# ina-foss/inaSpeechSegmenter

Hardware: AMD Instinct MI355X
Metric: hours-of-audio segmented/sec (smn+gender, 16 kHz mono) (higher is better)
Workload: dtype f32 (f16x3 split-operand MFMA, f32 accumulate; f64 FFT)

## Files before the change

### inaspeechsegmenter_amd/_native.py

```python
import ctypes as C
import os

import numpy as np

_HERE = os.path.dirname(os.path.abspath(__file__))
LIB_PATH = os.environ.get('ISS_LIB') or os.path.join(_HERE, 'libiss_hip.so')

PROG_COLS = 32
OP_CONV, OP_POOL, OP_SOFTMAX, OP_STATPOOL, OP_ACT, OP_ELT = 1, 2, 3, 4, 5, 6
(ELT_COPY, ELT_ADD, ELT_SUB, ELT_MUL, ELT_MAX, ELT_MIN, ELT_AVG, ELT_ZERO, ELT_PERMUTE) = range(9)
(C_OP, C_IN, C_OUT, C_RES, C_H, C_W, C_CIN, C_HO, C_WO, C_COUT, C_KH, C_KW, C_SH, C_SW, C_PT, C_PL,
 C_ACT, C_WOFF, C_BOFF, C_PSOFF, C_PTOFF, C_INMODE, C_POOLKIND, C_ORDER, C_FPOOLH, C_FPOOLW, C_DUALW, C_DUALB, C_ACTPARAM, C_ACTPARAM2, C_ACTPARAM3) = range(31)
PREC_BF16X3, PREC_F32, PREC_F16X3 = 0, 1, 2
K_ALIGN = 32
BUF_INPUT = -2
MAX_NETS = 8
RS_JOB = np.dtype([('src_offset', '<i8'), ('frames_in', '<i8'), ('channels', '<i4'), ('format', '<i4'), ('filter', '<i4'),
                   ('reserved', '<i4'), ('dst_offset', '<i8'), ('frames_out', '<i8')])
RS_FORMAT = {np.dtype(np.uint8): 0, np.dtype('<i2'): 1, np.dtype('<i4'): 2, np.dtype('<f4'): 3, np.dtype('<f8'): 4}
RS_I8, RS_ULAW, RS_ALAW, RS_SWAP = 8, 9, 10, 0x100
ADPCM_JOB = np.dtype([('src_offset', '<i8'), ('block_begin', '<i8'), ('nblocks', '<i8'), ('frames_total', '<i8'), ('channels', '<i4'),
                      ('block_align', '<i4'), ('output', '<i4'), ('filter', '<i4'), ('dst_offset', '<i8'), ('frames_out', '<i8')])
ADPCM_TO_SIGNAL, ADPCM_TO_STAGE = 0, 1
ADPCM_STATUS = {1: 'step index above 88'}
FLAC_INFO = np.dtype([('sample_rate', '<i4'), ('channels', '<i4'), ('bps', '<i4'), ('min_block', '<i4'), ('max_block', '<i4'),
                      ('reserved', '<i4'), ('total_samples', '<i8')])
FLAC_FRAME = np.dtype([('offset', '<i8'), ('length', '<i8'), ('first_sample', '<i8'), ('block_size', '<i4'),
                       ('channel_mode', '<i4'), ('bps', '<i4'), ('header_bytes', '<i4')])
FLAC_JOB = np.dtype([('src_offset', '<i8'), ('frame_begin', '<i8'), ('nframes', '<i8'), ('frames_total', '<i8'), ('channels', '<i4'),
                     ('bps', '<i4'), ('output', '<i4'), ('filter', '<i4'), ('dst_offset', '<i8'), ('frames_out', '<i8')])
FLAC_TO_SIGNAL, FLAC_TO_STAGE = 0, 1
FLAC_STATUS = {1: 'reserved subframe type', 2: 'subframe header padding bit set', 3: 'wasted bits exceed the sample size',
               4: 'reserved residual coding method', 5: 'residual partition order does not fit the block',
               6: 'invalid LPC precision', 7: 'negative LPC shift', 8: 'residual overruns the frame',
               9: 'nonzero padding before the footer', 10: 'subframes end before the footer', 11: 'CRC-16 mismatch'}


class NativeError(RuntimeError):
    pass


_lib = None


def lib():
    global _lib
    if _lib is not None:
        return _lib
    if not os.path.exists(LIB_PATH):
        raise NativeError(
            f"{LIB_PATH} is missing: the HIP extension has not been built. "
            "Run `python -c 'import __graft_entry__ as g; g.build()'` (needs hipcc). "
            "There is no CPU fallback for the feature/CNN path.")
    try:
        import torch
    except ImportError:
        pass
    L = C.CDLL(LIB_PATH)
    vp, i32, i64, u64 = C.c_void_p, C.c_int32, C.c_int64, C.c_uint64
    pf, pd, pi32, pi64, pu8, pi16 = (C.POINTER(C.c_float), C.POINTER(C.c_double), C.POINTER(C.c_int32),
                                     C.POINTER(C.c_int64), C.POINTER(C.c_uint8), C.POINTER(C.c_int16))
    sig = {
        'iss_create': (C.c_int, [C.c_int, C.POINTER(vp)]),
        'iss_destroy': (None, [vp]),
        'iss_last_error': (C.c_char_p, [vp]),
        'iss_version': (C.c_char_p, []),
        'iss_set_workspace_limit': (C.c_int, [vp, u64]),
        'iss_synchronize': (C.c_int, [vp]),
        'iss_sidekit_tables': (C.c_int, [vp, pd, pf]),
        'iss_signal_pcm16': (C.c_int, [vp, pi16, i64]),
        'iss_signal_f32': (C.c_int, [vp, pf, i64]),
        'iss_signal_pcm16_device': (C.c_int, [vp, vp, i64]),
        'iss_signal_pcm16_device_stream': (C.c_int, [vp, vp, i64, vp]),
        'iss_resample_filter': (C.c_int, [vp, i32, i32, pd, i64, pi32]),
        'iss_resample_pcm16': (C.c_int, [vp, vp, i64, vp, i32, i64]),
        'iss_get_signal_pcm16': (C.c_int, [vp, pi16, i64, i64]),
        'iss_resample_stats': (C.c_int, [vp, pi64, pi64]),
        'iss_flac_index': (C.c_int, [vp, i64, i64, vp, vp, i64, pi64, pi64, C.c_char_p, i32]),
        'iss_flac_crc': (C.c_int, [vp, i64, pi32, pi32]),
        'iss_flac_decode_host': (C.c_int, [vp, i64, vp, i64, i32, i32, i64, vp, pi32]),
        'iss_flac_decode': (C.c_int, [vp, vp, i64, vp, i64, vp, i32, i64, pi32]),
        'iss_flac_get_stage': (C.c_int, [vp, i32, vp, i64]),
        'iss_flac_stats': (C.c_int, [vp, pi64, pi64]),
        'iss_adpcm_decode_host': (C.c_int, [vp, i64, i64, i32, i32, i64, pi16, pi32]),
        'iss_adpcm_decode': (C.c_int, [vp, vp, i64, vp, i32, i64, i64, pi32]),
        'iss_adpcm_get_stage': (C.c_int, [vp, i32, vp, i64]),
        'iss_adpcm_stats': (C.c_int, [vp, pi64, pi64]),
        'iss_host_alloc': (C.c_int, [vp, C.c_size_t, C.POINTER(vp)]),
        'iss_host_free': (C.c_int, [vp, vp]),
        'iss_cnn_probs_async': (C.c_int, [vp, C.c_int, pi32, i32, pf, pu8, pi64]),
        'iss_cnn_dead_stats': (C.c_int, [vp, pi64, pi64]),
        'iss_wait': (C.c_int, [vp, i64]),
        'iss_comm_unique_id': (C.c_int, [vp, pu8]),
        'iss_comm_init': (C.c_int, [vp, pu8, i32, i32]),
        'iss_comm_destroy': (C.c_int, [vp]),
        'iss_allgather_segments': (C.c_int, [vp, pi32, i32, i32, pi32, pi32]),
        'iss_comm_allreduce_max': (C.c_int, [vp, pd]),
        'iss_comm_info': (C.c_int, [vp, pi32, pi32, pi32, C.c_char_p, i32]),
        'iss_sidekit': (C.c_int, [vp, pi32]),
        'iss_get_loge': (C.c_int, [vp, pf]),
        'iss_get_mspec': (C.c_int, [vp, pf]),
        'iss_set_mspec': (C.c_int, [vp, pf, i32]),
        'iss_cnn_load': (C.c_int, [vp, C.c_int, pi32, i32, pf, i64, i32, pi64, i32, i32, i32, i32]),
        'iss_cnn_load_shared': (C.c_int, [vp, C.c_int, C.c_int, pi32, i32, i32, pi64, i32, i32, i32, i32]),
        'iss_cnn_probs': (C.c_int, [vp, C.c_int, pi32, i32, pf, pu8]),
        'iss_cnn_forward': (C.c_int, [vp, C.c_int, pf, i32, pf]),
        'iss_cnn_flops': (C.c_int, [vp, C.c_int, pd]),
        'iss_set_precision': (C.c_int, [vp, C.c_int]),
        'iss_set_precision_guard': (C.c_int, [vp, C.c_float]),
        'iss_cnn_precision_info': (C.c_int, [vp, C.c_int, pi32, pf, pi32, pi32, pf]),
        'iss_cnn_set_net_precision': (C.c_int, [vp, C.c_int, C.c_int]),
        'iss_vbx_tables': (C.c_int, [vp, pd, pd]),
        'iss_vbx_features': (C.c_int, [vp, pi32, pd, i64, pf, pi32]),
        'iss_vbx_set_dither': (C.c_int, [vp, pd, i64]),
        'iss_vbx_features_pcm16': (C.c_int, [vp, pi16, i64, pf, pi32]),
        'iss_vbx_features_batch_pcm16': (C.c_int, [vp, pi16, pi64, i32, pi32, pf]),
        'iss_vbx_embed': (C.c_int, [vp, C.c_int, pi32, i32, pf]),
        'iss_prof_enable': (C.c_int, [vp, C.c_int]),
        'iss_prof_get': (C.c_int, [vp, C.c_int, pd, pi64, pd]),
        'iss_prof_reset': (C.c_int, [vp]),
        'iss_prof_get_row': (C.c_int, [vp, C.c_int, pd, pi64]),
        'iss_prof_get_instance': (C.c_int, [vp, C.c_int, C.c_char_p, i32, pd, pi64, pd]),
        'iss_set_diag': (C.c_int, [vp, C.c_uint32]),
        'iss_scribble': (C.c_int, [vp, C.c_uint32]),
        'iss_viterbi_f64': (C.c_int, [pd, i64, i32, pd, pi32]),
        'iss_viterbi_f32': (C.c_int, [pf, i64, i32, pd, pi32]),
        'iss_energy_viterbi': (C.c_int, [pf, i64, C.c_double, C.c_double, C.c_double, pd, pi32]),
        'iss_viterbi_segments_f32': (C.c_int, [pf, pi64, i64, i32, pd, pi32]),
    }
    for name, (res, args) in sig.items():
        fn = getattr(L, name)
        fn.restype = res
        fn.argtypes = args
    L._iss_symbols = tuple(sig)
    _lib = L
    return L


DIAG_BITS = {'no_shared_first': 0x001, 'no_flrows': 0x002, 'no_ws': 0x004, 'no_ws3': 0x008, 'no_direct1': 0x010,
             'no_nh2': 0x020, 'no_tr': 0x040, 'no_pw': 0x080, 'no_pws': 0x100, 'no_pws2': 0x200, 'no_wq': 0x400,
             'no_dual': 0x800, 'no_chain': 0x1000, 'no_ring': 0x2000, 'no_fsame': 0x4000, 'no_f32ws': 0x8000, 'no_ncb1': 0x10000, 'no_wsu3': 0x20000, 'no_gfused': 0x40000, 'no_hl': 0x80000,
             'no_skip_dead': 0x100000}


def diag_flags(names):
    flags = 0
    for nm in str(names).replace(' ', '').replace('+', ',').lower().split(','):
        if nm:
            flags |= DIAG_BITS[nm]
    return flags


def _ptr(a, ty):
    return a.ctypes.data_as(C.POINTER(ty))


def viterbi(emission, transition):
    L = lib()
    em = np.ascontiguousarray(emission)
    if em.dtype not in (np.float32, np.float64):
        em = em.astype(np.float64)
    tr = np.ascontiguousarray(transition, dtype=np.float64)
    T, K = em.shape
    out = np.empty(T, dtype=np.int32)
    if em.dtype == np.float32:
        rc = L.iss_viterbi_f32(_ptr(em, C.c_float), T, K, _ptr(tr, C.c_double), _ptr(out, C.c_int32))
    else:
        rc = L.iss_viterbi_f64(_ptr(em, C.c_double), T, K, _ptr(tr, C.c_double), _ptr(out, C.c_int32))
    if rc != 0:
        raise NativeError(f"iss_viterbi failed ({rc}): T={T} K={K}")
    return out


def viterbi_segments(emission, seg_len, transition):
    L = lib()
    em = np.ascontiguousarray(emission, dtype=np.float32)
    sl = np.ascontiguousarray(seg_len, dtype=np.int64)
    tr = np.ascontiguousarray(transition, dtype=np.float64)
    n, K = em.shape
    assert int(sl.sum()) == n
    out = np.empty(n, dtype=np.int32)
    rc = L.iss_viterbi_segments_f32(_ptr(em, C.c_float), _ptr(sl, C.c_int64), sl.size, K, _ptr(tr, C.c_double), _ptr(out, C.c_int32))
    if rc != 0:
        raise NativeError(f"iss_viterbi_segments_f32 failed ({rc}): n={n} K={K} segments={sl.size}")
    return out


_LOG_EPS = np.log(np.full(1, 1e-10))[0], np.log(np.full(1, 1 - 1e-10))[0]


def energy_viterbi(loge, threshold, transition):
    L = lib()
    x = np.ascontiguousarray(loge, dtype=np.float32)
    tr = np.ascontiguousarray(transition, dtype=np.float64)
    out = np.empty(x.size, dtype=np.int32)
    rc = L.iss_energy_viterbi(_ptr(x, C.c_float), x.size, float(threshold), float(_LOG_EPS[0]), float(_LOG_EPS[1]),
                              _ptr(tr, C.c_double), _ptr(out, C.c_int32))
    if rc != 0:
        raise NativeError(f"iss_energy_viterbi failed ({rc}): T={x.size}")
    return out


def flac_crc(buf):
    b = np.frombuffer(bytes(buf), dtype=np.uint8)
    c8, c16 = C.c_int32(), C.c_int32()
    if lib().iss_flac_crc(C.c_void_p(b.ctypes.data), b.size, C.byref(c8), C.byref(c16)) != 0:
        raise NativeError('iss_flac_crc failed')
    return c8.value, c16.value


def flac_index(buf, first_frame, info):
    L = lib()
    inf = np.ascontiguousarray(np.array(info, dtype=FLAC_INFO).reshape(1))
    cap = max(16, int(inf['total_samples'][0]) // max(1, int(inf['min_block'][0]) or 1) + 2) if inf['total_samples'][0] > 0 \
        else buf.size // 64 + 16
    err = C.create_string_buffer(256)
    n, off = C.c_int64(), C.c_int64()
    for _ in range(2):
        rows = np.zeros(cap, dtype=FLAC_FRAME)
        rc = L.iss_flac_index(C.c_void_p(buf.ctypes.data), buf.size, int(first_frame), C.c_void_p(inf.ctypes.data),
                              C.c_void_p(rows.ctypes.data), cap, C.byref(n), C.byref(off), err, 256)
        if rc != -5:
            break
        cap = buf.size // 9 + 16
    if rc != 0:
        raise ValueError(off.value, err.value.decode())
    return rows[:n.value].copy()


def flac_decode_host(buf, frames, channels, bps, frames_total):
    fr = np.ascontiguousarray(frames, dtype=FLAC_FRAME)
    out = np.empty((int(frames_total), int(channels)), dtype=np.int32 if bps > 16 else np.int16)
    st = np.zeros(len(fr), dtype=np.int32)
    rc = lib().iss_flac_decode_host(C.c_void_p(buf.ctypes.data), buf.size, C.c_void_p(fr.ctypes.data), len(fr), int(channels),
                                    int(bps), int(frames_total), C.c_void_p(out.ctypes.data), _ptr(st, C.c_int32))
    if rc != 0:
        raise NativeError(f'iss_flac_decode_host failed ({rc}): bad frame rows')
    return (out[:, 0] if channels == 1 else out), st


def adpcm_decode_host(buf, nblocks, channels, block_align, frames_total):
    buf = np.ascontiguousarray(buf, dtype=np.uint8)
    out = np.empty((int(frames_total), int(channels)), dtype=np.int16)
    st = np.zeros(int(nblocks), dtype=np.int32)
    rc = lib().iss_adpcm_decode_host(C.c_void_p(buf.ctypes.data), buf.size, int(nblocks), int(channels), int(block_align),
                                     int(frames_total), _ptr(out, C.c_int16), _ptr(st, C.c_int32))
    if rc != 0:
        raise NativeError(f'iss_adpcm_decode_host failed ({rc}): bad block geometry')
    return (out[:, 0] if channels == 1 else out), st


class Context:

    def __init__(self, device=0):
        self._L = lib()
        h = C.c_void_p()
        rc = self._L.iss_create(int(device), C.byref(h))
        if rc != 0:
            raise NativeError(f"iss_create(device={device}) failed ({rc}): "
                              f"{self._L.iss_last_error(None).decode()}")
        self._h = h
        self.device = device
        self.T = 0
        self._net_out = {}
        self._dither_n = 0
        self._pinned = {}
        self.comm_rank, self.comm_world = 0, 1
        self.precision = None
        self.workspace_limit = None
        self.diag = 0
        env = os.environ.get('ISS_DIAG', '')
        if env:
            self.set_diag(diag_flags(env))
        self.guard_threshold = None
        env = os.environ.get('ISS_PREC_GUARD', '')
        if env:
            self.set_precision_guard(float(env))

    def close(self):
        if getattr(self, '_h', None):
            for p in list(self._pinned.values()):
                self._L.iss_host_free(self._h, C.c_void_p(p))
            self._pinned.clear()
            self._L.iss_destroy(self._h)
            self._h = None

    def __del__(self):
        try:
            self.close()
        except Exception:
            pass

    def _ck(self, rc, what):
        if rc != 0:
            raise NativeError(f"{what} failed ({rc}): {self._L.iss_last_error(self._h).decode()}")

    def sidekit_tables(self, window, melbank):
        w = np.ascontiguousarray(window, dtype=np.float64)
        b = np.ascontiguousarray(melbank, dtype=np.float32)
        assert w.shape == (400,) and b.shape == (24, 257)
        self._ck(self._L.iss_sidekit_tables(self._h, _ptr(w, C.c_double), _ptr(b, C.c_float)), 'iss_sidekit_tables')

    def set_signal(self, sig):
        sig = np.ascontiguousarray(sig)
        if sig.dtype == np.int16:
            self._ck(self._L.iss_signal_pcm16(self._h, _ptr(sig, C.c_int16), sig.size), 'iss_signal_pcm16')
        elif sig.dtype == np.float32:
            self._ck(self._L.iss_signal_f32(self._h, _ptr(sig, C.c_float), sig.size), 'iss_signal_f32')
        else:
            raise TypeError(f"signal dtype {sig.dtype}: need int16 or float32")
        self._keep = sig

    def set_signal_device(self, dev_ptr, n, producer_stream=None):
        self._ck(self._L.iss_signal_pcm16_device_stream(self._h, C.c_void_p(int(dev_ptr)), int(n),
                                                        C.c_void_p(int(producer_stream)) if producer_stream else None),
                 'iss_signal_pcm16_device')

    def resample_filter(self, sr):
        from . import resample
        up, down, h = resample.plan(sr)
        fid = C.c_int32()
        self._ck(self._L.iss_resample_filter(self._h, up, down, _ptr(h, C.c_double), h.size, C.byref(fid)), 'iss_resample_filter')
        return fid.value, up, down

    def resample_job(self, x, sr, src_offset, dst_offset, fmt=None):
        fid, up, down = self.resample_filter(sr)
        n = x.shape[0]
        return (src_offset, n, 1 if x.ndim == 1 else x.shape[1], RS_FORMAT[x.dtype] if fmt is None else int(fmt), fid, 0,
                dst_offset, -(-n * up // down))

    def resample(self, src, jobs, n_signal=-1):
        src = np.ascontiguousarray(src, dtype=np.uint8)
        jb = np.ascontiguousarray(np.array(jobs, dtype=RS_JOB))
        self._ck(self._L.iss_resample_pcm16(self._h, C.c_void_p(src.ctypes.data), src.size, C.c_void_p(jb.ctypes.data),
                                            jb.size, int(n_signal)), 'iss_resample_pcm16')
        self._keep_rs = src

    def resample_signal(self, x, sr, fmt=None):
        x = np.ascontiguousarray(x)
        job = self.resample_job(x, sr, 0, 0, fmt)
        self.resample(x.reshape(-1).view(np.uint8), [job], n_signal=job[-1])
        return job[-1]

    def get_signal_pcm16(self, offset, n):
        out = np.empty(int(n), dtype=np.int16)
        self._ck(self._L.iss_get_signal_pcm16(self._h, _ptr(out, C.c_int16), int(offset), int(n)), 'iss_get_signal_pcm16')
        return out

    def _counters(self, fn):
        a, b = C.c_int64(), C.c_int64()
        self._ck(getattr(self._L, fn)(self._h, C.byref(a), C.byref(b)), fn)
        return a.value, b.value

    def _get_stage(self, fn, job, frames_total, channels, dtype):
        out = np.empty((int(frames_total), int(channels)), dtype=dtype)
        self._ck(getattr(self._L, fn)(self._h, int(job), C.c_void_p(out.ctypes.data), out.nbytes), fn)
        return out[:, 0] if channels == 1 else out

    def resample_stats(self):
        return self._counters('iss_resample_stats')

    def _status(self, name, n):
        st, n = self.__dict__.get(name), max(int(n), 1)
        if st is None or st.size < n:
            if st is not None:
                self.pinned_free(st)
            st = self.__dict__[name] = self.pinned_empty((int(n * 1.25) + 256,), np.int32)
        return st

    def flac_decode(self, src, frames, jobs, n_signal=-1):
        src = np.ascontiguousarray(src, dtype=np.uint8)
        fr = np.ascontiguousarray(frames, dtype=FLAC_FRAME)
        jb = np.ascontiguousarray(np.array(jobs, dtype=FLAC_JOB).reshape(-1))
        st = self._status('_flac_status', len(fr))
        self._ck(self._L.iss_flac_decode(self._h, C.c_void_p(src.ctypes.data), src.size, C.c_void_p(fr.ctypes.data), len(fr),
                                         C.c_void_p(jb.ctypes.data), jb.size, int(n_signal), _ptr(st, C.c_int32)),
                 'iss_flac_decode')
        self._keep_flac = (src, fr)
        return st[:len(fr)]

    def flac_get_stage(self, job, frames_total, channels, bps):
        return self._get_stage('iss_flac_get_stage', job, frames_total, channels, np.int32 if bps > 16 else np.int16)

    def flac_stats(self):
        return self._counters('iss_flac_stats')

    def adpcm_decode(self, src, jobs, nblocks, n_signal=-1):
        src = np.ascontiguousarray(src, dtype=np.uint8)
        jb = np.ascontiguousarray(np.array(jobs, dtype=ADPCM_JOB).reshape(-1))
        st = self._status('_adpcm_status', nblocks)
        self._ck(self._L.iss_adpcm_decode(self._h, C.c_void_p(src.ctypes.data), src.size, C.c_void_p(jb.ctypes.data), jb.size,
                                          int(nblocks), int(n_signal), _ptr(st, C.c_int32)), 'iss_adpcm_decode')
        self._keep_adpcm = src
        return st[:int(nblocks)]

    def adpcm_get_stage(self, job, frames_total, channels):
        return self._get_stage('iss_adpcm_get_stage', job, frames_total, channels, np.int16)

    def adpcm_stats(self):
        return self._counters('iss_adpcm_stats')

    def pinned_empty(self, shape, dtype):
        dt = np.dtype(dtype)
        n = int(np.prod(shape)) * dt.itemsize
        p = C.c_void_p()
        self._ck(self._L.iss_host_alloc(self._h, n, C.byref(p)), 'iss_host_alloc')
        buf = (C.c_uint8 * max(n, 1)).from_address(p.value)
        a = np.frombuffer(buf, dtype=dt, count=int(np.prod(shape))).reshape(shape)
        self._pinned[a.ctypes.data] = p.value
        return a

    def pinned_free(self, a):
        p = self._pinned.pop(a.ctypes.data, None)
        if p is not None and self._h:
            self._ck(self._L.iss_host_free(self._h, C.c_void_p(p)), 'iss_host_free')

    def sidekit(self):
        t = C.c_int32()
        self._ck(self._L.iss_sidekit(self._h, C.byref(t)), 'iss_sidekit')
        self.T = t.value
        return self.T

    def get_loge(self):
        out = np.empty(self.T, dtype=np.float32)
        self._ck(self._L.iss_get_loge(self._h, _ptr(out, C.c_float)), 'iss_get_loge')
        return out

    def get_mspec(self):
        out = np.empty((self.T, 24), dtype=np.float32)
        self._ck(self._L.iss_get_mspec(self._h, _ptr(out, C.c_float)), 'iss_get_mspec')
        return out

    def set_mspec(self, mspec):
        m = np.ascontiguousarray(mspec, dtype=np.float32)
        assert m.ndim == 2 and m.shape[1] == 24
        self._ck(self._L.iss_set_mspec(self._h, _ptr(m, C.c_float), m.shape[0]), 'iss_set_mspec')
        self.T = m.shape[0]

    def cnn_load(self, net_id, compiled):
        prog = np.ascontiguousarray(compiled.prog, dtype=np.int32)
        blob = np.ascontiguousarray(compiled.blob, dtype=np.float32)
        be = np.ascontiguousarray(compiled.buf_elems, dtype=np.int64)
        h, w, c = compiled.in_shape
        self._ck(self._L.iss_cnn_load(self._h, net_id, _ptr(prog, C.c_int32), prog.shape[0], _ptr(blob, C.c_float),
                                      blob.size, be.size, _ptr(be, C.c_int64), h, w, c, compiled.out_dim),
                 'iss_cnn_load')
        self._net_out[net_id] = compiled.out_dim

    def cnn_load_shared(self, net_id, src_id, compiled):
        prog = np.ascontiguousarray(compiled.prog, dtype=np.int32)
        be = np.ascontiguousarray(compiled.buf_elems, dtype=np.int64)
        h, w, c = compiled.in_shape
        self._ck(self._L.iss_cnn_load_shared(self._h, net_id, src_id, _ptr(prog, C.c_int32), prog.shape[0], be.size,
                                             _ptr(be, C.c_int64), h, w, c, compiled.out_dim), 'iss_cnn_load_shared')
        self._net_out[net_id] = compiled.out_dim

    def cnn_probs(self, net_id, win_row):
        wr = np.ascontiguousarray(win_row, dtype=np.int32)
        n = wr.size
        probs = np.empty((n, self._net_out[net_id]), dtype=np.float32)
        fin = np.empty(n, dtype=np.uint8)
        self._ck(self._L.iss_cnn_probs(self._h, net_id, _ptr(wr, C.c_int32), n, _ptr(probs, C.c_float),
                                       _ptr(fin, C.c_uint8)), 'iss_cnn_probs')
        return probs, fin.astype(bool)

    def cnn_probs_async(self, net_id, win_row, probs_out=None, finite_out=None):
        wr = np.ascontiguousarray(win_row, dtype=np.int32)
        n = wr.size
        if probs_out is None:
            probs_out = np.empty((n, self._net_out[net_id]), dtype=np.float32)
        if finite_out is None:
            finite_out = np.empty(n, dtype=np.uint8)
        assert probs_out.size >= n * self._net_out[net_id] and finite_out.size >= n
        t = C.c_int64(-1)
        self._ck(self._L.iss_cnn_probs_async(self._h, net_id, _ptr(wr, C.c_int32), n, _ptr(probs_out, C.c_float),
                                             _ptr(finite_out, C.c_uint8), C.byref(t)), 'iss_cnn_probs_async')
        return t.value, probs_out, finite_out

    def cnn_dead_stats(self):
        w, d = C.c_int64(0), C.c_int64(0)
        self._ck(self._L.iss_cnn_dead_stats(self._h, C.byref(w), C.byref(d)), 'iss_cnn_dead_stats')
        return {'windows': w.value, 'dead': d.value}

    def wait(self, ticket=-1):
        self._ck(self._L.iss_wait(self._h, int(ticket)), 'iss_wait')

    def comm_unique_id(self):
        buf = np.zeros(128, dtype=np.uint8)
        self._ck(self._L.iss_comm_unique_id(self._h, _ptr(buf, C.c_uint8)), 'iss_comm_unique_id')
        return buf.tobytes()

    def comm_init(self, uid, rank, world):
        buf = np.frombuffer(bytes(uid), dtype=np.uint8).copy()
        assert buf.size == 128
        self._ck(self._L.iss_comm_init(self._h, _ptr(buf, C.c_uint8), int(rank), int(world)), 'iss_comm_init')
        self.comm_rank, self.comm_world = int(rank), int(world)

    def comm_destroy(self):
        self._ck(self._L.iss_comm_destroy(self._h), 'iss_comm_destroy')
        self.comm_rank, self.comm_world = 0, 1

    def allgather_segments(self, rows, capacity):
        world = self.comm_world
        out = np.zeros((world, capacity, 4), dtype=np.int32)
        counts = np.zeros(world, dtype=np.int32)
        if rows is None:
            rows, n = np.zeros((1, 4), np.int32), -1
        else:
            rows = np.ascontiguousarray(rows, dtype=np.int32).reshape(-1, 4)
            n = rows.shape[0]
        self._ck(self._L.iss_allgather_segments(self._h, _ptr(rows, C.c_int32), n, int(capacity),
                                                _ptr(out, C.c_int32), _ptr(counts, C.c_int32)), 'iss_allgather_segments')
        return out, counts

    def comm_info(self):
        w, r, v = C.c_int32(), C.c_int32(), C.c_int32()
        buf = C.create_string_buffer(512)
        self._ck(self._L.iss_comm_info(self._h, C.byref(w), C.byref(r), C.byref(v), buf, 512), 'iss_comm_info')
        return {'world': w.value, 'rank': r.value, 'version': v.value, 'lib': buf.value.decode(errors='replace')}

    def comm_allreduce_max(self, value):
        v = C.c_double(float(value))
        self._ck(self._L.iss_comm_allreduce_max(self._h, C.byref(v)), 'iss_comm_allreduce_max')
        return v.value

    def cnn_forward(self, net_id, x):
        x = np.ascontiguousarray(x, dtype=np.float32)
        n = x.shape[0]
        out = np.empty((n, self._net_out[net_id]), dtype=np.float32)
        self._ck(self._L.iss_cnn_forward(self._h, net_id, _ptr(x, C.c_float), n, _ptr(out, C.c_float)), 'iss_cnn_forward')
        return out

    def cnn_flops(self, net_id):
        f = C.c_double()
        self._ck(self._L.iss_cnn_flops(self._h, net_id, C.byref(f)), 'iss_cnn_flops')
        return f.value

    def set_precision(self, mode):
        self._ck(self._L.iss_set_precision(self._h, int(mode)), 'iss_set_precision')
        self.precision = int(mode)

    def set_precision_guard(self, threshold):
        self._ck(self._L.iss_set_precision_guard(self._h, float(threshold)), 'iss_set_precision_guard')
        self.guard_threshold = float(threshold)

    def cnn_precision_info(self, net_id):
        mode, slots, state, d, du = C.c_int32(0), C.c_int32(0), C.c_int32(0), C.c_float(0), C.c_float(0)
        self._ck(self._L.iss_cnn_precision_info(self._h, int(net_id), C.byref(mode), C.byref(d), C.byref(slots), C.byref(state), C.byref(du)),
                 'iss_cnn_precision_info')
        return {'mode': {PREC_F32: 'f32', PREC_F16X3: 'f16x3'}.get(mode.value, 'bf16x3'), 'max_dlogp': None if d.value < 0 else float(d.value),
                'max_dlogp_in_use': None if du.value < 0 else float(du.value),
                'slots': slots.value, 'state': ('pending', 'passed', 'escalated', 'fixed')[state.value]}

    def cnn_set_net_precision(self, net_id, mode):
        self._ck(self._L.iss_cnn_set_net_precision(self._h, int(net_id), int(mode)), 'iss_cnn_set_net_precision')

    def set_workspace_limit(self, nbytes):
        self._ck(self._L.iss_set_workspace_limit(self._h, int(nbytes)), 'iss_set_workspace_limit')
        self.workspace_limit = int(nbytes)

    def mirror_settings(self, other):
        if getattr(other, 'precision', None) is not None and other.precision != getattr(self, 'precision', None):
            self.set_precision(other.precision)
        if getattr(other, 'workspace_limit', None) is not None and other.workspace_limit != getattr(self, 'workspace_limit', None):
            self.set_workspace_limit(other.workspace_limit)
        if getattr(other, 'diag', 0) != getattr(self, 'diag', 0):
            self.set_diag(other.diag)
        if getattr(other, 'guard_threshold', None) is not None and other.guard_threshold != getattr(self, 'guard_threshold', None):
            self.set_precision_guard(other.guard_threshold)

    def set_diag(self, flags):
        flags = diag_flags(flags) if isinstance(flags, str) else int(flags)
        self._ck(self._L.iss_set_diag(self._h, flags), 'iss_set_diag')
        self.diag = flags

    def scribble(self, word):
        self._ck(self._L.iss_scribble(self._h, int(word) & 0xFFFFFFFF), 'iss_scribble')

    def synchronize(self):
        self._ck(self._L.iss_synchronize(self._h), 'iss_synchronize')

    def vbx_tables(self, window, melbank):
        w = np.ascontiguousarray(window, dtype=np.float64)
        b = np.ascontiguousarray(melbank, dtype=np.float64)
        assert w.shape == (400,) and b.shape == (257, 64)
        self._ck(self._L.iss_vbx_tables(self._h, _ptr(w, C.c_double), _ptr(b, C.c_double)), 'iss_vbx_tables')

    def vbx_features(self, sig_i32, dither_u):
        s = np.ascontiguousarray(sig_i32, dtype=np.int32)
        u = np.ascontiguousarray(dither_u, dtype=np.float64)
        assert s.shape == u.shape and s.ndim == 1
        T = (s.size + 320 - 400) // 160 + 1
        out = np.empty((T, 64), dtype=np.float32)
        t = C.c_int32()
        self._ck(self._L.iss_vbx_features(self._h, _ptr(s, C.c_int32), _ptr(u, C.c_double), s.size,
                                          _ptr(out, C.c_float), C.byref(t)), 'iss_vbx_features')
        self._dither_n = 0
        assert t.value == T
        return out

    def vbx_set_dither(self, dither_u):
        u = np.ascontiguousarray(dither_u, dtype=np.float64)
        self._ck(self._L.iss_vbx_set_dither(self._h, _ptr(u, C.c_double), u.size), 'iss_vbx_set_dither')
        self._dither_n = u.size

    def vbx_features_pcm16(self, pcm, to_host=True):
        s = np.ascontiguousarray(pcm, dtype=np.int16)
        T = (s.size + 320 - 400) // 160 + 1
        t = C.c_int32()
        if not to_host:
            self._ck(self._L.iss_vbx_features_pcm16(self._h, _ptr(s, C.c_int16), s.size, None, C.byref(t)), 'iss_vbx_features_pcm16')
            assert t.value == T
            return T
        out = np.empty((T, 64), dtype=np.float32)
        self._ck(self._L.iss_vbx_features_pcm16(self._h, _ptr(s, C.c_int16), s.size, _ptr(out, C.c_float), C.byref(t)),
                 'iss_vbx_features_pcm16')
        assert t.value == T
        return out

    def vbx_features_batch_pcm16(self, pcms, to_host=True):
        pcms = [np.asarray(p, dtype=np.int16) for p in pcms]
        soff = np.zeros(len(pcms) + 1, dtype=np.int64)
        soff[1:] = np.cumsum([p.size for p in pcms])
        s = np.ascontiguousarray(np.concatenate(pcms) if pcms else np.zeros(0, np.int16))
        foff = np.zeros(len(pcms) + 1, dtype=np.int32)
        T = int(sum((p.size + 320 - 400) // 160 + 1 for p in pcms))
        out = np.empty((T, 64), dtype=np.float32) if to_host else None
        self._ck(self._L.iss_vbx_features_batch_pcm16(self._h, _ptr(s, C.c_int16), _ptr(soff, C.c_int64), len(pcms),
                                                      _ptr(foff, C.c_int32), _ptr(out, C.c_float) if to_host else None),
                 'iss_vbx_features_batch_pcm16')
        return foff, out

    def vbx_embed(self, net_id, starts):
        st = np.ascontiguousarray(starts, dtype=np.int32)
        out = np.empty((st.size, self._net_out[net_id]), dtype=np.float32)
        self._ck(self._L.iss_vbx_embed(self._h, net_id, _ptr(st, C.c_int32), st.size, _ptr(out, C.c_float)), 'iss_vbx_embed')
        return out

    def prof_enable(self, on=True):
        self._ck(self._L.iss_prof_enable(self._h, 1 if on else 0), 'iss_prof_enable')

    def prof_reset(self):
        self._ck(self._L.iss_prof_reset(self._h), 'iss_prof_reset')

    def prof_get(self, kind):
        ms, n, fl = C.c_double(), C.c_int64(), C.c_double()
        self._ck(self._L.iss_prof_get(self._h, kind, C.byref(ms), C.byref(n), C.byref(fl)), 'iss_prof_get')
        return ms.value, n.value, fl.value

    def prof_instances(self):
        out = []
        buf = C.create_string_buffer(192)
        i = 0
        while True:
            ms, n, fl = C.c_double(), C.c_int64(), C.c_double()
            if self._L.iss_prof_get_instance(self._h, i, buf, 192, C.byref(ms), C.byref(n), C.byref(fl)) != 0:
                break
            out.append({'kernel': buf.value.decode(), 'ms': ms.value, 'launches': n.value, 'flops': fl.value})
            i += 1
        return out

    def prof_get_row(self, row):
        ms, n = C.c_double(), C.c_int64()
        self._ck(self._L.iss_prof_get_row(self._h, int(row), C.byref(ms), C.byref(n)), 'iss_prof_get_row')
        return ms.value, n.value
```

### inaspeechsegmenter_amd/csrc/cnn.hip

```cpp
#include "conv_select.h"

using namespace issk;

namespace {

template <int MODE>
__global__ __launch_bounds__(256) void conv_igemm_kernel(const ConvArgs p) {
    __shared__ __attribute__((aligned(16))) float sA[2][BM * LDK];
    __shared__ __attribute__((aligned(16))) float sB[2][BN * LDK];

    const int tid = threadIdx.x, lane = tid & 63, wv = tid >> 6;
    unsigned mt, nt;
    gemm_tile_of_block(blockIdx.x, p.nblk, p.nblk_n, mt, nt);
    const long long m0 = (long long)mt * BM;
    const int n0 = (int)nt * BN;

    const int k4 = tid & 3;
    const int lr = tid >> 2;
    RowSrc rs[2];
#pragma unroll
    for (int j = 0; j < 2; ++j) rs[j] = row_source<MODE>(p, m0 + lr + 64 * j);
    const int bn = n0 + lr;
    const bool bok = bn < p.Cout;
    const float* wrow = p.w + (size_t)(bok ? bn : 0) * p.Kpad + k4 * 4;
// ... 918 lines not shown
    return ISS_OK;
}

namespace {
int cnn_set_program(iss_ctx* c, IssNet& n, const char* who, const int32_t* prog, int32_t nrows, int64_t blob_floats,
                    int32_t nbuf, const int64_t* buf_elems, int32_t in_h, int32_t in_w, int32_t in_c, int32_t out_dim,
                    std::vector<int32_t>& ktab) {
    n.prog.assign(prog, prog + (size_t)nrows * ISS_PROG_COLS);
    n.nrows = nrows; n.nbuf = nbuf; n.buf_elems.assign(buf_elems, buf_elems + nbuf);
    n.in_h = in_h; n.in_w = in_w; n.in_c = in_c; n.out_dim = out_dim;
    n.kpad.assign(nrows, 0); n.ktab_off.assign(nrows, -1);
    double flops = 0;
    for (int r = 0; r < nrows; ++r) {
        const int32_t* R = &n.prog[(size_t)r * ISS_PROG_COLS];
        auto bad = [&](const char* what) { return iss_fail(c, ISS_EINVAL, "%s: row %d: %s", who, r, what); };
        if (R[ISS_C_IN] != ISS_BUF_INPUT && (R[ISS_C_IN] < 0 || R[ISS_C_IN] >= nbuf)) return bad("IN buffer id");
        if (R[ISS_C_OUT] < 0 || R[ISS_C_OUT] >= nbuf) return bad("OUT buffer id");
        if (R[ISS_C_OP] == ISS_OP_CONV) {
            const int K = R[ISS_C_KH] * R[ISS_C_KW] * R[ISS_C_CIN];
            const int Kpad = roundup(K, KALIGN);
            if (K <= 0 || R[ISS_C_COUT] <= 0) return bad("conv shape");
            if (R[ISS_C_WOFF] < 0 || (R[ISS_C_WOFF] & 7) || (int64_t)R[ISS_C_WOFF] + (int64_t)R[ISS_C_COUT] * Kpad > blob_floats)
                return bad("weight offset misaligned or outside blob (weights must be [Cout][roundup32(K)], offset % 8 == 0)");
            if (R[ISS_C_RES] >= nbuf) return bad("RES buffer id");
            if (R[ISS_C_KH] > 32767 || R[ISS_C_KW] > 32767) return bad("kernel too large");
            int fph, fpw;
            fused_pool_of(R, fph, fpw);
            if (fph * fpw != 1 && fph * fpw != 2 && fph * fpw != 4) return bad("fused pool window must cover 2 or 4 outputs");
            if (fph * fpw > 1 && (R[ISS_C_RES] >= 0 || R[ISS_C_HO] / fph < 1 || R[ISS_C_WO] / fpw < 1))
                return bad("fused pool with residual / empty pooled output");
            const bool patch = R[ISS_C_INMODE] == 1;
            const bool window = R[ISS_C_INMODE] == 2;
            if (patch && (R[ISS_C_CIN] != 1 || R[ISS_C_H] != 68 || R[ISS_C_W] > 24)) return bad("patch-mode conv must read (68, <=24, 1)");
            if (window && (R[ISS_C_CIN] != 1 || R[ISS_C_H] != 64)) return bad("window-mode conv must read (64, frames, 1)");
            const int rs = patch ? 24 : (window ? 1 : R[ISS_C_W] * R[ISS_C_CIN]);
            const int ps = patch ? 1 : (window ? R[ISS_C_H] : R[ISS_C_CIN]);
            n.kpad[r] = Kpad; n.ktab_off[r] = (int64_t)ktab.size();
            for (int k = 0; k < Kpad; ++k) {
                if (k < K) {
                    const int cc = k % R[ISS_C_CIN], kk = k / R[ISS_C_CIN];
                    const int kx = kk % R[ISS_C_KW], ky = kk / R[ISS_C_KW];
                    ktab.push_back(ky * rs + kx * ps + cc);
                    ktab.push_back((ky << 16) | kx);
                } else {
                    ktab.push_back(0);
                    ktab.push_back((0x7fff << 16) | 0x7fff);
                }
            }
            flops += 2.0 * K * R[ISS_C_COUT] * (double)(R[ISS_C_HO] / fph * fph) * (double)(R[ISS_C_WO] / fpw * fpw);
            if (R[ISS_C_DUALW] != 0 || R[ISS_C_DUALB] != 0) {
                if (r < 1) return bad("ISS_C_DUALW on the first row");
                const int32_t* P = &n.prog[(size_t)(r - 1) * ISS_PROG_COLS];
                int pph, ppw;
                fused_pool_of(P, pph, ppw);
                const bool shapes = P[ISS_C_OP] == ISS_OP_CONV && P[ISS_C_KH] == 1 && P[ISS_C_KW] == 1 && R[ISS_C_KH] == 1 && R[ISS_C_KW] == 1 &&
                                    R[ISS_C_SH] == 1 && R[ISS_C_SW] == 1 && P[ISS_C_SH] >= 1 && P[ISS_C_SW] >= 1 &&
                                    R[ISS_C_PT] == 0 && R[ISS_C_PL] == 0 && P[ISS_C_PT] == 0 && P[ISS_C_PL] == 0 &&
                                    R[ISS_C_INMODE] == 0 && P[ISS_C_INMODE] == 0 && fph * fpw == 1 && pph * ppw == 1 &&
                                    R[ISS_C_HO] == R[ISS_C_H] && R[ISS_C_WO] == R[ISS_C_W] && P[ISS_C_HO] == R[ISS_C_HO] &&
                                    P[ISS_C_WO] == R[ISS_C_WO] && P[ISS_C_COUT] == R[ISS_C_COUT] &&
                                    (P[ISS_C_HO] - 1) * P[ISS_C_SH] < P[ISS_C_H] && (P[ISS_C_WO] - 1) * P[ISS_C_SW] < P[ISS_C_W] &&
                                    R[ISS_C_CIN] % 32 == 0 && P[ISS_C_CIN] % 32 == 0;
                const bool chain = R[ISS_C_RES] >= 0 && R[ISS_C_RES] == P[ISS_C_OUT] && R[ISS_C_OUT] == R[ISS_C_RES] &&
                                   R[ISS_C_IN] != P[ISS_C_OUT] && P[ISS_C_IN] != P[ISS_C_OUT] && P[ISS_C_RES] < 0 && P[ISS_C_ACT] == 0 &&
                                   P[ISS_C_PSOFF] < 0 && R[ISS_C_PSOFF] < 0 && P[ISS_C_BOFF] >= 0 && R[ISS_C_BOFF] >= 0;
                const int64_t wo = (int64_t)R[ISS_C_DUALW] - 1, bo = (int64_t)R[ISS_C_DUALB] - 1;
                const bool offs = wo >= 0 && bo >= 0 && (wo & 7) == 0 &&
                                  wo + (int64_t)R[ISS_C_COUT] * (R[ISS_C_CIN] + P[ISS_C_CIN]) <= blob_floats && bo + R[ISS_C_COUT] <= blob_floats;
                if (!shapes || !chain || !offs)
                    return bad("ISS_C_DUALW / ISS_C_DUALB: rows r - 1, r are not a linear 1x1 projection and the in-place 1x1 expansion it is added to, "
                               "or the concatenated parameters lie outside the blob (include/iss.h)");
            }
        } else if (R[ISS_C_OP] == ISS_OP_ACT) {
            if (R[ISS_C_ACT] < 4 || R[ISS_C_ACT] > 9) return bad("ISS_OP_ACT: activation code must be 4 (elu), 5 (leaky relu), 6 (selu), 7 (softplus), 8 (relu with max_value) or 9 (keras ReLU in full)");
            if (R[ISS_C_IN] == ISS_BUF_INPUT) return bad("ISS_OP_ACT: an elementwise activation cannot read the network input (it works in place)");
        } else if (R[ISS_C_OP] == ISS_OP_ELT) {
            const int k = R[ISS_C_ACT];
            const long long hw = (long long)R[ISS_C_H] * R[ISS_C_W];
            if (k < ISS_ELT_COPY || k > ISS_ELT_PERMUTE) return bad("ISS_OP_ELT: unknown kind");
            if (R[ISS_C_HO] < 1 || R[ISS_C_WO] < 1 || R[ISS_C_COUT] < 1 || R[ISS_C_CIN] < 1 || hw < 1) return bad("ISS_OP_ELT: shape");
            if ((long long)R[ISS_C_HO] * R[ISS_C_WO] * R[ISS_C_COUT] > buf_elems[R[ISS_C_OUT]]) return bad("ISS_OP_ELT: output larger than its buffer");
            if (R[ISS_C_IN] != ISS_BUF_INPUT && k != ISS_ELT_ZERO && hw * R[ISS_C_CIN] > buf_elems[R[ISS_C_IN]]) return bad("ISS_OP_ELT: input larger than its buffer");
            if (R[ISS_C_IN] == ISS_BUF_INPUT && k != ISS_ELT_ZERO) return bad("ISS_OP_ELT: a merge row cannot read the network input");
            if (k >= ISS_ELT_ADD && k <= ISS_ELT_AVG) {
                if (R[ISS_C_RES] < 0 || R[ISS_C_RES] >= nbuf) return bad("ISS_OP_ELT: a binary row needs its second operand in ISS_C_RES");
                if (R[ISS_C_HO] != R[ISS_C_H] || R[ISS_C_WO] != R[ISS_C_W] || R[ISS_C_COUT] != R[ISS_C_CIN]) return bad("ISS_OP_ELT: binary rows keep the shape");
                if (hw * R[ISS_C_CIN] > buf_elems[R[ISS_C_RES]]) return bad("ISS_OP_ELT: second operand larger than its buffer");
            } else if (k == ISS_ELT_COPY || k == ISS_ELT_ZERO) {
                if (R[ISS_C_HO] != R[ISS_C_H] || R[ISS_C_WO] != R[ISS_C_W]) return bad("ISS_OP_ELT: COPY / ZERO keep the pixel grid");
                if (R[ISS_C_KH] < 1 || R[ISS_C_PL] < 0 || R[ISS_C_PL] + R[ISS_C_KH] > R[ISS_C_COUT]) return bad("ISS_OP_ELT: destination channel range outside COUT");
                if (k == ISS_ELT_COPY && (R[ISS_C_PT] < 0 || R[ISS_C_PT] + R[ISS_C_KH] > R[ISS_C_CIN] || R[ISS_C_IN] == R[ISS_C_OUT]))
                    return bad("ISS_OP_ELT: COPY source channel range outside CIN, or IN == OUT");
            } else {
                const int pm[3] = {R[ISS_C_KH], R[ISS_C_KW], R[ISS_C_SH]};
                const int dims[3] = {R[ISS_C_H], R[ISS_C_W], R[ISS_C_CIN]};
                if (pm[0] < 0 || pm[0] > 2 || pm[1] < 0 || pm[1] > 2 || pm[2] < 0 || pm[2] > 2 || pm[0] == pm[1] || pm[0] == pm[2] || pm[1] == pm[2])
                    return bad("ISS_OP_ELT: PERMUTE needs a permutation of (0, 1, 2) in KH, KW, SH");
                if (R[ISS_C_HO] != dims[pm[0]] || R[ISS_C_WO] != dims[pm[1]] || R[ISS_C_COUT] != dims[pm[2]] || R[ISS_C_IN] == R[ISS_C_OUT])
                    return bad("ISS_OP_ELT: PERMUTE output shape is not the permuted input shape, or IN == OUT");
            }
        } else if (R[ISS_C_OP] != ISS_OP_POOL && R[ISS_C_OP] != ISS_OP_SOFTMAX && R[ISS_C_OP] != ISS_OP_STATPOOL) {
            return bad("unknown op");
        }
    }
    n.flops_per_sample = flops; n.blob_floats = blob_floats;
    return ISS_OK;
}

int cnn_upload_tables(iss_ctx* c, IssNet& n, const float* blob, const std::vector<int32_t>& ktab) {
    const int nrows = n.nrows;
    {
        std::vector<float> wsum;
        n.wsum_off.assign(nrows, -1);
        n.wsumx_off.assign(nrows, -1);
        std::vector<float> wdev;
        for (int r = 0; r < nrows; ++r) {
            const int32_t* R = &n.prog[(size_t)r * ISS_PROG_COLS];
            if (R[ISS_C_OP] != ISS_OP_CONV || R[ISS_C_INMODE] != 1) continue;
            const int K = R[ISS_C_KH] * R[ISS_C_KW] * R[ISS_C_CIN];
            const float* w = blob ? blob + R[ISS_C_WOFF] : nullptr;
            if (!w) {
                wdev.resize((size_t)R[ISS_C_COUT] * n.kpad[r]);
                ISS_HIP(c, hipMemcpy(wdev.data(), n.d_blob + R[ISS_C_WOFF], wdev.size() * sizeof(float), hipMemcpyDeviceToHost));
                w = wdev.data();
            }
            n.wsum_off[r] = (int64_t)wsum.size();
            for (int co = 0; co < R[ISS_C_COUT]; ++co) {
                double acc = 0.0;
                for (int k = 0; k < K; ++k) acc += (double)w[(int64_t)co * n.kpad[r] + k];
                wsum.push_back((float)acc);
            }
            while (wsum.size() % 8) wsum.push_back(0.f);
            if ((R[ISS_C_PT] != 0 || R[ISS_C_PL] != 0 || R[ISS_C_WO] == R[ISS_C_W]) && R[ISS_C_CIN] == 1 && R[ISS_C_SW] == 1) {
                n.wsumx_off[r] = (int64_t)wsum.size();
                const int W = R[ISS_C_W], kh = R[ISS_C_KH], kw = R[ISS_C_KW], pl = R[ISS_C_PL];
                for (int x = 0; x < W; ++x)
                    for (int co = 0; co < R[ISS_C_COUT]; ++co) {
                        double acc = 0.0;
                        for (int ky = 0; ky < kh; ++ky)
                            for (int kx = 0; kx < kw; ++kx)
                                if (x - pl + kx >= 0 && x - pl + kx < W) acc += (double)w[(int64_t)co * n.kpad[r] + ky * kw + kx];
                        wsum.push_back((float)acc);
                    }
                while (wsum.size() % 8) wsum.push_back(0.f);
            }
        }
        if (!wsum.empty()) {
            ISS_HIP(c, hipMalloc((void**)&n.d_wsum, wsum.size() * sizeof(float)));
            ISS_HIP(c, hipMemcpy(n.d_wsum, wsum.data(), wsum.size() * sizeof(float), hipMemcpyHostToDevice));
        }
    }
    if (!ktab.empty()) {
        ISS_HIP(c, hipMalloc((void**)&n.d_ktab, ktab.size() * sizeof(int32_t)));
        ISS_HIP(c, hipMemcpy(n.d_ktab, ktab.data(), ktab.size() * sizeof(int32_t), hipMemcpyHostToDevice));
    }
    return ISS_OK;
}
}

extern "C" int iss_cnn_load(iss_ctx* c, int id, const int32_t* prog, int32_t nrows, const float* blob,
                            int64_t blob_floats, int32_t nbuf, const int64_t* buf_elems, int32_t in_h, int32_t in_w,
                            int32_t in_c, int32_t out_dim) {
    if (!c) return ISS_EINVAL;
    if (id < 0 || id >= ISS_MAX_NETS || !prog || nrows <= 0 || !blob || blob_floats <= 0 || nbuf <= 0 || !buf_elems)
        return iss_fail(c, ISS_EINVAL, "iss_cnn_load: bad argument");
    ISS_HIP(c, hipSetDevice(c->device));
    iss_cnn_free(c, id);
    IssNet& n = c->nets[id];
    std::vector<int32_t> ktab;
    int rc = cnn_set_program(c, n, "iss_cnn_load", prog, nrows, blob_floats, nbuf, buf_elems, in_h, in_w, in_c, out_dim, ktab);
    if (rc) return rc;
    ISS_HIP(c, hipMalloc((void**)&n.d_blob, (size_t)blob_floats * sizeof(float)));
    ISS_HIP(c, hipMemcpy(n.d_blob, blob, (size_t)blob_floats * sizeof(float), hipMemcpyHostToDevice));
    {
        std::vector<uint16_t> hi((size_t)blob_floats), lo((size_t)blob_floats);
        for (int64_t i = 0; i < blob_floats; ++i) {
            hi[i] = bf16_rne(blob[i]);
            lo[i] = bf16_rne(blob[i] - bf16_to_f32(hi[i]));
        }
        std::vector<uint16_t> hi16((size_t)blob_floats), lo16((size_t)blob_floats);
        n.f16_ok = true;
        for (int64_t i = 0; i < blob_floats; ++i) {
            const float x = blob[i];
            if (!(std::fabs(x) < 65504.f)) { n.f16_ok = false; hi16[i] = lo16[i] = 0; continue; }
            const _Float16 h = (_Float16)x;
            const _Float16 l = (_Float16)(x - (float)h);
            memcpy(&hi16[i], &h, 2); memcpy(&lo16[i], &l, 2);
        }
        ISS_HIP(c, hipMalloc((void**)&n.d_wh16, (size_t)blob_floats * 2 + 16));
        ISS_HIP(c, hipMalloc((void**)&n.d_wl16, (size_t)blob_floats * 2 + 16));
        ISS_HIP(c, hipMemcpy(n.d_wh16, hi16.data(), (size_t)blob_floats * 2, hipMemcpyHostToDevice));
        ISS_HIP(c, hipMemcpy(n.d_wl16, lo16.data(), (size_t)blob_floats * 2, hipMemcpyHostToDevice));
        ISS_HIP(c, hipMalloc((void**)&n.d_wh, (size_t)blob_floats * 2 + 16));
        ISS_HIP(c, hipMalloc((void**)&n.d_wl, (size_t)blob_floats * 2 + 16));
        ISS_HIP(c, hipMemcpy(n.d_wh, hi.data(), (size_t)blob_floats * 2, hipMemcpyHostToDevice));
        ISS_HIP(c, hipMemcpy(n.d_wl, lo.data(), (size_t)blob_floats * 2, hipMemcpyHostToDevice));
    }
    if ((rc = cnn_upload_tables(c, n, blob, ktab))) return rc;
    n.loaded = true;
    return ISS_OK;
}

extern "C" int iss_cnn_load_shared(iss_ctx* c, int id, int src, const int32_t* prog, int32_t nrows, int32_t nbuf,
                                   const int64_t* buf_elems, int32_t in_h, int32_t in_w, int32_t in_c, int32_t out_dim) {
    if (!c) return ISS_EINVAL;
    if (id < 0 || id >= ISS_MAX_NETS || src < 0 || src >= ISS_MAX_NETS || src == id || !prog || nrows <= 0 || nbuf <= 0 || !buf_elems)
        return iss_fail(c, ISS_EINVAL, "iss_cnn_load_shared: bad argument");
    if (!c->nets[src].loaded || !c->nets[src].d_blob)
        return iss_fail(c, ISS_ESTATE, "iss_cnn_load_shared: source net %d not loaded", src);
    ISS_HIP(c, hipSetDevice(c->device));
    iss_cnn_free(c, id);
    IssNet& s = c->nets[src];
    IssNet& n = c->nets[id];
    std::vector<int32_t> ktab;
    int rc = cnn_set_program(c, n, "iss_cnn_load_shared", prog, nrows, s.blob_floats, nbuf, buf_elems, in_h, in_w, in_c, out_dim, ktab);
    if (rc) return rc;
    if (!s.shared_params) {
        s.shared_params = std::make_shared<IssParamArrays>();
        IssParamArrays& a = *s.shared_params;
        a.blob = s.d_blob; a.wh = s.d_wh; a.wl = s.d_wl; a.wh16 = s.d_wh16; a.wl16 = s.d_wl16;
    }
    n.shared_params = s.shared_params;
    n.d_blob = s.d_blob; n.d_wh = s.d_wh; n.d_wl = s.d_wl; n.d_wh16 = s.d_wh16; n.d_wl16 = s.d_wl16;
    n.f16_ok = s.f16_ok;
    if ((rc = cnn_upload_tables(c, n, nullptr, ktab))) return rc;
    n.loaded = true;
    return ISS_OK;
}

extern "C" int iss_set_precision(iss_ctx* c, int mode) {
    if (!c) return ISS_EINVAL;
    if (mode != ISS_PREC_BF16X3 && mode != ISS_PREC_F32 && mode != ISS_PREC_F16X3) return iss_fail(c, ISS_EINVAL, "iss_set_precision: unknown mode %d", mode);
    if (mode == c->precision) return ISS_OK;
    c->precision = mode;
    for (IssNet& n : c->nets) {
        if (!n.loaded || n.prec_by_caller) continue;
        n.prec_override = -1;
        n.guard_state = ISS_GUARD_PENDING;
        n.guard_dlogp = n.guard_dlogp_chosen = -1.f;
        n.guard_slots = 0;
    }
    return ISS_OK;
}

extern "C" int iss_set_precision_guard(iss_ctx* c, float threshold) {
    if (!c) return ISS_EINVAL;
    if (!(threshold == threshold)) return iss_fail(c, ISS_EINVAL, "iss_set_precision_guard: threshold is NaN");
    c->guard_threshold = threshold;
    return ISS_OK;
}

extern "C" int iss_cnn_set_net_precision(iss_ctx* c, int id, int mode) {
    if (!c || id < 0 || id >= ISS_MAX_NETS) return ISS_EINVAL;
    if (mode != -1 && mode != ISS_PREC_BF16X3 && mode != ISS_PREC_F32 && mode != ISS_PREC_F16X3) return iss_fail(c, ISS_EINVAL, "iss_cnn_set_net_precision: unknown mode %d", mode);
    if (!c->nets[id].loaded) return iss_fail(c, ISS_ESTATE, "net %d not loaded", id);
    c->nets[id].prec_override = mode;
    c->nets[id].prec_by_caller = mode != -1;
    c->nets[id].guard_state = mode == -1 ? ISS_GUARD_PENDING : ISS_GUARD_FIXED;
    return ISS_OK;
}

static bool net_reads_patches(const IssNet& n) {
    for (int r = 0; r < n.nrows; ++r)
        if (n.prog[(size_t)r * ISS_PROG_COLS + ISS_C_OP] == ISS_OP_CONV && n.prog[(size_t)r * ISS_PROG_COLS + ISS_C_INMODE] == 1) return true;
    return false;
}

static int effective_precision(const iss_ctx* c, const IssNet& n) {
    const int prec = n.prec_override >= 0 ? n.prec_override : c->precision;
    if (prec == ISS_PREC_F16X3 && !(n.f16_ok && n.d_wh16 != nullptr && net_reads_patches(n))) return ISS_PREC_BF16X3;
    return prec;
}

extern "C" int iss_cnn_precision_info(iss_ctx* c, int id, int32_t* mode, float* max_dlogp, int32_t* slots, int32_t* state, float* dlogp_in_use) {
    if (!c || id < 0 || id >= ISS_MAX_NETS) return ISS_EINVAL;
    const IssNet& n = c->nets[id];
    if (!n.loaded) return iss_fail(c, ISS_ESTATE, "net %d not loaded", id);
    if (mode) *mode = effective_precision(c, n);
    if (max_dlogp) *max_dlogp = n.guard_dlogp;
    if (slots) *slots = n.guard_slots;
    if (state) *state = n.guard_state;
    if (dlogp_in_use) *dlogp_in_use = n.guard_dlogp_chosen;
    return ISS_OK;
}

extern "C" int iss_set_diag(iss_ctx* c, uint32_t flags) {
    if (!c) return ISS_EINVAL;
    if (flags & ~(uint32_t)ISS_DIAG_ALL) return iss_fail(c, ISS_EINVAL, "iss_set_diag: unknown bits 0x%x", flags & ~(uint32_t)ISS_DIAG_ALL);
    c->diag = flags;
    return ISS_OK;
}

extern "C" int iss_cnn_flops(iss_ctx* c, int id, double* f) {
    if (!c || id < 0 || id >= ISS_MAX_NETS || !f) return ISS_EINVAL;
    if (!c->nets[id].loaded) return iss_fail(c, ISS_ESTATE, "net %d not loaded", id);
    *f = c->nets[id].flops_per_sample;
    return ISS_OK;
}

namespace {

struct PassIo { const int32_t* d_winrow; const float* d_stats; const uint8_t* d_fin; const float* d_input; };

int conv_args(iss_ctx* c, IssNet& n, const PassIo& io, int bc, const ConvChoice& ch, ConvArgs& a) {
    const int r = ch.row;
    const int32_t* R = &n.prog[(size_t)r * ISS_PROG_COLS];
    memset(&a, 0, sizeof(a));
    fill_geometry(a, R, bc);
    a.in = R[ISS_C_IN] == ISS_BUF_INPUT ? io.d_input : (const float*)c->act[R[ISS_C_IN]].p;
    a.w = n.d_blob + R[ISS_C_WOFF];
    a.bias = R[ISS_C_BOFF] >= 0 ? n.d_blob + R[ISS_C_BOFF] : nullptr;
    a.ps = R[ISS_C_PSOFF] >= 0 ? n.d_blob + R[ISS_C_PSOFF] : nullptr;
    a.pt = R[ISS_C_PTOFF] >= 0 ? n.d_blob + R[ISS_C_PTOFF] : nullptr;
    a.res = R[ISS_C_RES] >= 0 ? (const float*)c->act[R[ISS_C_RES]].p : nullptr;
    a.out = (float*)c->act[R[ISS_C_OUT]].p;
    a.ktab = n.d_ktab + n.ktab_off[r];
    a.wh = n.d_wh + R[ISS_C_WOFF]; a.wl = n.d_wl + R[ISS_C_WOFF];
    a.Kpad = n.kpad[r]; a.mode = ch.mode; a.tmr = ch.tmr;
    if (ch.kernel == ConvKernel::Dhl) return ISS_OK;
    if (R[ISS_C_INMODE] == 1) {
        if (!io.d_winrow) return iss_fail(c, ISS_ESTATE, "patch-mode network run without a window list");
        a.in = (const float*)c->mspec.p; a.win_row = io.d_winrow; a.stats = io.d_stats; a.finite = io.d_fin;
    } else if (R[ISS_C_INMODE] == 2) {
        if (!io.d_winrow || !c->vbx_out.p) return iss_fail(c, ISS_ESTATE, "window-mode network run without resident vbx features");
        a.in = (const float*)c->vbx_out.p; a.win_row = io.d_winrow;
    } else if (!a.in) return iss_fail(c, ISS_ESTATE, "network input missing");
    a.nblk = (unsigned)((a.M + BM - 1) / BM);
    set_fast_div(a, 0, a.pp); set_fast_div(a, 1, a.pw); set_fast_div(a, 2, a.Hq * a.Wq); set_fast_div(a, 3, a.Wq);
#ifdef ISS_EXPERIMENTS
    { static const int dbg = getenv("ISS_DBG") ? atoi(getenv("ISS_DBG")) : 0; a.dbg = dbg; }
#endif
    a.nblk_n = (unsigned)((a.Cout + BN - 1) / BN);
    if (ch.kernel == ConvKernel::Pwc) {
        const int32_t* Q = &n.prog[(size_t)ch.partner * ISS_PROG_COLS];
        a.wh2 = n.d_wh + Q[ISS_C_WOFF]; a.wl2 = n.d_wl + Q[ISS_C_WOFF];
        a.bias2 = Q[ISS_C_BOFF] >= 0 ? n.d_blob + Q[ISS_C_BOFF] : nullptr;
        a.out2 = (float*)c->act[Q[ISS_C_OUT]].p;
        a.act2 = Q[ISS_C_ACT]; a.Cout2 = Q[ISS_C_COUT];
    } else if (ch.kernel == ConvKernel::Pws2Dual) {
        const int32_t* P = &n.prog[(size_t)ch.partner * ISS_PROG_COLS];
        a.in2 = P[ISS_C_IN] == ISS_BUF_INPUT ? io.d_input : (const float*)c->act[P[ISS_C_IN]].p;
        a.Cin2 = P[ISS_C_CIN]; a.H2 = P[ISS_C_H]; a.W2 = P[ISS_C_W]; a.sh2 = P[ISS_C_SH]; a.sw2 = P[ISS_C_SW];
        const int64_t wo = (int64_t)R[ISS_C_DUALW] - 1;
        a.w = n.d_blob + wo; a.wh = n.d_wh + wo; a.wl = n.d_wl + wo;
        a.bias = n.d_blob + (R[ISS_C_DUALB] - 1); a.res = nullptr;
        a.Kpad = a.Cin + a.Cin2;
    }
    if (ch.f16) { a.f16 = 1; a.wh = n.d_wh16 + R[ISS_C_WOFF]; a.wl = n.d_wl16 + R[ISS_C_WOFF]; }
    if (ch.kernel == ConvKernel::Wq3h) { a.in_hl = 1; a.in_np = ch.in_np; }
    if (ch.out != OutLayout::F32) { a.out_hl = 1; a.out_np = ch.out_np; a.out_f16 = ch.generic_out && ch.out_f16 ? 1 : 0; }
    return ISS_OK;
}

int launch_shared_first_layer(iss_ctx* c, IssNet& n, const PassIo& io, int pend, int bc, int rmin, int rmax, ConvArgs& a, double* fl) {
    const int32_t* R1 = &n.prog[(size_t)pend * ISS_PROG_COLS];
    const bool fs1 = R1[ISS_C_HO] == R1[ISS_C_H];
    int ph1, pw1;
    fused_pool_of(R1, ph1, pw1);
    const bool pool1 = ph1 * pw1 != 1;
    const long long rrows = (long long)(rmax - rmin) + R1[ISS_C_HO];
    const long long rtot = rrows * R1[ISS_C_WO] * (R1[ISS_C_COUT] / 4);
    const int f_ne = fs1 ? R1[ISS_C_KH] - 1 : 0;
    const long long etot = (long long)bc * f_ne * R1[ISS_C_WO] * (R1[ISS_C_COUT] / 4);
    const int plane_rows = pool1 ? (int)(rrows / ph1) + 2 : 0;
    const long long ptot = pool1 ? (long long)ph1 * plane_rows * (R1[ISS_C_WO] / pw1) * (R1[ISS_C_COUT] / 4) : 0;
    { const int rc = iss_reserve(c, c->raw1, (size_t)(rtot + etot + ptot) * 16 + (pool1 ? (size_t)bc * 4 + 16 : 0)); if (rc) return rc; }
    float* Rraw = (float*)c->raw1.p;
    const float* mspec = (const float*)c->mspec.p;
    const float* w1 = n.d_blob + R1[ISS_C_WOFF];
    const size_t lds1 = (size_t)R1[ISS_C_KH] * R1[ISS_C_KW] * R1[ISS_C_COUT] * 4;
    iss_prof_begin(c, 2, 0);
    if (fs1) {
        const int pt1 = R1[ISS_C_PT], pl1 = R1[ISS_C_PL], pb1 = R1[ISS_C_KH] - 1 - pt1;
        const float* S = n.d_wsum + n.wsumx_off[pend];
        if (rtot >= (1ll << 31) || etot >= (1ll << 31)) return iss_fail(c, ISS_EINVAL, "internal: shared first layer over %lld + %lld items", rtot, etot);
        hipLaunchKernelGGL(first_layer_same_kernel, dim3((unsigned)std::min<long long>((rtot + 255) / 256, 4096)), dim3(256), lds1, c->stream,
                           mspec, (int)c->T, rmin, rtot, R1[ISS_C_WO], R1[ISS_C_COUT], R1[ISS_C_KH], R1[ISS_C_KW], pt1, pl1, w1, n.kpad[pend], Rraw);
        if (etot > 0)
            hipLaunchKernelGGL(first_layer_edge_kernel, dim3((unsigned)std::min<long long>((etot + 255) / 256, 8192)), dim3(256), lds1, c->stream,
                               mspec, io.d_winrow, io.d_stats, etot, R1[ISS_C_H], R1[ISS_C_WO], R1[ISS_C_COUT], R1[ISS_C_KH],
                               R1[ISS_C_KW], pt1, pb1, pl1, w1, n.kpad[pend], S, Rraw + (size_t)rtot * 4);
        a.f_padt = pt1; a.f_padb = pb1; a.f_erow0 = (int)rrows;
    } else {
        const dim3 rgrid((unsigned)std::min<long long>((rtot + 255) / 256, 4096));
        const bool no_rows = (c->diag & ISS_DIAG_NO_FLROWS) != 0;
        const bool rows_ok = !no_rows && R1[ISS_C_KH] == 4 && R1[ISS_C_KW] == 5 && (R1[ISS_C_WO] == 17 || R1[ISS_C_WO] == 20) &&
                             rrows * (R1[ISS_C_COUT] / 4) < (1ll << 31);
        const dim3 rowgrid((unsigned)std::min<long long>((rrows * (R1[ISS_C_COUT] / 4) + 255) / 256, 4096));
        if (rows_ok && R1[ISS_C_WO] == 17)
            hipLaunchKernelGGL((first_layer_rows_kernel<4, 5, 17>), rowgrid, dim3(256), lds1, c->stream, mspec, rmin, (int)rrows, R1[ISS_C_COUT], w1, n.kpad[pend], Rraw);
        else if (rows_ok)
            hipLaunchKernelGGL((first_layer_rows_kernel<4, 5, 20>), rowgrid, dim3(256), lds1, c->stream, mspec, rmin, (int)rrows, R1[ISS_C_COUT], w1, n.kpad[pend], Rraw);
        else if (R1[ISS_C_KH] == 4 && R1[ISS_C_KW] == 5)
            hipLaunchKernelGGL((first_layer_raw_kernel<4, 5>), rgrid, dim3(256), lds1, c->stream, mspec, rmin, rtot, R1[ISS_C_WO], R1[ISS_C_COUT], 4, 5, w1, n.kpad[pend], Rraw);
        else
            hipLaunchKernelGGL((first_layer_raw_kernel<0, 0>), rgrid, dim3(256), lds1, c->stream, mspec, rmin, rtot, R1[ISS_C_WO], R1[ISS_C_COUT],
                               R1[ISS_C_KH], R1[ISS_C_KW], w1, n.kpad[pend], Rraw);
    }
    a.in = Rraw; a.win_row = io.d_winrow; a.f_rmin = rmin;
    if (pool1) {
        if (ptot >= (1ll << 40)) return iss_fail(c, ISS_EINVAL, "internal: pooled first layer over %lld items", ptot);
        float* P = Rraw + (size_t)(rtot + etot) * 4;
        int32_t* wr2 = reinterpret_cast<int32_t*>(P + (size_t)ptot * 4);
        hipLaunchKernelGGL(pool_rows_kernel, dim3((unsigned)std::min<long long>((ptot + 255) / 256, 8192)), dim3(256), 0, c->stream,
                           (const float*)Rraw, P, ptot, (int)rrows, R1[ISS_C_WO], R1[ISS_C_COUT], ph1, pw1, plane_rows);
        hipLaunchKernelGGL(winrow_pool_kernel, dim3((unsigned)((bc + 255) / 256)), dim3(256), 0, c->stream, io.d_winrow, wr2, bc, rmin, ph1, plane_rows);
        a.in = P; a.win_row = wr2; a.f_rmin = 0;
    }
    iss_prof_end(c);
    a.stats = io.d_stats; a.finite = io.d_fin;
    a.f_bias = n.d_blob + R1[ISS_C_BOFF];
    a.f_wsum = fs1 ? n.d_wsum + n.wsumx_off[pend] : n.d_wsum + n.wsum_off[pend];
    a.f_ps = R1[ISS_C_PSOFF] >= 0 ? n.d_blob + R1[ISS_C_PSOFF] : nullptr;
    a.f_pt = R1[ISS_C_PTOFF] >= 0 ? n.d_blob + R1[ISS_C_PTOFF] : nullptr;
    a.f_act = R1[ISS_C_ACT];
    *fl += 2.0 * R1[ISS_C_KH] * R1[ISS_C_KW] * (double)R1[ISS_C_COUT] * (double)bc * R1[ISS_C_HO] * R1[ISS_C_WO];
    return ISS_OK;
}

int launch_conv(iss_ctx* c, IssNet& n, const ConvChoice& ch, ConvArgs& a, double fl) {
    const int r = ch.row;
    const int32_t* R = &n.prog[(size_t)r * ISS_PROG_COLS];
    const bool padded = ch.padded, tr = ch.tr, fused = ch.fused;
    const int nh = ch.nh;
    const dim3 grid(a.nblk, a.nblk_n);
    const unsigned ny = (unsigned)std::max(1, a.Cout / (2 * BN));
    const unsigned tiles = (unsigned)((a.M + WS_TM - 1) / WS_TM);
    const unsigned groups = (unsigned)((a.M + (long long)WS_TM * WS_G - 1) / ((long long)WS_TM * WS_G));
    const unsigned qtiles = ch.tmr > 0 ? (unsigned)((a.M + ch.tmr - 1) / ch.tmr) : 0;
    iss_prof_begin(c, 0, fl);
    iss_prof_tag(c, ch.tag), iss_prof_row(c, r), iss_prof_inst(c, "%s", inst_name(ch).c_str());
    switch (ch.kernel) {
    case ConvKernel::Dhl: {
        const int K = R[ISS_C_CIN];
        uint16_t*& wp = n.dhl_wp[{r, ch.f16 ? 1 : 0}];
        if (!wp) {
            ISS_HIP(c, hipMalloc((void**)&wp, dhl_packed_elems(K, R[ISS_C_COUT]) * 2));
            iss_dhl_pack((ch.f16 ? n.d_wh16 : n.d_wh) + R[ISS_C_WOFF], (ch.f16 ? n.d_wl16 : n.d_wl) + R[ISS_C_WOFF], wp, R[ISS_C_COUT], n.kpad[r], K, c->stream);
        }
        DhlArgs d;
        d.a = reinterpret_cast<const uint16_t*>(a.in); d.wp = wp; d.bias = a.bias; d.out = a.out;
        d.np = ch.in_np; d.M = (int)a.M; d.K = K; d.Cout = R[ISS_C_COUT]; d.act = R[ISS_C_ACT];
        iss_dhl_launch(d, c->stream, ch.f16);
        break;
    }
    case ConvKernel::Pwc: iss_pwc_launch(a, c->stream); break;
    case ConvKernel::Pws2Dual: iss_pws2_launch(a, c->stream, false, true); break;
    case ConvKernel::Direct1: {
        const long long items = (long long)(a.M / ((long long)a.H * a.W)) * ((a.H + 7) / 8) * a.W * (a.Cout / 4);
        if (items >= (1ll << 32)) return iss_fail(c, ISS_EINVAL, "internal: direct first layer over %lld work items", items);
        const dim3 dgrid((unsigned)std::min<long long>((items + 255) / 256, 8192));
        const size_t dlds = (size_t)9 * a.Cout * sizeof(float);
        if (ch.window) hipLaunchKernelGGL(conv1_direct3x3_kernel<true>, dgrid, dim3(256), dlds, c->stream, a);
        else hipLaunchKernelGGL(conv1_direct3x3_kernel<false>, dgrid, dim3(256), dlds, c->stream, a);
        break;
    }
    case ConvKernel::WsNh2F32: iss_ws_launch_f32_nh2_3x3(a, dim3(std::min<unsigned>(tiles, std::max(1u, 256u / ny)), ny), c->stream, tr); break;
    case ConvKernel::WsNh2: {
        const dim3 g2(std::min<unsigned>(tiles, std::max(1u, 256u / ny)), ny);
        if (padded && !tr) iss_ws_launch_nh2_3x3_padded_pool(a, g2, c->stream);
        else if (padded) iss_ws_launch_nh2_3x3_padded(a, g2, c->stream);
        else iss_ws_launch_nh2_3x3(a, g2, c->stream, tr);
        break;
    }
    case ConvKernel::Wq3: case ConvKernel::Wq3h: {
        const dim3 qgrid(std::min<unsigned>((qtiles + 1) / 2, std::max(1u, 256u / ny)), ny);
        if (ch.kernel == ConvKernel::Wq3h) iss_wq3h_launch(a, qgrid, c->stream, ch.kind);
        else iss_wq3_launch(a, qgrid, c->stream, ch.kind);
        break;
    }
    case ConvKernel::WsPlainU: iss_ws_launch_plain_3x3_unpadded(a, dim3(std::min<unsigned>(groups, std::max(1u, 256u / grid.y)), grid.y), c->stream, tr); break;
    case ConvKernel::WsPlain: iss_ws_launch_plain_3x3(a, dim3(std::min<unsigned>(groups, std::max(1u, 256u / grid.y)), grid.y), c->stream); break;
    case ConvKernel::WsF32Fused: iss_ws_launch_f32_fused_5x3(a, dim3(std::min<unsigned>(groups, 256u), grid.y), c->stream); break;
    case ConvKernel::WsRing: iss_ws_launch_ring(a, dim3(std::min<unsigned>(qtiles, 256u), grid.y), c->stream, padded); break;
    case ConvKernel::WsFs: {
        const dim3 wgrid(std::min<unsigned>(tiles, 256u), grid.y);
        if (tr) iss_ws_launch_fs_5x3_tr(a, wgrid, c->stream);
        else if (a.H_k == 5) iss_ws_launch_fs_5x3(a, wgrid, c->stream, padded);
        else iss_ws_launch_fs_3x3(a, wgrid, c->stream, padded);
        break;
    }
    case ConvKernel::WsNcb1: iss_ws_launch_ncb1_5x3(a, dim3(std::min<unsigned>(groups, 256u), grid.y), c->stream); break;
    case ConvKernel::Wq: iss_wq_launch_5x3(a, dim3(std::min<unsigned>((qtiles + 1) / 2, 256u), grid.y), c->stream); break;
    case ConvKernel::Ws: {
        const dim3 wgrid(std::min<unsigned>(groups, 256u), grid.y);
#define ISS_WS_CASE(KH_, KW_) if (a.H_k == KH_ && a.kw == KW_) iss_ws_launch_##KH_##x##KW_(a, wgrid, c->stream, padded, tr, fused); else
        ISS_WS_SHAPES(ISS_WS_CASE) { return iss_fail(c, ISS_EINVAL, "internal: no weight-stationary kernel for %dx%d", a.H_k, a.kw); }
#undef ISS_WS_CASE
        break;
    }
    case ConvKernel::Fp: {
        const dim3 pgrid(std::min<unsigned>(a.nblk, 512u), grid.y / nh);
#define ISS_FP_CASE(KH_, KW_) if (a.H_k == KH_ && a.kw == KW_) iss_fp_launch_##KH_##x##KW_(a, pgrid, c->stream, padded, tr, fused, nh); else
        ISS_FP_SHAPES(ISS_FP_CASE) { return iss_fail(c, ISS_EINVAL, "internal: no footprint kernel for %dx%d", a.H_k, a.kw); }
#undef ISS_FP_CASE
        break;
    }
    case ConvKernel::Patch1: {
        const dim3 pgrid(std::min<unsigned>(a.nblk, 512u), grid.y);
        if (tr && ch.f16) hipLaunchKernelGGL((conv1_patch_x3_kernel<true, true>), pgrid, dim3(256), 0, c->stream, a);
        else if (tr) hipLaunchKernelGGL((conv1_patch_x3_kernel<true, false>), pgrid, dim3(256), 0, c->stream, a);
        else if (ch.f16) hipLaunchKernelGGL((conv1_patch_x3_kernel<false, true>), pgrid, dim3(256), 0, c->stream, a);
        else hipLaunchKernelGGL((conv1_patch_x3_kernel<false, false>), pgrid, dim3(256), 0, c->stream, a);
        break;
    }
    case ConvKernel::Gather: case ConvKernel::X3: {
        constexpr int ntn = 2;
        a.nblk_n = (unsigned)((a.Cout + 32 * ntn - 1) / (32 * ntn));
        const dim3 gridw(a.nblk * a.nblk_n);
        if (a.mode == 4 && tr) hipLaunchKernelGGL((conv_x3_kernel<4, true, 2>), gridw, dim3(256), 0, c->stream, a);
        else if (a.mode == 4) hipLaunchKernelGGL((conv_x3_kernel<4, false, 2>), gridw, dim3(256), 0, c->stream, a);
        else if (a.mode == 3 && tr) hipLaunchKernelGGL((conv_x3_kernel<3, true, 2>), gridw, dim3(256), 0, c->stream, a);
        else if (a.mode == 3) hipLaunchKernelGGL((conv_x3_kernel<3, false, 2>), gridw, dim3(256), 0, c->stream, a);
        else if (a.mode == 0 && tr) hipLaunchKernelGGL((conv_x3_kernel<0, true, 2>), gridw, dim3(256), 0, c->stream, a);
        else if (a.mode == 0) hipLaunchKernelGGL((conv_x3_kernel<0, false, 2>), gridw, dim3(256), 0, c->stream, a);
        else if (a.mode == 1 && tr) hipLaunchKernelGGL((conv_x3_kernel<1, true, 2>), gridw, dim3(256), 0, c->stream, a);
        else if (a.mode == 1) hipLaunchKernelGGL((conv_x3_kernel<1, false, 2>), gridw, dim3(256), 0, c->stream, a);
        else hipLaunchKernelGGL((conv_x3_kernel<2, false, 2>), gridw, dim3(256), 0, c->stream, a);
        break;
    }
    case ConvKernel::Pws2Strided: case ConvKernel::Pws2: case ConvKernel::Pws: case ConvKernel::Pw: {
        if (ch.kernel == ConvKernel::Pws2Strided) iss_pws2_launch(a, c->stream, true);
        else if (ch.kernel == ConvKernel::Pws2) iss_pws2_launch(a, c->stream);
        else if (ch.kernel == ConvKernel::Pws) iss_pws_launch(a, dim3(std::min<unsigned>(a.nblk * a.nblk_n, 512u)), c->stream);
        else if (ch.f16) hipLaunchKernelGGL(conv_x3_pw_kernel<true>, dim3(std::min<unsigned>(a.nblk * a.nblk_n, 768u)), dim3(256), 0, c->stream, a);
        else hipLaunchKernelGGL(conv_x3_pw_kernel<false>, dim3(std::min<unsigned>(a.nblk * a.nblk_n, 768u)), dim3(256), 0, c->stream, a);
        break;
    }
    case ConvKernel::Igemm: {
        const dim3 grid1(a.nblk * a.nblk_n);
        if (a.mode == 0) hipLaunchKernelGGL(conv_igemm_kernel<0>, grid1, dim3(256), 0, c->stream, a);
        else if (a.mode == 1) hipLaunchKernelGGL(conv_igemm_kernel<1>, grid1, dim3(256), 0, c->stream, a);
        else hipLaunchKernelGGL(conv_igemm_kernel<2>, grid1, dim3(256), 0, c->stream, a);
        break;
    }
    case ConvKernel::Declined: return iss_fail(c, ISS_EINVAL, "internal: row %d has no kernel", r);
    }
    iss_prof_end(c);
    return ISS_OK;
}

int run_conv(iss_ctx* c, IssNet& n, const ConvEnv& env, const PassIo& io, const ConvChoice& ch, int pend) {
    const int32_t* R = &n.prog[(size_t)ch.row * ISS_PROG_COLS];
    ConvArgs a;
    int rc = conv_args(c, n, io, env.bc, ch, a);
    if (rc) return rc;
    double fl = conv_flops(R, (double)a.M);
    if (ch.kernel == ConvKernel::Dhl) fl = 2.0 * R[ISS_C_CIN] * (double)R[ISS_C_COUT] * (double)env.bc;
    if (ch.kernel == ConvKernel::Pwc) fl += 2.0 * a.Cout * (double)a.Cout2 * (double)a.M;
    if (ch.kernel == ConvKernel::Pws2Dual) fl += 2.0 * a.Cin2 * (double)a.Cout * (double)a.M;
    if (ch.first == FirstLayer::Fused || ch.first == FirstLayer::Gather)
        if ((rc = launch_shared_first_layer(c, n, io, pend, env.bc, env.rmin, env.rmax, a, &fl))) return rc;
    return launch_conv(c, n, ch, a, fl);
}

int run_program(iss_ctx* c, IssNet& n, int bc, const int32_t* d_winrow, const float* d_stats,
                const uint8_t* d_fin, const float* d_input, float** result, int rmin = 0, int rmax = -1,
                bool share_first = false) {
    const PassIo io{d_winrow, d_stats, d_fin, d_input};
    std::vector<ChlState> layout(std::max<size_t>(c->act.size(), (size_t)n.nbuf));
    ConvEnv env = make_env(n, bc, rmin, rmax, share_first, effective_precision(c, n), c->diag, d_winrow != nullptr, d_input != nullptr,
                           c->vbx_out.p != nullptr, layout.data());
    int pending = -1;
    for (int r = 0; r < n.nrows; ++r) {
        const int32_t* R = &n.prog[(size_t)r * ISS_PROG_COLS];
        const float* in = R[ISS_C_IN] == ISS_BUF_INPUT ? d_input : (const float*)c->act[R[ISS_C_IN]].p;
        float* out = (float*)c->act[R[ISS_C_OUT]].p;
        const int op = R[ISS_C_OP];
        ChlState out_layout;
        if (op == ISS_OP_CONV) {
            if (pending < 0 && can_defer(env, r)) { pending = r; *result = out; continue; }
            const ConvChoice ch = select_conv(env, r, pending);
            int rc = ISS_OK;
            if (ch.first == FirstLayer::Alone) rc = run_conv(c, n, env, io, select_row(env, pending, -1, -1, -1), -1);
            if (!rc) rc = run_conv(c, n, env, io, ch, pending);
            if (pending >= 0) layout[n.prog[(size_t)pending * ISS_PROG_COLS + ISS_C_OUT]] = ChlState{};
            pending = -1;
            if (rc) return rc;
            if (ch.rows == 1 && env.layout_of(R[ISS_C_IN]).np && !ch.in_np)
                return iss_fail(c, ISS_EINVAL, "internal: row %d reads a CHL tensor on a kernel that expects f32", r);
            if (ch.rows == 2) {
                layout[R[ISS_C_OUT]] = ChlState{};
                R = &n.prog[(size_t)++r * ISS_PROG_COLS];
                out = (float*)c->act[R[ISS_C_OUT]].p;
            }
            if (ch.out != OutLayout::F32) out_layout = ChlState{ch.out_np, ch.out_f16, ch.out == OutLayout::ChlDense};
        } else if (op == ISS_OP_POOL) {
            const long long total = (long long)bc * R[ISS_C_HO] * R[ISS_C_WO] * R[ISS_C_CIN];
            iss_prof_begin(c, 2, 0);
            hipLaunchKernelGGL(pool_kernel, dim3((unsigned)((total + 255) / 256)), dim3(256), 0, c->stream, in, out,
                               total, R[ISS_C_H], R[ISS_C_W], R[ISS_C_CIN], R[ISS_C_HO], R[ISS_C_WO], R[ISS_C_KH],
                               R[ISS_C_KW], R[ISS_C_SH], R[ISS_C_SW], R[ISS_C_PT], R[ISS_C_PL], R[ISS_C_POOLKIND]);
            iss_prof_end(c);
        } else if (op == ISS_OP_SOFTMAX) {
            const long long rows = (long long)bc * R[ISS_C_H] * R[ISS_C_W];
            iss_prof_begin(c, 2, 0);
            hipLaunchKernelGGL(softmax_kernel, dim3((unsigned)((rows + 255) / 256)), dim3(256), 0, c->stream, in, out,
                               rows, R[ISS_C_CIN]);
            iss_prof_end(c);
        } else if (op == ISS_OP_ACT) {
            const long long total = (long long)bc * R[ISS_C_H] * R[ISS_C_W] * R[ISS_C_CIN];
            float alpha, p2, p3;
            { const int32_t bits = R[ISS_C_ACTPARAM]; memcpy(&alpha, &bits, sizeof(float)); }
            { const int32_t bits = R[ISS_C_ACTPARAM2]; memcpy(&p2, &bits, sizeof(float)); }
            { const int32_t bits = R[ISS_C_ACTPARAM3]; memcpy(&p3, &bits, sizeof(float)); }
            iss_prof_begin(c, 2, 0);
            hipLaunchKernelGGL(act_kernel, dim3((unsigned)std::min<long long>((total + 1023) / 1024, 1 << 20)), dim3(256), 0, c->stream, in, out, total,
                               R[ISS_C_ACT], alpha, p2, p3);
            iss_prof_end(c);
        } else if (op == ISS_OP_ELT) {
            const int k = R[ISS_C_ACT];
            const long long hw = (long long)R[ISS_C_H] * R[ISS_C_W];
            const bool chan = k == ISS_ELT_COPY || k == ISS_ELT_ZERO;
            const long long total = (long long)bc * hw * (chan ? R[ISS_C_KH] : R[ISS_C_CIN]);
            const float* res = R[ISS_C_RES] >= 0 ? (const float*)c->act[R[ISS_C_RES]].p : nullptr;
            if (res && layout[R[ISS_C_RES]].np) return iss_fail(c, ISS_EINVAL, "internal: row %d reads a CHL tensor", r);
            int st[3] = {0, 0, 0};
            if (k == ISS_ELT_PERMUTE) {
                const int sin[3] = {R[ISS_C_W] * R[ISS_C_CIN], R[ISS_C_CIN], 1};
                st[0] = sin[R[ISS_C_KH]]; st[1] = sin[R[ISS_C_KW]]; st[2] = sin[R[ISS_C_SH]];
            }
            iss_prof_begin(c, 2, 0);
            hipLaunchKernelGGL(elt_kernel, dim3((unsigned)std::min<long long>((total + 255) / 256, 1 << 20)), dim3(256), 0, c->stream, in, res, out,
                               total, k, R[ISS_C_CIN], R[ISS_C_COUT], R[ISS_C_KH], R[ISS_C_PT], R[ISS_C_PL],
                               R[ISS_C_HO], R[ISS_C_WO], R[ISS_C_COUT], st[0], st[1], st[2], R[ISS_C_ORDER] == 1 ? 1 : 0);
            iss_prof_end(c);
        } else if (op == ISS_OP_STATPOOL) {
            const long long total = (long long)bc * R[ISS_C_H] * R[ISS_C_CIN];
            iss_prof_begin(c, 2, 0);
            hipLaunchKernelGGL(statpool_kernel, dim3((unsigned)((total + 255) / 256)), dim3(256), 0, c->stream, in, out,
                               total, R[ISS_C_H], R[ISS_C_W], R[ISS_C_CIN]);
            iss_prof_end(c);
        }
        ISS_HIP(c, hipGetLastError());
        *result = out;
        layout[R[ISS_C_OUT]] = out_layout;
        if (op != ISS_OP_CONV && R[ISS_C_IN] != ISS_BUF_INPUT && layout[R[ISS_C_IN]].np)
            return iss_fail(c, ISS_EINVAL, "internal: row %d reads a CHL tensor", r);
    }
    return ISS_OK;
}

int plan_chunk(iss_ctx* c, IssNet& n, int total, int* bc_out) {
    int64_t per = 0;
    for (auto e : n.buf_elems) per += e;
    int64_t bc = (int64_t)(c->ws_limit / (uint64_t)(per * sizeof(float)));
    if (bc < 1) bc = 1;
    if (bc > total) bc = total;
    int64_t emax = 1;
    for (auto e : n.buf_elems) emax = std::max<int64_t>(emax, e);
    bc = std::min<int64_t>(bc, ((1ll << 31) - 1) / emax);
    if (bc < 1) return iss_fail(c, ISS_EINVAL, "network activation of %lld floats per sample exceeds the 2^31 element limit", (long long)emax);
    if (bc > 8) bc -= bc % 8;
    if ((int)c->act.size() < n.nbuf) c->act.resize(n.nbuf);
    for (int i = 0; i < n.nbuf; ++i) {
        int rc = iss_reserve(c, c->act[i], (size_t)bc * n.buf_elems[i] * sizeof(float) + issk::ISS_ACT_SLACK);
        if (rc) return rc;
    }
    *bc_out = (int)bc;
    return ISS_OK;
}

}

static int cnn_probs_impl(iss_ctx* c, int id, const int32_t* win_row, int32_t nslots, float* probs_out,
                          uint8_t* finite_out, bool async, int64_t* ticket_out);

static int precision_guard(iss_ctx* c, int id, const int32_t* win_row, int32_t nslots) {
    IssNet& n = c->nets[id];
    const int eff = effective_precision(c, n);
    if (eff == ISS_PREC_F32) { n.guard_state = ISS_GUARD_FIXED; return ISS_OK; }
    if (!(c->guard_threshold > 0.f)) return ISS_OK;
    const int runs = nslots >= 256 ? 4 : 1, per = nslots >= 256 ? 64 : nslots;
    const size_t od = (size_t)n.out_dim;
    std::vector<float> pref((size_t)runs * per * od), pm((size_t)per * od);
    std::vector<uint8_t> fref((size_t)runs * per), fm(per);
    auto window_run = [&](int r) { return win_row + (runs == 1 ? 0 : (size_t)r * (nslots - per) / (runs - 1)); };
    int rc = ISS_OK, compared = 0;
    auto probe = [&](int mode, double& worst) {
        worst = 0.0; compared = 0;
        for (int r = 0; r < runs && rc == ISS_OK; ++r) {
            n.prec_override = mode;
            rc = cnn_probs_impl(c, id, window_run(r), per, pm.data(), fm.data(), false, nullptr);
            if (rc != ISS_OK) return;
            for (int i = 0; i < per; ++i) {
                if (!fm[i] || !fref[(size_t)r * per + i]) continue;
                ++compared;
                for (size_t k = 0; k < od; ++k) {
                    const float a = pm[(size_t)i * od + k], b = pref[((size_t)r * per + i) * od + k];
                    if (!(a == a)) { worst = 1e30; continue; }
                    if (!(a > 1e-30f) || !(b > 1e-30f)) continue;
                    worst = std::max(worst, std::fabs(std::log((double)a) - std::log((double)b)));
                }
            }
        }
    };
    c->in_guard = true;
    for (int r = 0; r < runs && rc == ISS_OK; ++r) {
        n.prec_override = ISS_PREC_F32;
        rc = cnn_probs_impl(c, id, window_run(r), per, pref.data() + (size_t)r * per * od, fref.data() + (size_t)r * per, false, nullptr);
    }
    double worst = 0.0;
    int chosen = eff;
    if (rc == ISS_OK) probe(eff, worst);
    const double first = worst;
    if (rc == ISS_OK && worst > (double)c->guard_threshold) {
        chosen = ISS_PREC_F32;
        const int other = eff == ISS_PREC_BF16X3 ? ISS_PREC_F16X3 : ISS_PREC_BF16X3;
        if (other == ISS_PREC_BF16X3 || n.f16_ok) {
            double w2 = 0.0;
            probe(other, w2);
            if (rc == ISS_OK && w2 <= (double)c->guard_threshold) { chosen = other; worst = w2; }
        }
    }
    c->in_guard = false;
    n.prec_override = -1;
    if (rc != ISS_OK) return rc;
    if (compared == 0) { n.guard_slots = 0; return ISS_OK; }
    n.guard_dlogp = (float)std::min(first, 1e30); n.guard_slots = compared;
    n.guard_dlogp_chosen = chosen == eff ? n.guard_dlogp : (chosen == ISS_PREC_F32 ? 0.f : (float)worst);
    if (chosen != eff) { n.prec_override = chosen; n.guard_state = ISS_GUARD_ESCALATED; }
    else n.guard_state = ISS_GUARD_PASSED;
    return ISS_OK;
}

static int ensure_row_flags(iss_ctx* c) {
    if (c->flags_epoch == c->feat_epoch) return ISS_OK;
    int rc;
    if ((rc = iss_reserve(c, c->d_rowflag, (size_t)c->T))) return rc;
    if ((rc = iss_rowflag_host(c, (size_t)c->T))) return rc;
    iss_prof_begin(c, 2, 0);
    hipLaunchKernelGGL(row_flags_kernel, dim3((c->T + 255) / 256), dim3(256), 0, c->stream, (const float*)c->mspec.p, (int)c->T,
                       (uint8_t*)c->d_rowflag.p);
    iss_prof_end(c);
    ISS_HIP(c, hipGetLastError());
    ISS_HIP(c, hipMemcpyAsync(c->h_rowflag, c->d_rowflag.p, (size_t)c->T, hipMemcpyDeviceToHost, c->stream));
    ISS_HIP(c, hipStreamSynchronize(c->stream));
    c->bad_prefix.clear();
    c->flags_epoch = c->feat_epoch;
    return ISS_OK;
}

static const std::vector<int32_t>& bad_prefix(iss_ctx* c, int w) {
    std::vector<int32_t>& P = c->bad_prefix[w];
    if (P.size() != (size_t)c->T + 1) {
        P.resize((size_t)c->T + 1);
        P[0] = 0;
        for (int32_t t = 0; t < c->T; ++t) P[t + 1] = P[t] + (c->h_rowflag[t] < w ? 1 : 0);
    }
    return P;
}

extern "C" int iss_cnn_dead_stats(iss_ctx* c, int64_t* windows, int64_t* dead) {
    if (!c) return ISS_EINVAL;
    if (windows) *windows = c->win_total;
    if (dead) *dead = c->win_dead;
    return ISS_OK;
}

static int cnn_probs_impl(iss_ctx* c, int id, const int32_t* win_row, int32_t nslots, float* probs_out,
                          uint8_t* finite_out, bool async, int64_t* ticket_out) {
    if (!c) return ISS_EINVAL;
    if (ticket_out) *ticket_out = -1;
    if (id < 0 || id >= ISS_MAX_NETS || nslots < 0 || (nslots > 0 && (!win_row || !probs_out || !finite_out)))
        return iss_fail(c, ISS_EINVAL, "iss_cnn_probs: bad argument");
    IssNet& n = c->nets[id];
    if (!n.loaded) return iss_fail(c, ISS_ESTATE, "iss_cnn_probs: net %d not loaded", id);
    if (!c->have_feats) return iss_fail(c, ISS_ESTATE, "iss_cnn_probs: no mel spectrogram resident");
    if (n.in_h != 68 || n.in_c != 1 || n.in_w > 24) return iss_fail(c, ISS_EINVAL, "net %d is not a (68,h,1) patch network", id);
    if (nslots == 0) return ISS_OK;
    for (int i = 0; i < nslots; ++i)
        if (win_row[i] < 0 || win_row[i] + 68 > c->T)
            return iss_fail(c, ISS_EINVAL, "iss_cnn_probs: window %d (row %d) outside the %d resident frames", i, win_row[i], c->T);
    ISS_HIP(c, hipSetDevice(c->device));
    int rc;
    std::vector<int32_t> lm;
    int nlive = nslots;
    if (!(c->diag & ISS_DIAG_NO_SKIP_DEAD)) {
        if ((rc = ensure_row_flags(c))) return rc;
        const std::vector<int32_t>& P = bad_prefix(c, n.in_w);
        int dead = 0;
        for (int i = 0; i < nslots; ++i) dead += P[win_row[i] + 68] != P[win_row[i]];
        if (dead) {
            nlive = nslots - dead;
            lm.resize(2 * (size_t)nlive);
            for (int i = 0, j = 0; i < nslots; ++i)
                if (P[win_row[i] + 68] == P[win_row[i]]) { lm[j] = win_row[i]; lm[(size_t)nlive + j] = i; ++j; }
        }
        if (!c->in_guard) c->win_dead += dead;
    }
    if (!c->in_guard) c->win_total += nslots;
    const bool compact = nlive < nslots;
    const int32_t* rows = compact ? lm.data() : win_row;
    if (!c->in_guard && n.guard_state == ISS_GUARD_PENDING && nlive > 0 && (rc = precision_guard(c, id, rows, nlive))) return rc;
    const size_t nup = compact ? 2 * (size_t)nlive : (size_t)nslots;
    if ((rc = iss_reserve(c, c->d_winrow, (nup ? nup : 1) * 4))) return rc;
    if ((rc = iss_reserve(c, c->d_stats, (size_t)nslots * 8))) return rc;
    if ((rc = iss_reserve(c, c->d_finite, (size_t)nslots))) return rc;
    if (compact && (rc = iss_reserve(c, c->d_lfinite, (size_t)(nlive ? nlive : 1)))) return rc;
    if ((rc = iss_reserve(c, c->d_out, (size_t)nslots * n.out_dim * 4))) return rc;
    int bc = 0;
    if (nlive > 0 && (rc = plan_chunk(c, n, nlive, &bc))) return rc;
    if (nup == 0) {
    } else if (async || compact) {
        void* pinned; int slot;
        if ((rc = iss_stage_host(c, rows, nup * 4, &pinned, &slot))) return rc;
        ISS_HIP(c, hipMemcpyAsync(c->d_winrow.p, pinned, nup * 4, hipMemcpyHostToDevice, c->stream));
        iss_stage_mark(c, slot);
    } else {
        ISS_HIP(c, hipMemcpyAsync(c->d_winrow.p, win_row, (size_t)nslots * 4, hipMemcpyHostToDevice, c->stream));
    }
    const int32_t* d_map = (const int32_t*)c->d_winrow.p + nlive;
    uint8_t* d_fin = compact ? (uint8_t*)c->d_lfinite.p : (uint8_t*)c->d_finite.p;
    const long long tot = (long long)nslots * n.out_dim;
    if (compact) {
        iss_prof_begin(c, 2, 0);
        hipLaunchKernelGGL(fill_half_kernel, dim3((unsigned)((tot + 255) / 256)), dim3(256), 0, c->stream, (float*)c->d_out.p, tot);
        iss_prof_end(c);
        ISS_HIP(c, hipGetLastError());
        ISS_HIP(c, hipMemsetAsync(c->d_finite.p, 0, (size_t)nslots, c->stream));
    }
    if (nlive > 0) {
        iss_prof_begin(c, 2, 0);
        hipLaunchKernelGGL(patch_stats_kernel, dim3((nlive + 3) / 4), dim3(256), 0, c->stream, (const float*)c->mspec.p,
                           (const int32_t*)c->d_winrow.p, nlive, n.in_w, (float*)c->d_stats.p, d_fin);
        iss_prof_end(c);
        ISS_HIP(c, hipGetLastError());
    }
    bool share = !(c->diag & ISS_DIAG_NO_SHARED_FIRST);
    if (nlive > 0) {
        int gmin = rows[0], gmax = rows[0];
        for (int i = 1; i < nlive; ++i) { gmin = std::min(gmin, rows[i]); gmax = std::max(gmax, rows[i]); }
        if ((long long)(gmax - gmin + 68) * 4 > (long long)nlive * 68) share = false;
    }
    for (int s0 = 0; s0 < nlive; s0 += bc) {
        const int cur = std::min(bc, nlive - s0);
        float* res = nullptr;
        int rmin = rows[s0], rmax = rows[s0];
        for (int i = s0 + 1; i < s0 + cur; ++i) { rmin = std::min(rmin, rows[i]); rmax = std::max(rmax, rows[i]); }
        rc = run_program(c, n, cur, (const int32_t*)c->d_winrow.p + s0, (const float*)c->d_stats.p + 2 * (size_t)s0,
                         (const uint8_t*)d_fin + s0, nullptr, &res, rmin, rmax, share);
        if (rc) return rc;
        if (compact) {
            const long long ct = (long long)cur * n.out_dim;
            iss_prof_begin(c, 2, 0);
            hipLaunchKernelGGL(scatter_probs_kernel, dim3((unsigned)((ct + 255) / 256)), dim3(256), 0, c->stream, (const float*)res,
                               (const uint8_t*)d_fin + s0, d_map + s0, (long long)cur, n.out_dim, (float*)c->d_out.p, (uint8_t*)c->d_finite.p);
            iss_prof_end(c);
            ISS_HIP(c, hipGetLastError());
        } else {
            ISS_HIP(c, hipMemcpyAsync((float*)c->d_out.p + (size_t)s0 * n.out_dim, res, (size_t)cur * n.out_dim * 4,
                                      hipMemcpyDeviceToDevice, c->stream));
        }
    }
    if (!compact) {
        hipLaunchKernelGGL(mask_probs_kernel, dim3((unsigned)((tot + 255) / 256)), dim3(256), 0, c->stream,
                           (float*)c->d_out.p, (const uint8_t*)c->d_finite.p, (long long)nslots, n.out_dim);
        ISS_HIP(c, hipGetLastError());
    }
    ISS_HIP(c, hipMemcpyAsync(probs_out, c->d_out.p, (size_t)tot * 4, hipMemcpyDeviceToHost, c->stream));
    ISS_HIP(c, hipMemcpyAsync(finite_out, c->d_finite.p, (size_t)nslots, hipMemcpyDeviceToHost, c->stream));
    if (async) {
        hipEvent_t ev;
        if (!c->ev_pool.empty()) { ev = c->ev_pool.back(); c->ev_pool.pop_back(); }
        else ISS_HIP(c, hipEventCreate(&ev));
        ISS_HIP(c, hipEventRecord(ev, c->stream));
        c->ticket_ev.push_back(ev);
        if (ticket_out) *ticket_out = c->ticket_base + (int64_t)c->ticket_ev.size() - 1;
        return ISS_OK;
    }
    ISS_HIP(c, hipStreamSynchronize(c->stream));
    iss_prof_collect(c);
    return ISS_OK;
}

extern "C" int iss_cnn_probs(iss_ctx* c, int id, const int32_t* win_row, int32_t nslots, float* probs_out,
                             uint8_t* finite_out) {
    return cnn_probs_impl(c, id, win_row, nslots, probs_out, finite_out, false, nullptr);
}

extern "C" int iss_cnn_probs_async(iss_ctx* c, int id, const int32_t* win_row, int32_t nslots, float* probs_out,
                                   uint8_t* finite_out, int64_t* ticket_out) {
    return cnn_probs_impl(c, id, win_row, nslots, probs_out, finite_out, true, ticket_out);
}

extern "C" int iss_cnn_forward(iss_ctx* c, int id, const float* x, int32_t nsamp, float* out) {
    if (!c) return ISS_EINVAL;
    if (id < 0 || id >= ISS_MAX_NETS || nsamp < 0 || (nsamp > 0 && (!x || !out)))
        return iss_fail(c, ISS_EINVAL, "iss_cnn_forward: bad argument");
    IssNet& n = c->nets[id];
    if (!n.loaded) return iss_fail(c, ISS_ESTATE, "iss_cnn_forward: net %d not loaded", id);
    if (net_reads_patches(n)) return iss_fail(c, ISS_EINVAL, "iss_cnn_forward: net %d reads mspec patches; use iss_cnn_probs", id);
    if (nsamp == 0) return ISS_OK;
    ISS_HIP(c, hipSetDevice(c->device));
    const size_t in_elems = (size_t)n.in_h * n.in_w * n.in_c;
    int rc, bc = 0;
    if ((rc = plan_chunk(c, n, nsamp, &bc))) return rc;
    if ((rc = iss_reserve(c, c->d_in, (size_t)bc * in_elems * 4))) return rc;
    if ((rc = iss_reserve(c, c->d_out, (size_t)nsamp * n.out_dim * 4))) return rc;
    for (int s0 = 0; s0 < nsamp; s0 += bc) {
        const int cur = std::min(bc, nsamp - s0);
        ISS_HIP(c, hipMemcpyAsync(c->d_in.p, x + (size_t)s0 * in_elems, (size_t)cur * in_elems * 4, hipMemcpyHostToDevice, c->stream));
        float* res = nullptr;
        rc = run_program(c, n, cur, nullptr, nullptr, nullptr, (const float*)c->d_in.p, &res);
        if (rc) return rc;
        ISS_HIP(c, hipMemcpyAsync((float*)c->d_out.p + (size_t)s0 * n.out_dim, res, (size_t)cur * n.out_dim * 4,
                                  hipMemcpyDeviceToDevice, c->stream));
    }
    ISS_HIP(c, hipMemcpyAsync(out, c->d_out.p, (size_t)nsamp * n.out_dim * 4, hipMemcpyDeviceToHost, c->stream));
    ISS_HIP(c, hipStreamSynchronize(c->stream));
    iss_prof_collect(c);
    return ISS_OK;
}

extern "C" int iss_vbx_embed(iss_ctx* c, int id, const int32_t* starts, int32_t nwin, float* out) {
    if (!c) return ISS_EINVAL;
    if (id < 0 || id >= ISS_MAX_NETS || nwin < 0 || (nwin > 0 && (!starts || !out)))
        return iss_fail(c, ISS_EINVAL, "iss_vbx_embed: bad argument");
    IssNet& n = c->nets[id];
    if (!n.loaded) return iss_fail(c, ISS_ESTATE, "iss_vbx_embed: net %d not loaded", id);
    if (n.prog[ISS_C_OP] != ISS_OP_CONV || n.prog[ISS_C_INMODE] != 2)
        return iss_fail(c, ISS_EINVAL, "iss_vbx_embed: net %d does not start with a window-mode conv", id);
    if (c->vbx_T <= 0) return iss_fail(c, ISS_ESTATE, "iss_vbx_embed: no vbx features resident (iss_vbx_features*)");
    if (nwin == 0) return ISS_OK;
    for (int i = 0; i < nwin; ++i)
        if (starts[i] < 0 || starts[i] + n.in_w > c->vbx_T)
            return iss_fail(c, ISS_EINVAL, "iss_vbx_embed: window %d (frames %d..%d) outside the %d resident frames", i, starts[i],
                            starts[i] + n.in_w, c->vbx_T);
    ISS_HIP(c, hipSetDevice(c->device));
    int rc, bc = 0;
    if ((rc = iss_reserve(c, c->d_winrow, (size_t)nwin * 4))) return rc;
    if ((rc = iss_reserve(c, c->d_out, (size_t)nwin * n.out_dim * 4))) return rc;
    if ((rc = plan_chunk(c, n, nwin, &bc))) return rc;
    ISS_HIP(c, hipMemcpyAsync(c->d_winrow.p, starts, (size_t)nwin * 4, hipMemcpyHostToDevice, c->stream));
    for (int s0 = 0; s0 < nwin; s0 += bc) {
        const int cur = std::min(bc, nwin - s0);
        float* res = nullptr;
        rc = run_program(c, n, cur, (const int32_t*)c->d_winrow.p + s0, nullptr, nullptr, nullptr, &res);
        if (rc) return rc;
        ISS_HIP(c, hipMemcpyAsync((float*)c->d_out.p + (size_t)s0 * n.out_dim, res, (size_t)cur * n.out_dim * 4,
                                  hipMemcpyDeviceToDevice, c->stream));
    }
    ISS_HIP(c, hipMemcpyAsync(out, c->d_out.p, (size_t)nwin * n.out_dim * 4, hipMemcpyDeviceToHost, c->stream));
    ISS_HIP(c, hipStreamSynchronize(c->stream));
    iss_prof_collect(c);
    return ISS_OK;
}
```

### inaspeechsegmenter_amd/csrc/iss_core.cpp

```cpp
#include "iss_internal.h"
#include <cstring>
#include <cmath>
#include <mutex>

static std::string g_err;
static std::mutex g_err_mu;

int iss_fail(iss_ctx* c, int code, const char* fmt, ...) {
    char buf[1024];
    va_list ap;
    va_start(ap, fmt);
    vsnprintf(buf, sizeof(buf), fmt, ap);
    va_end(ap);
    if (c) c->err = buf;
    else { std::lock_guard<std::mutex> l(g_err_mu); g_err = buf; }
    return code;
}

int iss_reserve(iss_ctx* c, DevBuf& b, size_t bytes) {
    if (bytes <= b.cap) return ISS_OK;
    if (b.p) { ISS_HIP(c, hipStreamSynchronize(c->stream)); ISS_HIP(c, hipFree(b.p)); b.p = nullptr; b.cap = 0; }
    size_t want = bytes + (bytes >> 3) + 256;
    hipError_t e = hipMalloc(&b.p, want);
    if (e != hipSuccess) {
        b.p = nullptr;
        return iss_fail(c, ISS_ENOMEM, "hipMalloc(%zu) failed: %s", want, hipGetErrorString(e));
    }
    b.cap = want;
    return ISS_OK;
}

extern "C" const char* iss_version(void) { return "iss-hip 0.1 (gfx950)"; }

extern "C" const char* iss_last_error(const iss_ctx* c) {
    if (c) return c->err.c_str();
    std::lock_guard<std::mutex> l(g_err_mu);
    return g_err.c_str();
}

extern "C" int iss_create(int device_id, iss_ctx** out) {
    if (!out) return iss_fail(nullptr, ISS_EINVAL, "iss_create: out is NULL");
    *out = nullptr;
    int ndev = 0;
    hipError_t e = hipGetDeviceCount(&ndev);
    if (e != hipSuccess || ndev <= 0)
        return iss_fail(nullptr, ISS_ENODEV, "no HIP device visible (%s); this library has no CPU fallback",
                        e == hipSuccess ? "device count 0" : hipGetErrorString(e));
    if (device_id < 0 || device_id >= ndev)
        return iss_fail(nullptr, ISS_EINVAL, "device_id %d out of range [0,%d)", device_id, ndev);
    hipDeviceProp_t prop;
    e = hipGetDeviceProperties(&prop, device_id);
    if (e != hipSuccess) return iss_fail(nullptr, ISS_EHIP, "hipGetDeviceProperties: %s", hipGetErrorString(e));
    if (strncmp(prop.gcnArchName, "gfx950", 6) != 0)
        return iss_fail(nullptr, ISS_ENODEV, "device %d is %s; this library is built for gfx950 only",
                        device_id, prop.gcnArchName);
    iss_ctx* c = new iss_ctx();
    c->device = device_id;
    if (hipSetDevice(device_id) != hipSuccess ||
        hipStreamCreateWithFlags(&c->stream, hipStreamNonBlocking) != hipSuccess) {
        delete c;
        return iss_fail(nullptr, ISS_EHIP, "cannot create a stream on device %d", device_id);
    }
    *out = c;
    return ISS_OK;
}

static void free_buf(DevBuf& b) { if (b.p) (void)hipFree(b.p); b.p = nullptr; b.cap = 0; }

extern "C" void iss_destroy(iss_ctx* c) {
    if (!c) return;
    (void)hipSetDevice(c->device);
    if (c->stream) (void)hipStreamSynchronize(c->stream);
    for (int i = 0; i < ISS_MAX_NETS; ++i) iss_cnn_free(c, i);
    void* singles[] = {c->d_window, c->d_melw, c->d_mellim, c->d_tw, c->d_vbx_window, c->d_vbx_melw, c->d_vbx_mellim};
    for (void* p : singles) if (p) (void)hipFree(p);
    DevBuf* bufs[] = {&c->sig, &c->mspec, &c->loge, &c->d_winrow, &c->d_stats, &c->d_finite, &c->d_out, &c->d_in, &c->raw1, &c->d_rowflag, &c->d_lfinite,
                      &c->vbx_sig, &c->vbx_dither, &c->vbx_fb, &c->vbx_out, &c->vbx_meta, &c->rs_src, &c->rs_jobs,
                      &c->flac.src, &c->flac.rows, &c->flac.status, &c->flac.stage,
                      &c->adpcm.src, &c->adpcm.rows, &c->adpcm.status, &c->adpcm.stage};
    for (DevBuf* b : bufs) free_buf(*b);
    for (auto& b : c->act) free_buf(b);
    for (auto& f : c->rs_filters) if (f.d_taps) (void)hipFree(f.d_taps);
    for (auto& p : c->pending) { (void)hipEventDestroy(p.a); (void)hipEventDestroy(p.b); }
    for (auto& e : c->ev_pool) (void)hipEventDestroy(e);
    for (auto& e : c->ticket_ev) (void)hipEventDestroy(e);
    for (auto& s : c->staging) { if (s.p) (void)hipHostFree(s.p); if (s.done) (void)hipEventDestroy(s.done); }
    if (c->order_ev) (void)hipEventDestroy(c->order_ev);
    if (c->h_rowflag) (void)hipHostFree(c->h_rowflag);
    iss_comm_destroy(c);
    free_buf(c->comm_send); free_buf(c->comm_recv);
    if (c->stream) (void)hipStreamDestroy(c->stream);
    delete c;
}

extern "C" int iss_set_workspace_limit(iss_ctx* c, uint64_t bytes) {
    if (!c) return ISS_EINVAL;
    if (bytes < (64ull << 20)) return iss_fail(c, ISS_EINVAL, "workspace limit below 64 MiB");
    c->ws_limit = bytes;
    return ISS_OK;
}

extern "C" int iss_synchronize(iss_ctx* c) {
    if (!c) return ISS_EINVAL;
    ISS_HIP(c, hipSetDevice(c->device));
    ISS_HIP(c, hipStreamSynchronize(c->stream));
    return ISS_OK;
}

extern "C" int iss_scribble(iss_ctx* c, uint32_t word) {
    if (!c) return ISS_EINVAL;
    ISS_HIP(c, hipSetDevice(c->device));
    ISS_HIP(c, hipStreamSynchronize(c->stream));
    std::vector<DevBuf*> bufs = {&c->raw1, &c->d_stats, &c->d_finite, &c->d_lfinite, &c->d_out, &c->d_in, &c->d_winrow, &c->d_rowflag,
                                 &c->vbx_fb, &c->vbx_meta, &c->vbx_sig, &c->rs_src, &c->rs_jobs,
                                 &c->flac.src, &c->flac.rows, &c->flac.status, &c->flac.stage,
                                 &c->adpcm.src, &c->adpcm.rows, &c->adpcm.status, &c->adpcm.stage};
    for (auto& b : c->act) bufs.push_back(&b);
    for (DevBuf* b : bufs) {
        if (!b->p) continue;
        if (b->cap >= 4) ISS_HIP(c, hipMemsetD32Async((hipDeviceptr_t)b->p, (int)word, b->cap / 4, c->stream));
        for (size_t i = b->cap & ~(size_t)3; i < b->cap; ++i)
            ISS_HIP(c, hipMemsetD8Async((hipDeviceptr_t)((char*)b->p + i), (unsigned char)(word >> (8 * (i & 3))), 1, c->stream));
    }
    c->flags_epoch = 0;
    c->bad_prefix.clear();
    return ISS_OK;
}

extern "C" int iss_sidekit_tables(iss_ctx* c, const double* window400, const float* bank) {
    if (!c || !window400 || !bank) return iss_fail(c, ISS_EINVAL, "iss_sidekit_tables: NULL argument");
    ISS_HIP(c, hipSetDevice(c->device));
    std::vector<int32_t> lim(24 * 3);
    std::vector<float> w;
    for (int f = 0; f < 24; ++f) {
        int lo = -1, hi = -1;
        for (int k = 0; k < 257; ++k)
            if (bank[f * 257 + k] != 0.0f) { if (lo < 0) lo = k; hi = k; }
        if (lo < 0) { lo = 0; hi = -1; }
        if (hi >= 256) return iss_fail(c, ISS_EINVAL, "mel filter %d touches bin 256; unsupported table", f);
        lim[f * 3 + 0] = lo; lim[f * 3 + 1] = hi - lo + 1; lim[f * 3 + 2] = (int32_t)w.size();
        for (int k = lo; k <= hi; ++k) w.push_back(bank[f * 257 + k]);
    }
    if (w.size() > 1024) return iss_fail(c, ISS_EINVAL, "mel bank has %zu weights (>1024)", w.size());
    std::vector<double> tw(2 * 256 * 2);
    for (int k = 0; k < 256; ++k) {
        tw[2 * k] = cos(-2.0 * M_PI * k / 256.0);       tw[2 * k + 1] = sin(-2.0 * M_PI * k / 256.0);
        tw[512 + 2 * k] = cos(-2.0 * M_PI * k / 512.0); tw[512 + 2 * k + 1] = sin(-2.0 * M_PI * k / 512.0);
    }
    if (!c->d_window) ISS_HIP(c, hipMalloc((void**)&c->d_window, 400 * sizeof(double)));
    if (!c->d_melw) ISS_HIP(c, hipMalloc((void**)&c->d_melw, 1024 * sizeof(float)));
    if (!c->d_mellim) ISS_HIP(c, hipMalloc((void**)&c->d_mellim, 72 * sizeof(int32_t)));
    if (!c->d_tw) ISS_HIP(c, hipMalloc((void**)&c->d_tw, tw.size() * sizeof(double)));
    w.resize(1024, 0.0f);
    ISS_HIP(c, hipMemcpy(c->d_window, window400, 400 * sizeof(double), hipMemcpyHostToDevice));
    ISS_HIP(c, hipMemcpy(c->d_melw, w.data(), 1024 * sizeof(float), hipMemcpyHostToDevice));
    ISS_HIP(c, hipMemcpy(c->d_mellim, lim.data(), 72 * sizeof(int32_t), hipMemcpyHostToDevice));
    ISS_HIP(c, hipMemcpy(c->d_tw, tw.data(), tw.size() * sizeof(double), hipMemcpyHostToDevice));
    c->sk_tables = true;
    return ISS_OK;
}

void iss_set_signal(iss_ctx* c, const void* ptr, int kind, int64_t n) {
    c->sig_ptr = ptr; c->sig_kind = kind; c->sig_n = n;
    c->have_feats = false; ++c->feat_epoch;
}

static int put_signal(iss_ctx* c, const void* host, int64_t n, size_t esz, int kind) {
    if (!c || (!host && n > 0) || n < 0) return iss_fail(c, ISS_EINVAL, "iss_signal: bad argument");
    ISS_HIP(c, hipSetDevice(c->device));
    int rc = iss_reserve(c, c->sig, (size_t)n * esz + 16);
    if (rc) return rc;
    if (n > 0) ISS_HIP(c, hipMemcpyAsync(c->sig.p, host, (size_t)n * esz, hipMemcpyHostToDevice, c->stream));
    iss_set_signal(c, c->sig.p, kind, n);
    return ISS_OK;
}
extern "C" int iss_signal_pcm16(iss_ctx* c, const int16_t* pcm, int64_t n) { return put_signal(c, pcm, n, 2, 1); }
extern "C" int iss_signal_f32(iss_ctx* c, const float* sig, int64_t n) { return put_signal(c, sig, n, 4, 2); }
extern "C" int iss_signal_pcm16_device_stream(iss_ctx* c, const void* dev, int64_t n, void* producer_stream) {
    if (!c || (!dev && n > 0) || n < 0) return iss_fail(c, ISS_EINVAL, "iss_signal_pcm16_device: bad argument");
    ISS_HIP(c, hipSetDevice(c->device));
    if (n > 0) {
        hipPointerAttribute_t at;
        hipError_t e = hipPointerGetAttributes(&at, dev);
        if (e != hipSuccess) {
            (void)hipGetLastError();
            return iss_fail(c, ISS_EINVAL, "iss_signal_pcm16_device: %p is not a HIP allocation (%s)", dev, hipGetErrorString(e));
        }
        if (at.type != hipMemoryTypeDevice || at.device != c->device)
            return iss_fail(c, ISS_EINVAL, "iss_signal_pcm16_device: pointer belongs to %s %d, the context runs on device %d",
                            at.type == hipMemoryTypeDevice ? "device" : "host / managed memory of device", at.device, c->device);
    }
    if (!c->order_ev) ISS_HIP(c, hipEventCreateWithFlags(&c->order_ev, hipEventDisableTiming));
    ISS_HIP(c, hipEventRecord(c->order_ev, (hipStream_t)producer_stream));
    ISS_HIP(c, hipStreamWaitEvent(c->stream, c->order_ev, 0));
    iss_set_signal(c, dev, 1, n);
    return ISS_OK;
}
extern "C" int iss_signal_pcm16_device(iss_ctx* c, const void* dev, int64_t n) {
    return iss_signal_pcm16_device_stream(c, dev, n, nullptr);
}
extern "C" int iss_get_signal_pcm16(iss_ctx* c, int16_t* out, int64_t offset, int64_t n) {
    if (!c || (!out && n > 0) || offset < 0 || n < 0) return iss_fail(c, ISS_EINVAL, "iss_get_signal_pcm16: bad argument");
    if (c->sig_kind != 1) return iss_fail(c, ISS_ESTATE, "iss_get_signal_pcm16: no resident PCM16 signal");
    if (offset + n > c->sig_n)
        return iss_fail(c, ISS_EINVAL, "iss_get_signal_pcm16: [%lld, %lld) outside the %lld-sample signal", (long long)offset,
                        (long long)(offset + n), (long long)c->sig_n);
    ISS_HIP(c, hipSetDevice(c->device));
    if (n > 0) ISS_HIP(c, hipMemcpyAsync(out, (const int16_t*)c->sig_ptr + offset, (size_t)n * 2, hipMemcpyDeviceToHost, c->stream));
    ISS_HIP(c, hipStreamSynchronize(c->stream));
    return ISS_OK;
}

extern "C" int iss_host_alloc(iss_ctx* c, size_t bytes, void** out) {
    if (!c || !out) return iss_fail(c, ISS_EINVAL, "iss_host_alloc: NULL argument");
    *out = nullptr;
    ISS_HIP(c, hipSetDevice(c->device));
    hipError_t e = hipHostMalloc(out, bytes ? bytes : 1, hipHostMallocDefault);
    if (e != hipSuccess) { *out = nullptr; return iss_fail(c, ISS_ENOMEM, "hipHostMalloc(%zu) failed: %s", bytes, hipGetErrorString(e)); }
    return ISS_OK;
}
extern "C" int iss_host_free(iss_ctx* c, void* p) {
    if (!c) return ISS_EINVAL;
    if (!p) return ISS_OK;
    ISS_HIP(c, hipSetDevice(c->device));
    ISS_HIP(c, hipStreamSynchronize(c->stream));
    ISS_HIP(c, hipHostFree(p));
    return ISS_OK;
}

int iss_stage_host(iss_ctx* c, const void* src, size_t bytes, void** pinned_out, int* slot_out) {
    int slot = -1;
    for (size_t i = 0; i < c->staging.size(); ++i) {
        auto& s = c->staging[i];
        if (s.busy && hipEventQuery(s.done) == hipSuccess) s.busy = false;
        if (!s.busy && s.cap >= bytes && slot < 0) slot = (int)i;
    }
    if (slot < 0) {
        for (size_t i = 0; i < c->staging.size() && slot < 0; ++i)
            if (!c->staging[i].busy) slot = (int)i;
        if (slot < 0) { c->staging.emplace_back(); slot = (int)c->staging.size() - 1; }
        auto& s = c->staging[slot];
        if (s.p) { (void)hipHostFree(s.p); s.p = nullptr; s.cap = 0; }
        const size_t want = bytes + (bytes >> 2) + 4096;
        hipError_t e = hipHostMalloc(&s.p, want, hipHostMallocDefault);
        if (e != hipSuccess) { s.p = nullptr; return iss_fail(c, ISS_ENOMEM, "hipHostMalloc(%zu) failed: %s", want, hipGetErrorString(e)); }
        s.cap = want;
        if (!s.done) ISS_HIP(c, hipEventCreateWithFlags(&s.done, hipEventDisableTiming));
    }
    memcpy(c->staging[slot].p, src, bytes);
    *pinned_out = c->staging[slot].p;
    *slot_out = slot;
    return ISS_OK;
}
int iss_rowflag_host(iss_ctx* c, size_t rows) {
    if (rows <= c->h_rowflag_cap) return ISS_OK;
    if (c->h_rowflag) { ISS_HIP(c, hipStreamSynchronize(c->stream)); (void)hipHostFree(c->h_rowflag); c->h_rowflag = nullptr; c->h_rowflag_cap = 0; }
    const size_t want = rows + (rows >> 2) + 4096;
    hipError_t e = hipHostMalloc((void**)&c->h_rowflag, want, hipHostMallocDefault);
    if (e != hipSuccess) { c->h_rowflag = nullptr; return iss_fail(c, ISS_ENOMEM, "hipHostMalloc(%zu) failed: %s", want, hipGetErrorString(e)); }
    c->h_rowflag_cap = want;
    return ISS_OK;
}
void iss_stage_mark(iss_ctx* c, int slot) {
    auto& s = c->staging[slot];
    (void)hipEventRecord(s.done, c->stream);
    s.busy = true;
}

extern "C" int iss_wait(iss_ctx* c, int64_t ticket) {
    if (!c) return ISS_EINVAL;
    ISS_HIP(c, hipSetDevice(c->device));
    const int64_t last = c->ticket_base + (int64_t)c->ticket_ev.size() - 1;
    if (ticket < 0 || ticket >= last) {
        ISS_HIP(c, hipStreamSynchronize(c->stream));
        for (auto e : c->ticket_ev) c->ev_pool.push_back(e);
        c->ticket_base += (int64_t)c->ticket_ev.size();
        c->ticket_ev.clear();
        iss_prof_collect(c);
        return ISS_OK;
    }
    if (ticket < c->ticket_base) return ISS_OK;
    ISS_HIP(c, hipEventSynchronize(c->ticket_ev[(size_t)(ticket - c->ticket_base)]));
    return ISS_OK;
}

extern "C" int iss_sidekit(iss_ctx* c, int32_t* T_out) {
    if (!c) return ISS_EINVAL;
    if (!c->sk_tables) return iss_fail(c, ISS_ESTATE, "iss_sidekit: call iss_sidekit_tables first");
    if (c->sig_kind == 0) return iss_fail(c, ISS_ESTATE, "iss_sidekit: no resident signal");
    ISS_HIP(c, hipSetDevice(c->device));
    int64_t n = c->sig_n;
    int64_t T = n >= 400 ? (n - 400) / 160 + 1 : 0;
    if (T > 0x7fffffffLL / 24) return iss_fail(c, ISS_EINVAL, "signal too long (%lld frames)", (long long)T);
    c->T = (int32_t)T;
    int rc = iss_reserve(c, c->mspec, (size_t)(T > 0 ? T : 1) * 24 * sizeof(float));
    if (rc) return rc;
    rc = iss_reserve(c, c->loge, (size_t)(T > 0 ? T : 1) * sizeof(float));
    if (rc) return rc;
    if (T > 0) { rc = iss_launch_sidekit(c); if (rc) return rc; }
    c->have_feats = true; ++c->feat_epoch;
    if (T_out) *T_out = (int32_t)T;
    return ISS_OK;
}

extern "C" int iss_get_loge(iss_ctx* c, float* out) {
    if (!c || !out) return iss_fail(c, ISS_EINVAL, "iss_get_loge: NULL");
    if (!c->have_feats) return iss_fail(c, ISS_ESTATE, "iss_get_loge: no features resident");
    ISS_HIP(c, hipSetDevice(c->device));
    if (c->T > 0) ISS_HIP(c, hipMemcpyAsync(out, c->loge.p, (size_t)c->T * sizeof(float), hipMemcpyDeviceToHost, c->stream));
    ISS_HIP(c, hipStreamSynchronize(c->stream));
    iss_prof_collect(c);
    return ISS_OK;
}

extern "C" int iss_get_mspec(iss_ctx* c, float* out) {
    if (!c || !out) return iss_fail(c, ISS_EINVAL, "iss_get_mspec: NULL");
    if (!c->have_feats) return iss_fail(c, ISS_ESTATE, "iss_get_mspec: no features resident");
    ISS_HIP(c, hipSetDevice(c->device));
    if (c->T > 0) ISS_HIP(c, hipMemcpyAsync(out, c->mspec.p, (size_t)c->T * 24 * sizeof(float), hipMemcpyDeviceToHost, c->stream));
    ISS_HIP(c, hipStreamSynchronize(c->stream));
    iss_prof_collect(c);
    return ISS_OK;
}

extern "C" int iss_set_mspec(iss_ctx* c, const float* mspec, int32_t T) {
    if (!c || !mspec || T <= 0) return iss_fail(c, ISS_EINVAL, "iss_set_mspec: bad argument");
    ISS_HIP(c, hipSetDevice(c->device));
    int rc = iss_reserve(c, c->mspec, (size_t)T * 24 * sizeof(float));
    if (rc) return rc;
    ISS_HIP(c, hipMemcpyAsync(c->mspec.p, mspec, (size_t)T * 24 * sizeof(float), hipMemcpyHostToDevice, c->stream));
    ISS_HIP(c, hipStreamSynchronize(c->stream));
    c->T = T; c->have_feats = true; ++c->feat_epoch;
    if ((rc = iss_rowflag_host(c, (size_t)T))) return rc;
    for (int32_t t = 0; t < T; ++t) c->h_rowflag[t] = (uint8_t)iss_row_flag(mspec + (size_t)t * 24);
    c->bad_prefix.clear();
    c->flags_epoch = c->feat_epoch;
    return ISS_OK;
}

static hipEvent_t get_event(iss_ctx* c) {
    if (!c->ev_pool.empty()) { hipEvent_t e = c->ev_pool.back(); c->ev_pool.pop_back(); return e; }
    hipEvent_t e; (void)hipEventCreate(&e); return e;
}
void iss_prof_begin(iss_ctx* c, int kind, double flops) {
    if (!c->prof) return;
    iss_ctx::Pending p; p.a = get_event(c); p.b = get_event(c); p.kind = kind; p.sub = -1; p.row = -1; p.flops = flops;
    (void)hipEventRecord(p.a, c->stream);
    c->pending.push_back(p);
}
void iss_prof_tag(iss_ctx* c, int sub) {
    if (!c->prof || c->pending.empty() || sub < 0 || sub >= ISS_PROF_KINDS) return;
    c->pending.back().sub = sub;
}
void iss_prof_row(iss_ctx* c, int row) {
    if (!c->prof || c->pending.empty() || row < 0 || row >= ISS_PROF_ROWS) return;
    c->pending.back().row = row;
}
void iss_prof_inst(iss_ctx* c, const char* fmt, ...) {
    if (!c->prof || c->pending.empty()) return;
    char buf[160];
    va_list ap;
    va_start(ap, fmt);
    vsnprintf(buf, sizeof(buf), fmt, ap);
    va_end(ap);
    c->pending.back().inst = buf;
}
void iss_prof_end(iss_ctx* c) {
    if (!c->prof || c->pending.empty()) return;
    (void)hipEventRecord(c->pending.back().b, c->stream);
}
void iss_prof_collect(iss_ctx* c) {
    for (auto& p : c->pending) {
        float ms = 0;
        if (hipEventElapsedTime(&ms, p.a, p.b) == hipSuccess) {
            c->prof_ms[p.kind] += ms; c->prof_launch[p.kind] += 1; c->prof_flops[p.kind] += p.flops;
            if (p.sub >= 0) { c->prof_ms[p.sub] += ms; c->prof_launch[p.sub] += 1; c->prof_flops[p.sub] += p.flops; }
            if (p.row >= 0) { c->prof_row_ms[p.row] += ms; c->prof_row_launch[p.row] += 1; }
            if (!p.inst.empty()) {
                iss_ctx::Inst* e = nullptr;
                for (auto& i : c->prof_inst) if (i.name == p.inst) { e = &i; break; }
                if (!e) { c->prof_inst.emplace_back(); e = &c->prof_inst.back(); e->name = p.inst; }
                e->ms += ms; e->launches += 1; e->flops += p.flops;
            }
        }
        c->ev_pool.push_back(p.a); c->ev_pool.push_back(p.b);
    }
    c->pending.clear();
}
extern "C" int iss_prof_enable(iss_ctx* c, int on) { if (!c) return ISS_EINVAL; c->prof = on != 0; return ISS_OK; }
extern "C" int iss_prof_reset(iss_ctx* c) {
    if (!c) return ISS_EINVAL;
    ISS_HIP(c, hipStreamSynchronize(c->stream));
    iss_prof_collect(c);
    for (int i = 0; i < ISS_PROF_KINDS; ++i) { c->prof_ms[i] = 0; c->prof_launch[i] = 0; c->prof_flops[i] = 0; }
    for (int i = 0; i < ISS_PROF_ROWS; ++i) { c->prof_row_ms[i] = 0; c->prof_row_launch[i] = 0; }
    c->prof_inst.clear();
    return ISS_OK;
}
extern "C" int iss_prof_get_instance(iss_ctx* c, int index, char* name_out, int32_t name_len, double* ms, int64_t* launches, double* flops) {
    if (!c || index < 0) return ISS_EINVAL;
    ISS_HIP(c, hipStreamSynchronize(c->stream));
    iss_prof_collect(c);
    if (index >= (int)c->prof_inst.size()) return ISS_EINVAL;
    const iss_ctx::Inst& e = c->prof_inst[(size_t)index];
    if (name_out && name_len > 0) { snprintf(name_out, (size_t)name_len, "%s", e.name.c_str()); }
    if (ms) *ms = e.ms;
    if (launches) *launches = e.launches;
    if (flops) *flops = e.flops;
    return ISS_OK;
}
extern "C" int iss_prof_get_row(iss_ctx* c, int row, double* ms, int64_t* launches) {
    if (!c || row < 0 || row >= ISS_PROF_ROWS) return ISS_EINVAL;
    ISS_HIP(c, hipStreamSynchronize(c->stream));
    iss_prof_collect(c);
    if (ms) *ms = c->prof_row_ms[row];
    if (launches) *launches = c->prof_row_launch[row];
    return ISS_OK;
}
extern "C" int iss_prof_get(iss_ctx* c, int kind, double* ms, int64_t* launches, double* flops) {
    if (!c || kind < 0 || kind >= ISS_PROF_KINDS) return ISS_EINVAL;
    ISS_HIP(c, hipStreamSynchronize(c->stream));
    iss_prof_collect(c);
    if (ms) *ms = c->prof_ms[kind];
    if (launches) *launches = c->prof_launch[kind];
    if (flops) *flops = c->prof_flops[kind];
    return ISS_OK;
}
```

### inaspeechsegmenter_amd/csrc/iss_internal.h

```cpp
#pragma once
#include <hip/hip_runtime.h>
#include <array>
#include <cstdint>
#include <cstdio>
#include <cstdarg>
#include <string>
#include <vector>
#include <unordered_map>
#include <map>
#include <memory>
#include "../../include/iss.h"

struct DevBuf {
    void* p = nullptr;
    size_t cap = 0;
};

struct ConvOp;

struct IssCounters { int64_t launches = 0, units = 0; };
struct IssCodec {
    const char* name;
    DevBuf src, rows, status, stage;
    std::vector<int64_t> stage_off, stage_bytes;
    IssCounters count;
};

struct IssParamArrays {
    float* blob = nullptr;
    uint16_t *wh = nullptr, *wl = nullptr, *wh16 = nullptr, *wl16 = nullptr;
    ~IssParamArrays();
};

struct IssNet {
    bool loaded = false;
    std::vector<int32_t> prog;
    int nrows = 0;
    float* d_blob = nullptr;
    uint16_t* d_wh = nullptr;
    uint16_t* d_wl = nullptr;
    uint16_t* d_wh16 = nullptr;
    uint16_t* d_wl16 = nullptr;
    bool f16_ok = false;
    std::shared_ptr<IssParamArrays> shared_params;
    std::map<std::pair<int, int>, uint16_t*> dhl_wp;
    float* d_wsum = nullptr;
    std::vector<int64_t> wsum_off;
    std::vector<int64_t> wsumx_off;
    int64_t blob_floats = 0;
    std::vector<int64_t> w_dev_off;
    std::vector<int32_t> kpad;
    int32_t* d_ktab = nullptr;
    std::vector<int64_t> ktab_off;
    int nbuf = 0;
    std::vector<int64_t> buf_elems;
    int in_h = 0, in_w = 0, in_c = 0, out_dim = 0;
    double flops_per_sample = 0;
    std::map<std::array<int, 4>, int> fp_pix;
    int prec_override = -1;
    bool prec_by_caller = false;
    int guard_state = 0;
    float guard_dlogp = -1.f;
    float guard_dlogp_chosen = -1.f;
    int guard_slots = 0;
};

struct iss_ctx {
    int device = -1;
    hipStream_t stream = nullptr;
    std::string err;

    bool sk_tables = false;
    double* d_window = nullptr;
    float* d_melw = nullptr;
    int32_t* d_mellim = nullptr;
    double* d_tw = nullptr;

    DevBuf sig;
    const void* sig_ptr = nullptr;
    int sig_kind = 0;
    int64_t sig_n = 0;

    struct RsFilter { int32_t up = 1, down = 1, hl = 0; int64_t ntaps = 1; double* d_taps = nullptr; };
    std::vector<RsFilter> rs_filters;
    std::map<std::pair<int32_t, int32_t>, int32_t> rs_filter_id;
    DevBuf rs_src, rs_jobs;
    IssCounters rs_count;

    IssCodec flac{"flac"}, adpcm{"adpcm"};

    DevBuf mspec, loge;
    int32_t T = 0;
    bool have_feats = false;
    uint64_t feat_epoch = 1;

    uint64_t flags_epoch = 0;
    DevBuf d_rowflag;
    uint8_t* h_rowflag = nullptr;
    size_t h_rowflag_cap = 0;
    std::map<int, std::vector<int32_t>> bad_prefix;
    DevBuf d_lfinite;
    int64_t win_total = 0, win_dead = 0;

    IssNet nets[ISS_MAX_NETS];
    uint64_t ws_limit = 24ull << 30;
    int precision = ISS_PREC_F16X3;
    float guard_threshold = 5e-4f;
    bool in_guard = false;
    uint32_t diag = 0;
    std::vector<DevBuf> act;
    DevBuf d_winrow, d_stats, d_finite, d_out, d_in;
    DevBuf raw1;

    bool vbx_tables = false;
    double* d_vbx_window = nullptr;
    double* d_vbx_melw = nullptr;
    int32_t* d_vbx_mellim = nullptr;
    DevBuf vbx_sig, vbx_dither, vbx_fb, vbx_out;
    DevBuf vbx_meta;
    int32_t vbx_T = 0;
    int64_t vbx_dither_n = 0;

    struct Staging { void* p = nullptr; size_t cap = 0; hipEvent_t done = nullptr; bool busy = false; };
    std::vector<Staging> staging;
    std::vector<hipEvent_t> ticket_ev;
    int64_t ticket_base = 1;
    hipEvent_t order_ev = nullptr;

    void* comm = nullptr;
    int comm_rank = 0, comm_world = 1;
    DevBuf comm_send, comm_recv;

    bool prof = false;
    double prof_ms[ISS_PROF_KINDS] = {};
    int64_t prof_launch[ISS_PROF_KINDS] = {};
    double prof_flops[ISS_PROF_KINDS] = {};
    double prof_row_ms[ISS_PROF_ROWS] = {};
    int64_t prof_row_launch[ISS_PROF_ROWS] = {};
    struct Pending { hipEvent_t a, b; int kind; int sub; int row; double flops; std::string inst; };
    std::vector<Pending> pending;
    struct Inst { std::string name; double ms = 0; int64_t launches = 0; double flops = 0; };
    std::vector<Inst> prof_inst;
    std::vector<hipEvent_t> ev_pool;
};

int iss_fail(iss_ctx* c, int code, const char* fmt, ...);
int iss_reserve(iss_ctx* c, DevBuf& b, size_t bytes);
void iss_set_signal(iss_ctx* c, const void* ptr, int kind, int64_t n);
int iss_stage_host(iss_ctx* c, const void* src, size_t bytes, void** pinned_out, int* slot_out);
void iss_stage_mark(iss_ctx* c, int slot);
int iss_rowflag_host(iss_ctx* c, size_t rows);

__host__ __device__ inline int iss_row_flag(const float* row) {
    for (int k = 0; k < 24; ++k) {
        const float v = row[k];
        if (!(v - v == 0.f)) return k;
    }
    return 24;
}

#define ISS_HIP(c, call)                                                                  \
    do {                                                                                  \
        hipError_t e__ = (call);                                                          \
        if (e__ != hipSuccess)                                                            \
            return iss_fail((c), ISS_EHIP, "%s failed: %s (%s:%d)", #call,                \
                            hipGetErrorString(e__), __FILE__, __LINE__);                  \
    } while (0)

void iss_prof_begin(iss_ctx* c, int kind, double flops);
void iss_prof_tag(iss_ctx* c, int sub);
void iss_prof_row(iss_ctx* c, int row);
void iss_prof_inst(iss_ctx* c, const char* fmt, ...);
void iss_prof_end(iss_ctx* c);
void iss_prof_collect(iss_ctx* c);

struct RsJobDev {
    int64_t src_off, n_in, dst_off, n_out, tile_base;
    const double* taps;
    int32_t ch, fmt, up, down, hl, tile, lds_tab, pad;
};
struct IssRsPlan {
    std::vector<RsJobDev> dj;
    int64_t tiles = 0, lds = 0;
};
int iss_resample_plan(iss_ctx* c, const iss_resample_job* jobs, int32_t njobs, int64_t src_bytes, int64_t nsig,
                      std::vector<std::pair<int64_t, int64_t>> ranges, const char* who, IssRsPlan& plan);
int iss_resample_launch(iss_ctx* c, const uint8_t* dev_src, const IssRsPlan& plan);

int iss_launch_sidekit(iss_ctx* c);
int iss_cnn_free(iss_ctx* c, int net_id);
```

### include/iss.h

```cpp
#ifndef ISS_H
#define ISS_H

#include <stdint.h>
#include <stddef.h>

#ifdef __cplusplus
extern "C" {
#endif

#define ISS_OK        0
#define ISS_EINVAL   -1
#define ISS_ENODEV   -2
#define ISS_EHIP     -3
#define ISS_ESTATE   -4
#define ISS_ENOMEM   -5
#define ISS_ETIMEOUT -6

typedef struct iss_ctx iss_ctx;

int         iss_create(int device_id, iss_ctx** out);
void        iss_destroy(iss_ctx* ctx);
const char* iss_last_error(const iss_ctx* ctx);
const char* iss_version(void);
int         iss_set_workspace_limit(iss_ctx* ctx, uint64_t bytes);
int         iss_synchronize(iss_ctx* ctx);


int iss_sidekit_tables(iss_ctx* ctx, const double* window400, const float* melbank_24x257);

int iss_signal_pcm16(iss_ctx* ctx, const int16_t* pcm, int64_t n);
int iss_signal_f32(iss_ctx* ctx, const float* sig, int64_t n);
int iss_signal_pcm16_device(iss_ctx* ctx, const void* dev_pcm, int64_t n);
int iss_signal_pcm16_device_stream(iss_ctx* ctx, const void* dev_pcm, int64_t n, void* producer_stream);

#define ISS_RS_U8   0
#define ISS_RS_I16  1
#define ISS_RS_I32  2
#define ISS_RS_F32  3
#define ISS_RS_F64  4
#define ISS_RS_I8   8
#define ISS_RS_ULAW 9
#define ISS_RS_ALAW 10
#define ISS_RS_SWAP 0x100
typedef struct {
    int64_t src_offset;
    int64_t frames_in;
    int32_t channels;
    int32_t format;
    int32_t filter;
    int32_t reserved;
    int64_t dst_offset;
    int64_t frames_out;
} iss_resample_job;
int iss_resample_filter(iss_ctx* ctx, int32_t up, int32_t down, const double* taps, int64_t ntaps, int32_t* id_out);
int iss_resample_pcm16(iss_ctx* ctx, const void* src, int64_t src_bytes, const iss_resample_job* jobs, int32_t njobs,
                       int64_t n_signal);
int iss_get_signal_pcm16(iss_ctx* ctx, int16_t* out, int64_t offset, int64_t n);
int iss_resample_stats(iss_ctx* ctx, int64_t* launches, int64_t* jobs);

typedef struct {
    int32_t sample_rate, channels, bps;
    int32_t min_block, max_block;
    int32_t reserved;
    int64_t total_samples;
} iss_flac_info;
typedef struct {
    int64_t offset;
    int64_t length;
    int64_t first_sample;
    int32_t block_size;
    int32_t channel_mode;
    int32_t bps;
    int32_t header_bytes;
} iss_flac_frame;
int iss_flac_index(const uint8_t* buf, int64_t len, int64_t first_frame, const iss_flac_info* info, iss_flac_frame* frames,
                   int64_t cap, int64_t* nframes, int64_t* err_offset, char* err, int32_t err_len);
int iss_flac_crc(const uint8_t* buf, int64_t n, int32_t* crc8_out, int32_t* crc16_out);
#define ISS_FLAC_OK               0
#define ISS_FLAC_SUBFRAME_TYPE    1
#define ISS_FLAC_PAD_BIT          2
#define ISS_FLAC_WASTED           3
#define ISS_FLAC_RESIDUAL_METHOD  4
#define ISS_FLAC_PARTITION        5
#define ISS_FLAC_LPC_PRECISION    6
#define ISS_FLAC_LPC_SHIFT        7
#define ISS_FLAC_OVERRUN          8
#define ISS_FLAC_PADDING          9
#define ISS_FLAC_FOOTER          10
#define ISS_FLAC_CRC16           11
int iss_flac_decode_host(const uint8_t* buf, int64_t len, const iss_flac_frame* frames, int64_t nframes, int32_t channels,
                         int32_t bps, int64_t frames_total, void* out, int32_t* status_out);
#define ISS_FLAC_TO_SIGNAL  0
#define ISS_FLAC_TO_STAGE   1
typedef struct {
    int64_t src_offset;
    int64_t frame_begin;
    int64_t nframes;
    int64_t frames_total;
    int32_t channels;
    int32_t bps;
    int32_t output;
    int32_t filter;
    int64_t dst_offset;
    int64_t frames_out;
} iss_flac_job;
int iss_flac_decode(iss_ctx* ctx, const void* src, int64_t src_bytes, const iss_flac_frame* frames, int64_t nframes,
                    const iss_flac_job* jobs, int32_t njobs, int64_t n_signal, int32_t* status_out);
int iss_flac_get_stage(iss_ctx* ctx, int32_t job, void* out, int64_t bytes);
int iss_flac_stats(iss_ctx* ctx, int64_t* launches, int64_t* frames);

#define ISS_ADPCM_OK          0
#define ISS_ADPCM_STEP_INDEX  1
#define ISS_ADPCM_TO_SIGNAL   0
#define ISS_ADPCM_TO_STAGE    1
typedef struct {
    int64_t src_offset;
    int64_t block_begin;
    int64_t nblocks;
    int64_t frames_total;
    int32_t channels;
    int32_t block_align;
    int32_t output;
    int32_t filter;
    int64_t dst_offset;
    int64_t frames_out;
} iss_adpcm_job;
int iss_adpcm_decode_host(const uint8_t* buf, int64_t len, int64_t nblocks, int32_t channels, int32_t block_align,
                          int64_t frames_total, int16_t* out, int32_t* status_out);
int iss_adpcm_decode(iss_ctx* ctx, const void* src, int64_t src_bytes, const iss_adpcm_job* jobs, int32_t njobs,
                     int64_t nblocks_total, int64_t n_signal, int32_t* status_out);
int iss_adpcm_get_stage(iss_ctx* ctx, int32_t job, void* out, int64_t bytes);
int iss_adpcm_stats(iss_ctx* ctx, int64_t* launches, int64_t* blocks);

int iss_host_alloc(iss_ctx* ctx, size_t bytes, void** out);
int iss_host_free(iss_ctx* ctx, void* p);

int iss_sidekit(iss_ctx* ctx, int32_t* T_out);
int iss_get_loge(iss_ctx* ctx, float* loge_out );
int iss_get_mspec(iss_ctx* ctx, float* mspec_out );
int iss_set_mspec(iss_ctx* ctx, const float* mspec, int32_t T);

#define ISS_MAX_NETS   8
#define ISS_PROG_COLS  32

enum {
    ISS_OP_CONV     = 1,
    ISS_OP_POOL     = 2,
    ISS_OP_SOFTMAX  = 3,
    ISS_OP_STATPOOL = 4,
    ISS_OP_ACT      = 5,
    ISS_OP_ELT      = 6,
};
enum { ISS_ELT_COPY = 0, ISS_ELT_ADD = 1, ISS_ELT_SUB = 2, ISS_ELT_MUL = 3, ISS_ELT_MAX = 4, ISS_ELT_MIN = 5, ISS_ELT_AVG = 6,
       ISS_ELT_ZERO = 7, ISS_ELT_PERMUTE = 8 };
enum {
    ISS_C_OP = 0, ISS_C_IN, ISS_C_OUT, ISS_C_RES,
    ISS_C_H, ISS_C_W, ISS_C_CIN, ISS_C_HO, ISS_C_WO, ISS_C_COUT,
    ISS_C_KH, ISS_C_KW, ISS_C_SH, ISS_C_SW, ISS_C_PT, ISS_C_PL,
    ISS_C_ACT,
    ISS_C_WOFF, ISS_C_BOFF,
    ISS_C_PSOFF, ISS_C_PTOFF,
    ISS_C_INMODE,
    ISS_C_POOLKIND,
    ISS_C_ORDER,
    ISS_C_FPOOLH, ISS_C_FPOOLW,
    ISS_C_DUALW, ISS_C_DUALB,
    ISS_C_ACTPARAM,
    ISS_C_ACTPARAM2, ISS_C_ACTPARAM3,
};
#define ISS_BUF_INPUT  (-2)

int iss_cnn_load(iss_ctx* ctx, int net_id, const int32_t* prog, int32_t nrows,
                 const float* blob, int64_t blob_floats,
                 int32_t nbuf, const int64_t* buf_elems,
                 int32_t in_h, int32_t in_w, int32_t in_c, int32_t out_dim);
int iss_cnn_load_shared(iss_ctx* ctx, int net_id, int src_id, const int32_t* prog, int32_t nrows,
                        int32_t nbuf, const int64_t* buf_elems,
                        int32_t in_h, int32_t in_w, int32_t in_c, int32_t out_dim);

int iss_cnn_probs(iss_ctx* ctx, int net_id, const int32_t* win_row, int32_t n,
                  float* probs_out , uint8_t* finite_out );

int iss_cnn_probs_async(iss_ctx* ctx, int net_id, const int32_t* win_row, int32_t n,
                        float* probs_out , uint8_t* finite_out , int64_t* ticket_out);
int iss_cnn_dead_stats(iss_ctx* ctx, int64_t* windows, int64_t* dead);
int iss_wait(iss_ctx* ctx, int64_t ticket);

int iss_cnn_forward(iss_ctx* ctx, int net_id, const float* x, int32_t n, float* out );

#define ISS_PREC_BF16X3 0
#define ISS_PREC_F32    1
#define ISS_PREC_F16X3  2
int iss_set_precision(iss_ctx* ctx, int mode);

#define ISS_GUARD_PENDING   0
#define ISS_GUARD_PASSED    1
#define ISS_GUARD_ESCALATED 2
#define ISS_GUARD_FIXED     3
int iss_set_precision_guard(iss_ctx* ctx, float threshold);
int iss_cnn_precision_info(iss_ctx* ctx, int id, int32_t* mode, float* max_dlogp, int32_t* slots, int32_t* state, float* dlogp_in_use);
int iss_cnn_set_net_precision(iss_ctx* ctx, int id, int mode);

#define ISS_DIAG_NO_SHARED_FIRST 0x001u
#define ISS_DIAG_NO_FLROWS       0x002u
#define ISS_DIAG_NO_WS           0x004u
#define ISS_DIAG_NO_WS3          0x008u
#define ISS_DIAG_NO_DIRECT1      0x010u
#define ISS_DIAG_NO_NH2          0x020u
#define ISS_DIAG_NO_TR           0x040u
#define ISS_DIAG_NO_PW           0x080u
#define ISS_DIAG_NO_PWS          0x100u
#define ISS_DIAG_NO_PWS2         0x200u
#define ISS_DIAG_NO_WQ           0x400u
#define ISS_DIAG_NO_DUAL         0x800u
#define ISS_DIAG_NO_CHAIN        0x1000u
#define ISS_DIAG_NO_RING         0x2000u
#define ISS_DIAG_NO_FSAME        0x4000u
#define ISS_DIAG_NO_F32WS        0x8000u
#define ISS_DIAG_NO_NCB1         0x10000u
#define ISS_DIAG_NO_WSU3         0x20000u
#define ISS_DIAG_NO_GFUSED       0x40000u
#define ISS_DIAG_NO_HL           0x80000u
#define ISS_DIAG_NO_SKIP_DEAD    0x100000u
#define ISS_DIAG_ALL             0x1fffffu
int iss_set_diag(iss_ctx* ctx, uint32_t flags);

int iss_cnn_flops(iss_ctx* ctx, int net_id, double* flops_per_sample);

int iss_vbx_tables(iss_ctx* ctx, const double* window400, const double* melbank_257x64);
int iss_vbx_features(iss_ctx* ctx, const int32_t* sig_i32, const double* dither_u, int64_t n,
                     float* fea_out , int32_t* T_out);
int iss_vbx_set_dither(iss_ctx* ctx, const double* dither_u, int64_t n);
int iss_vbx_features_pcm16(iss_ctx* ctx, const int16_t* pcm, int64_t n,
                           float* fea_out , int32_t* T_out);
int iss_vbx_features_batch_pcm16(iss_ctx* ctx, const int16_t* pcm, const int64_t* sample_off, int32_t nfiles,
                                 int32_t* frame_off_out, float* fea_out );
int iss_vbx_embed(iss_ctx* ctx, int net_id, const int32_t* starts, int32_t n, float* out );

#define ISS_COMM_ID_BYTES 128
int iss_comm_unique_id(iss_ctx* ctx, uint8_t id_out[ISS_COMM_ID_BYTES]);
int iss_comm_init(iss_ctx* ctx, const uint8_t id[ISS_COMM_ID_BYTES], int32_t rank, int32_t world);
int iss_comm_destroy(iss_ctx* ctx);
int iss_allgather_segments(iss_ctx* ctx, const int32_t* local_rows, int32_t n_local, int32_t capacity,
                           int32_t* all_rows, int32_t* counts );
int iss_comm_allreduce_max(iss_ctx* ctx, double* value);
int iss_comm_info(iss_ctx* ctx, int32_t* world, int32_t* rank, int32_t* version, char* lib_path, int32_t lib_path_len);

#define ISS_PROF_GEMM      0
#define ISS_PROF_FRONTEND  1
#define ISS_PROF_OTHER     2
#define ISS_PROF_WS        3
#define ISS_PROF_FP        4
#define ISS_PROF_PW        5
#define ISS_PROF_GATHER    6
#define ISS_PROF_PATCH1    7
#define ISS_PROF_F32       8
#define ISS_PROF_KINDS     9
int iss_prof_enable(iss_ctx* ctx, int on);
int iss_prof_get(iss_ctx* ctx, int kind, double* ms, int64_t* launches, double* flops);
int iss_prof_reset(iss_ctx* ctx);
#define ISS_PROF_ROWS      512
int iss_prof_get_row(iss_ctx* ctx, int row, double* ms, int64_t* launches);
int iss_prof_get_instance(iss_ctx* ctx, int index, char* name_out, int32_t name_len, double* ms, int64_t* launches, double* flops);

int iss_scribble(iss_ctx* ctx, uint32_t word);

int iss_viterbi_f64(const double* emission, int64_t T, int32_t K, const double* transition,
                    int32_t* states_out);
int iss_viterbi_f32(const float* emission, int64_t T, int32_t K, const double* transition,
                    int32_t* states_out);
int iss_viterbi_segments_f32(const float* emission, const int64_t* seg_len, int64_t nseg, int32_t K,
                             const double* transition, int32_t* states_out);
int iss_energy_viterbi(const float* loge, int64_t T, double threshold, double log_eps, double log_1m_eps,
                       const double* transition, int32_t* states_out);

#ifdef __cplusplus
}
#endif
#endif
```

Before: 6.977.

## Run CNN passes on two concurrent stream lanes with per-lane activation buffers

Introduces IssLane structs, each with its own HIP stream, activation buffers and first-layer scratch, and threads a lane through conv argument setup and kernel launches. With two lanes enabled by default, independent CNN batch chunks can run concurrently on separate streams and overlap small, underfilled kernels. The cost is duplicated activation memory, extra cross-stream synchronisation in buffer reallocation and teardown, and a synchronisation added after lazy weight packing. Profiling events now record on the stream of each lane.

```diff
diff --git a/inaspeechsegmenter_amd/_native.py b/inaspeechsegmenter_amd/_native.py
--- a/inaspeechsegmenter_amd/_native.py
+++ b/inaspeechsegmenter_amd/_native.py
@@ -122,6 +122,7 @@
         'iss_prof_get_row': (C.c_int, [vp, C.c_int, pd, pi64]),
         'iss_prof_get_instance': (C.c_int, [vp, C.c_int, C.c_char_p, i32, pd, pi64, pd]),
         'iss_set_diag': (C.c_int, [vp, C.c_uint32]),
+        'iss_set_lanes': (C.c_int, [vp, C.c_int]),
         'iss_scribble': (C.c_int, [vp, C.c_uint32]),
         'iss_viterbi_f64': (C.c_int, [pd, i64, i32, pd, pi32]),
         'iss_viterbi_f32': (C.c_int, [pf, i64, i32, pd, pi32]),
@@ -270,8 +271,12 @@
         self.workspace_limit = None
         self.diag = 0
         env = os.environ.get('ISS_DIAG', '')
+        self.lanes = 2
         if env:
-            self.set_diag(diag_flags(env))
+            names = [nm for nm in env.replace(' ', '').replace('+', ',').lower().split(',') if nm]
+            if 'no_lanes' in names:
+                self.set_lanes(1)
+            self.set_diag(diag_flags(','.join(nm for nm in names if nm != 'no_lanes')))
         self.guard_threshold = None
         env = os.environ.get('ISS_PREC_GUARD', '')
         if env:
@@ -568,6 +573,12 @@
             self.set_diag(other.diag)
         if getattr(other, 'guard_threshold', None) is not None and other.guard_threshold != getattr(self, 'guard_threshold', None):
             self.set_precision_guard(other.guard_threshold)
+        if getattr(other, 'lanes', 2) != getattr(self, 'lanes', 2):
+            self.set_lanes(other.lanes)
+
+    def set_lanes(self, lanes):
+        self._ck(self._L.iss_set_lanes(self._h, int(lanes)), 'iss_set_lanes')
+        self.lanes = int(lanes)
 
     def set_diag(self, flags):
         flags = diag_flags(flags) if isinstance(flags, str) else int(flags)
diff --git a/inaspeechsegmenter_amd/csrc/cnn.hip b/inaspeechsegmenter_amd/csrc/cnn.hip
--- a/inaspeechsegmenter_amd/csrc/cnn.hip
+++ b/inaspeechsegmenter_amd/csrc/cnn.hip
@@ -1244,18 +1244,18 @@
 
 struct PassIo { const int32_t* d_winrow; const float* d_stats; const uint8_t* d_fin; const float* d_input; };
 
-int conv_args(iss_ctx* c, IssNet& n, const PassIo& io, int bc, const ConvChoice& ch, ConvArgs& a) {
+int conv_args(iss_ctx* c, IssLane& L, IssNet& n, const PassIo& io, int bc, const ConvChoice& ch, ConvArgs& a) {
     const int r = ch.row;
     const int32_t* R = &n.prog[(size_t)r * ISS_PROG_COLS];
     memset(&a, 0, sizeof(a));
     fill_geometry(a, R, bc);
-    a.in = R[ISS_C_IN] == ISS_BUF_INPUT ? io.d_input : (const float*)c->act[R[ISS_C_IN]].p;
+    a.in = R[ISS_C_IN] == ISS_BUF_INPUT ? io.d_input : (const float*)L.act[R[ISS_C_IN]].p;
     a.w = n.d_blob + R[ISS_C_WOFF];
     a.bias = R[ISS_C_BOFF] >= 0 ? n.d_blob + R[ISS_C_BOFF] : nullptr;
     a.ps = R[ISS_C_PSOFF] >= 0 ? n.d_blob + R[ISS_C_PSOFF] : nullptr;
     a.pt = R[ISS_C_PTOFF] >= 0 ? n.d_blob + R[ISS_C_PTOFF] : nullptr;
-    a.res = R[ISS_C_RES] >= 0 ? (const float*)c->act[R[ISS_C_RES]].p : nullptr;
-    a.out = (float*)c->act[R[ISS_C_OUT]].p;
+    a.res = R[ISS_C_RES] >= 0 ? (const float*)L.act[R[ISS_C_RES]].p : nullptr;
+    a.out = (float*)L.act[R[ISS_C_OUT]].p;
     a.ktab = n.d_ktab + n.ktab_off[r];
     a.wh = n.d_wh + R[ISS_C_WOFF]; a.wl = n.d_wl + R[ISS_C_WOFF];
     a.Kpad = n.kpad[r]; a.mode = ch.mode; a.tmr = ch.tmr;
@@ -1277,11 +1277,11 @@
         const int32_t* Q = &n.prog[(size_t)ch.partner * ISS_PROG_COLS];
         a.wh2 = n.d_wh + Q[ISS_C_WOFF]; a.wl2 = n.d_wl + Q[ISS_C_WOFF];
         a.bias2 = Q[ISS_C_BOFF] >= 0 ? n.d_blob + Q[ISS_C_BOFF] : nullptr;
-        a.out2 = (float*)c->act[Q[ISS_C_OUT]].p;
+        a.out2 = (float*)L.act[Q[ISS_C_OUT]].p;
         a.act2 = Q[ISS_C_ACT]; a.Cout2 = Q[ISS_C_COUT];
     } else if (ch.kernel == ConvKernel::Pws2Dual) {
         const int32_t* P = &n.prog[(size_t)ch.partner * ISS_PROG_COLS];
-        a.in2 = P[ISS_C_IN] == ISS_BUF_INPUT ? io.d_input : (const float*)c->act[P[ISS_C_IN]].p;
+        a.in2 = P[ISS_C_IN] == ISS_BUF_INPUT ? io.d_input : (const float*)L.act[P[ISS_C_IN]].p;
         a.Cin2 = P[ISS_C_CIN]; a.H2 = P[ISS_C_H]; a.W2 = P[ISS_C_W]; a.sh2 = P[ISS_C_SH]; a.sw2 = P[ISS_C_SW];
         const int64_t wo = (int64_t)R[ISS_C_DUALW] - 1;
         a.w = n.d_blob + wo; a.wh = n.d_wh + wo; a.wl = n.d_wl + wo;
@@ -1294,7 +1294,7 @@
     return ISS_OK;
 }
 
-int launch_shared_first_layer(iss_ctx* c, IssNet& n, const PassIo& io, int pend, int bc, int rmin, int rmax, ConvArgs& a, double* fl) {
+int launch_shared_first_layer(iss_ctx* c, IssLane& L, IssNet& n, const PassIo& io, int pend, int bc, int rmin, int rmax, ConvArgs& a, double* fl) {
     const int32_t* R1 = &n.prog[(size_t)pend * ISS_PROG_COLS];
     const bool fs1 = R1[ISS_C_HO] == R1[ISS_C_H];
     int ph1, pw1;
@@ -1306,20 +1306,20 @@
     const long long etot = (long long)bc * f_ne * R1[ISS_C_WO] * (R1[ISS_C_COUT] / 4);
     const int plane_rows = pool1 ? (int)(rrows / ph1) + 2 : 0;
     const long long ptot = pool1 ? (long long)ph1 * plane_rows * (R1[ISS_C_WO] / pw1) * (R1[ISS_C_COUT] / 4) : 0;
-    { const int rc = iss_reserve(c, c->raw1, (size_t)(rtot + etot + ptot) * 16 + (pool1 ? (size_t)bc * 4 + 16 : 0)); if (rc) return rc; }
-    float* Rraw = (float*)c->raw1.p;
+    { const int rc = iss_reserve(c, L.raw1, (size_t)(rtot + etot + ptot) * 16 + (pool1 ? (size_t)bc * 4 + 16 : 0)); if (rc) return rc; }
+    float* Rraw = (float*)L.raw1.p;
     const float* mspec = (const float*)c->mspec.p;
     const float* w1 = n.d_blob + R1[ISS_C_WOFF];
     const size_t lds1 = (size_t)R1[ISS_C_KH] * R1[ISS_C_KW] * R1[ISS_C_COUT] * 4;
-    iss_prof_begin(c, 2, 0);
+    iss_prof_begin(c, 2, 0, &L);
     if (fs1) {
         const int pt1 = R1[ISS_C_PT], pl1 = R1[ISS_C_PL], pb1 = R1[ISS_C_KH] - 1 - pt1;
         const float* S = n.d_wsum + n.wsumx_off[pend];
         if (rtot >= (1ll << 31) || etot >= (1ll << 31)) return iss_fail(c, ISS_EINVAL, "internal: shared first layer over %lld + %lld items", rtot, etot);
-        hipLaunchKernelGGL(first_layer_same_kernel, dim3((unsigned)std::min<long long>((rtot + 255) / 256, 4096)), dim3(256), lds1, c->stream,
+        hipLaunchKernelGGL(first_layer_same_kernel, dim3((unsigned)std::min<long long>((rtot + 255) / 256, 4096)), dim3(256), lds1, L.stream,
                            mspec, (int)c->T, rmin, rtot, R1[ISS_C_WO], R1[ISS_C_COUT], R1[ISS_C_KH], R1[ISS_C_KW], pt1, pl1, w1, n.kpad[pend], Rraw);
         if (etot > 0)
-            hipLaunchKernelGGL(first_layer_edge_kernel, dim3((unsigned)std::min<long long>((etot + 255) / 256, 8192)), dim3(256), lds1, c->stream,
+            hipLaunchKernelGGL(first_layer_edge_kernel, dim3((unsigned)std::min<long long>((etot + 255) / 256, 8192)), dim3(256), lds1, L.stream,
                                mspec, io.d_winrow, io.d_stats, etot, R1[ISS_C_H], R1[ISS_C_WO], R1[ISS_C_COUT], R1[ISS_C_KH],
                                R1[ISS_C_KW], pt1, pb1, pl1, w1, n.kpad[pend], S, Rraw + (size_t)rtot * 4);
         a.f_padt = pt1; a.f_padb = pb1; a.f_erow0 = (int)rrows;
@@ -1330,13 +1330,13 @@
                              rrows * (R1[ISS_C_COUT] / 4) < (1ll << 31);
         const dim3 rowgrid((unsigned)std::min<long long>((rrows * (R1[ISS_C_COUT] / 4) + 255) / 256, 4096));
         if (rows_ok && R1[ISS_C_WO] == 17)
-            hipLaunchKernelGGL((first_layer_rows_kernel<4, 5, 17>), rowgrid, dim3(256), lds1, c->stream, mspec, rmin, (int)rrows, R1[ISS_C_COUT], w1, n.kpad[pend], Rraw);
+            hipLaunchKernelGGL((first_layer_rows_kernel<4, 5, 17>), rowgrid, dim3(256), lds1, L.stream, mspec, rmin, (int)rrows, R1[ISS_C_COUT], w1, n.kpad[pend], Rraw);
         else if (rows_ok)
-            hipLaunchKernelGGL((first_layer_rows_kernel<4, 5, 20>), rowgrid, dim3(256), lds1, c->stream, mspec, rmin, (int)rrows, R1[ISS_C_COUT], w1, n.kpad[pend], Rraw);
+            hipLaunchKernelGGL((first_layer_rows_kernel<4, 5, 20>), rowgrid, dim3(256), lds1, L.stream, mspec, rmin, (int)rrows, R1[ISS_C_COUT], w1, n.kpad[pend], Rraw);
         else if (R1[ISS_C_KH] == 4 && R1[ISS_C_KW] == 5)
-            hipLaunchKernelGGL((first_layer_raw_kernel<4, 5>), rgrid, dim3(256), lds1, c->stream, mspec, rmin, rtot, R1[ISS_C_WO], R1[ISS_C_COUT], 4, 5, w1, n.kpad[pend], Rraw);
+            hipLaunchKernelGGL((first_layer_raw_kernel<4, 5>), rgrid, dim3(256), lds1, L.stream, mspec, rmin, rtot, R1[ISS_C_WO], R1[ISS_C_COUT], 4, 5, w1, n.kpad[pend], Rraw);
         else
-            hipLaunchKernelGGL((first_layer_raw_kernel<0, 0>), rgrid, dim3(256), lds1, c->stream, mspec, rmin, rtot, R1[ISS_C_WO], R1[ISS_C_COUT],
+            hipLaunchKernelGGL((first_layer_raw_kernel<0, 0>), rgrid, dim3(256), lds1, L.stream, mspec, rmin, rtot, R1[ISS_C_WO], R1[ISS_C_COUT],
                                R1[ISS_C_KH], R1[ISS_C_KW], w1, n.kpad[pend], Rraw);
     }
     a.in = Rraw; a.win_row = io.d_winrow; a.f_rmin = rmin;
@@ -1344,9 +1344,9 @@
         if (ptot >= (1ll << 40)) return iss_fail(c, ISS_EINVAL, "internal: pooled first layer over %lld items", ptot);
         float* P = Rraw + (size_t)(rtot + etot) * 4;
         int32_t* wr2 = reinterpret_cast<int32_t*>(P + (size_t)ptot * 4);
-        hipLaunchKernelGGL(pool_rows_kernel, dim3((unsigned)std::min<long long>((ptot + 255) / 256, 8192)), dim3(256), 0, c->stream,
+        hipLaunchKernelGGL(pool_rows_kernel, dim3((unsigned)std::min<long long>((ptot + 255) / 256, 8192)), dim3(256), 0, L.stream,
                            (const float*)Rraw, P, ptot, (int)rrows, R1[ISS_C_WO], R1[ISS_C_COUT], ph1, pw1, plane_rows);
-        hipLaunchKernelGGL(winrow_pool_kernel, dim3((unsigned)((bc + 255) / 256)), dim3(256), 0, c->stream, io.d_winrow, wr2, bc, rmin, ph1, plane_rows);
+        hipLaunchKernelGGL(winrow_pool_kernel, dim3((unsigned)((bc + 255) / 256)), dim3(256), 0, L.stream, io.d_winrow, wr2, bc, rmin, ph1, plane_rows);
         a.in = P; a.win_row = wr2; a.f_rmin = 0;
     }
     iss_prof_end(c);
@@ -1360,7 +1360,7 @@
     return ISS_OK;
 }
 
-int launch_conv(iss_ctx* c, IssNet& n, const ConvChoice& ch, ConvArgs& a, double fl) {
+int launch_conv(iss_ctx* c, IssLane& L, IssNet& n, const ConvChoice& ch, ConvArgs& a, double fl) {
     const int r = ch.row;
     const int32_t* R = &n.prog[(size_t)r * ISS_PROG_COLS];
     const bool padded = ch.padded, tr = ch.tr, fused = ch.fused;
@@ -1370,7 +1370,7 @@
     const unsigned tiles = (unsigned)((a.M + WS_TM - 1) / WS_TM);
     const unsigned groups = (unsigned)((a.M + (long long)WS_TM * WS_G - 1) / ((long long)WS_TM * WS_G));
     const unsigned qtiles = ch.tmr > 0 ? (unsigned)((a.M + ch.tmr - 1) / ch.tmr) : 0;
-    iss_prof_begin(c, 0, fl);
+    iss_prof_begin(c, 0, fl, &L);
     iss_prof_tag(c, ch.tag), iss_prof_row(c, r), iss_prof_inst(c, "%s", inst_name(ch).c_str());
     switch (ch.kernel) {
     case ConvKernel::Dhl: {
@@ -1378,102 +1378,103 @@
         uint16_t*& wp = n.dhl_wp[{r, ch.f16 ? 1 : 0}];
         if (!wp) {
             ISS_HIP(c, hipMalloc((void**)&wp, dhl_packed_elems(K, R[ISS_C_COUT]) * 2));
-            iss_dhl_pack((ch.f16 ? n.d_wh16 : n.d_wh) + R[ISS_C_WOFF], (ch.f16 ? n.d_wl16 : n.d_wl) + R[ISS_C_WOFF], wp, R[ISS_C_COUT], n.kpad[r], K, c->stream);
+            iss_dhl_pack((ch.f16 ? n.d_wh16 : n.d_wh) + R[ISS_C_WOFF], (ch.f16 ? n.d_wl16 : n.d_wl) + R[ISS_C_WOFF], wp, R[ISS_C_COUT], n.kpad[r], K, L.stream);
+            ISS_HIP(c, hipStreamSynchronize(L.stream));
         }
         DhlArgs d;
         d.a = reinterpret_cast<const uint16_t*>(a.in); d.wp = wp; d.bias = a.bias; d.out = a.out;
         d.np = ch.in_np; d.M = (int)a.M; d.K = K; d.Cout = R[ISS_C_COUT]; d.act = R[ISS_C_ACT];
-        iss_dhl_launch(d, c->stream, ch.f16);
+        iss_dhl_launch(d, L.stream, ch.f16);
         break;
     }
-    case ConvKernel::Pwc: iss_pwc_launch(a, c->stream); break;
-    case ConvKernel::Pws2Dual: iss_pws2_launch(a, c->stream, false, true); break;
+    case ConvKernel::Pwc: iss_pwc_launch(a, L.stream); break;
+    case ConvKernel::Pws2Dual: iss_pws2_launch(a, L.stream, false, true); break;
     case ConvKernel::Direct1: {
         const long long items = (long long)(a.M / ((long long)a.H * a.W)) * ((a.H + 7) / 8) * a.W * (a.Cout / 4);
         if (items >= (1ll << 32)) return iss_fail(c, ISS_EINVAL, "internal: direct first layer over %lld work items", items);
         const dim3 dgrid((unsigned)std::min<long long>((items + 255) / 256, 8192));
         const size_t dlds = (size_t)9 * a.Cout * sizeof(float);
-        if (ch.window) hipLaunchKernelGGL(conv1_direct3x3_kernel<true>, dgrid, dim3(256), dlds, c->stream, a);
-        else hipLaunchKernelGGL(conv1_direct3x3_kernel<false>, dgrid, dim3(256), dlds, c->stream, a);
+        if (ch.window) hipLaunchKernelGGL(conv1_direct3x3_kernel<true>, dgrid, dim3(256), dlds, L.stream, a);
+        else hipLaunchKernelGGL(conv1_direct3x3_kernel<false>, dgrid, dim3(256), dlds, L.stream, a);
         break;
     }
-    case ConvKernel::WsNh2F32: iss_ws_launch_f32_nh2_3x3(a, dim3(std::min<unsigned>(tiles, std::max(1u, 256u / ny)), ny), c->stream, tr); break;
+    case ConvKernel::WsNh2F32: iss_ws_launch_f32_nh2_3x3(a, dim3(std::min<unsigned>(tiles, std::max(1u, 256u / ny)), ny), L.stream, tr); break;
     case ConvKernel::WsNh2: {
         const dim3 g2(std::min<unsigned>(tiles, std::max(1u, 256u / ny)), ny);
-        if (padded && !tr) iss_ws_launch_nh2_3x3_padded_pool(a, g2, c->stream);
-        else if (padded) iss_ws_launch_nh2_3x3_padded(a, g2, c->stream);
-        else iss_ws_launch_nh2_3x3(a, g2, c->stream, tr);
+        if (padded && !tr) iss_ws_launch_nh2_3x3_padded_pool(a, g2, L.stream);
+        else if (padded) iss_ws_launch_nh2_3x3_padded(a, g2, L.stream);
+        else iss_ws_launch_nh2_3x3(a, g2, L.stream, tr);
         break;
     }
     case ConvKernel::Wq3: case ConvKernel::Wq3h: {
         const dim3 qgrid(std::min<unsigned>((qtiles + 1) / 2, std::max(1u, 256u / ny)), ny);
-        if (ch.kernel == ConvKernel::Wq3h) iss_wq3h_launch(a, qgrid, c->stream, ch.kind);
-        else iss_wq3_launch(a, qgrid, c->stream, ch.kind);
+        if (ch.kernel == ConvKernel::Wq3h) iss_wq3h_launch(a, qgrid, L.stream, ch.kind);
+        else iss_wq3_launch(a, qgrid, L.stream, ch.kind);
         break;
     }
-    case ConvKernel::WsPlainU: iss_ws_launch_plain_3x3_unpadded(a, dim3(std::min<unsigned>(groups, std::max(1u, 256u / grid.y)), grid.y), c->stream, tr); break;
-    case ConvKernel::WsPlain: iss_ws_launch_plain_3x3(a, dim3(std::min<unsigned>(groups, std::max(1u, 256u / grid.y)), grid.y), c->stream); break;
-    case ConvKernel::WsF32Fused: iss_ws_launch_f32_fused_5x3(a, dim3(std::min<unsigned>(groups, 256u), grid.y), c->stream); break;
-    case ConvKernel::WsRing: iss_ws_launch_ring(a, dim3(std::min<unsigned>(qtiles, 256u), grid.y), c->stream, padded); break;
+    case ConvKernel::WsPlainU: iss_ws_launch_plain_3x3_unpadded(a, dim3(std::min<unsigned>(groups, std::max(1u, 256u / grid.y)), grid.y), L.stream, tr); break;
+    case ConvKernel::WsPlain: iss_ws_launch_plain_3x3(a, dim3(std::min<unsigned>(groups, std::max(1u, 256u / grid.y)), grid.y), L.stream); break;
+    case ConvKernel::WsF32Fused: iss_ws_launch_f32_fused_5x3(a, dim3(std::min<unsigned>(groups, 256u), grid.y), L.stream); break;
+    case ConvKernel::WsRing: iss_ws_launch_ring(a, dim3(std::min<unsigned>(qtiles, 256u), grid.y), L.stream, padded); break;
     case ConvKernel::WsFs: {
         const dim3 wgrid(std::min<unsigned>(tiles, 256u), grid.y);
-        if (tr) iss_ws_launch_fs_5x3_tr(a, wgrid, c->stream);
-        else if (a.H_k == 5) iss_ws_launch_fs_5x3(a, wgrid, c->stream, padded);
-        else iss_ws_launch_fs_3x3(a, wgrid, c->stream, padded);
+        if (tr) iss_ws_launch_fs_5x3_tr(a, wgrid, L.stream);
+        else if (a.H_k == 5) iss_ws_launch_fs_5x3(a, wgrid, L.stream, padded);
+        else iss_ws_launch_fs_3x3(a, wgrid, L.stream, padded);
         break;
     }
-    case ConvKernel::WsNcb1: iss_ws_launch_ncb1_5x3(a, dim3(std::min<unsigned>(groups, 256u), grid.y), c->stream); break;
-    case ConvKernel::Wq: iss_wq_launch_5x3(a, dim3(std::min<unsigned>((qtiles + 1) / 2, 256u), grid.y), c->stream); break;
+    case ConvKernel::WsNcb1: iss_ws_launch_ncb1_5x3(a, dim3(std::min<unsigned>(groups, 256u), grid.y), L.stream); break;
+    case ConvKernel::Wq: iss_wq_launch_5x3(a, dim3(std::min<unsigned>((qtiles + 1) / 2, 256u), grid.y), L.stream); break;
     case ConvKernel::Ws: {
         const dim3 wgrid(std::min<unsigned>(groups, 256u), grid.y);
-#define ISS_WS_CASE(KH_, KW_) if (a.H_k == KH_ && a.kw == KW_) iss_ws_launch_##KH_##x##KW_(a, wgrid, c->stream, padded, tr, fused); else
+#define ISS_WS_CASE(KH_, KW_) if (a.H_k == KH_ && a.kw == KW_) iss_ws_launch_##KH_##x##KW_(a, wgrid, L.stream, padded, tr, fused); else
         ISS_WS_SHAPES(ISS_WS_CASE) { return iss_fail(c, ISS_EINVAL, "internal: no weight-stationary kernel for %dx%d", a.H_k, a.kw); }
 #undef ISS_WS_CASE
         break;
     }
     case ConvKernel::Fp: {
         const dim3 pgrid(std::min<unsigned>(a.nblk, 512u), grid.y / nh);
-#define ISS_FP_CASE(KH_, KW_) if (a.H_k == KH_ && a.kw == KW_) iss_fp_launch_##KH_##x##KW_(a, pgrid, c->stream, padded, tr, fused, nh); else
+#define ISS_FP_CASE(KH_, KW_) if (a.H_k == KH_ && a.kw == KW_) iss_fp_launch_##KH_##x##KW_(a, pgrid, L.stream, padded, tr, fused, nh); else
         ISS_FP_SHAPES(ISS_FP_CASE) { return iss_fail(c, ISS_EINVAL, "internal: no footprint kernel for %dx%d", a.H_k, a.kw); }
 #undef ISS_FP_CASE
         break;
     }
     case ConvKernel::Patch1: {
         const dim3 pgrid(std::min<unsigned>(a.nblk, 512u), grid.y);
-        if (tr && ch.f16) hipLaunchKernelGGL((conv1_patch_x3_kernel<true, true>), pgrid, dim3(256), 0, c->stream, a);
-        else if (tr) hipLaunchKernelGGL((conv1_patch_x3_kernel<true, false>), pgrid, dim3(256), 0, c->stream, a);
-        else if (ch.f16) hipLaunchKernelGGL((conv1_patch_x3_kernel<false, true>), pgrid, dim3(256), 0, c->stream, a);
-        else hipLaunchKernelGGL((conv1_patch_x3_kernel<false, false>), pgrid, dim3(256), 0, c->stream, a);
+        if (tr && ch.f16) hipLaunchKernelGGL((conv1_patch_x3_kernel<true, true>), pgrid, dim3(256), 0, L.stream, a);
+        else if (tr) hipLaunchKernelGGL((conv1_patch_x3_kernel<true, false>), pgrid, dim3(256), 0, L.stream, a);
+        else if (ch.f16) hipLaunchKernelGGL((conv1_patch_x3_kernel<false, true>), pgrid, dim3(256), 0, L.stream, a);
+        else hipLaunchKernelGGL((conv1_patch_x3_kernel<false, false>), pgrid, dim3(256), 0, L.stream, a);
         break;
     }
     case ConvKernel::Gather: case ConvKernel::X3: {
         constexpr int ntn = 2;
         a.nblk_n = (unsigned)((a.Cout + 32 * ntn - 1) / (32 * ntn));
         const dim3 gridw(a.nblk * a.nblk_n);
-        if (a.mode == 4 && tr) hipLaunchKernelGGL((conv_x3_kernel<4, true, 2>), gridw, dim3(256), 0, c->stream, a);
-        else if (a.mode == 4) hipLaunchKernelGGL((conv_x3_kernel<4, false, 2>), gridw, dim3(256), 0, c->stream, a);
-        else if (a.mode == 3 && tr) hipLaunchKernelGGL((conv_x3_kernel<3, true, 2>), gridw, dim3(256), 0, c->stream, a);
-        else if (a.mode == 3) hipLaunchKernelGGL((conv_x3_kernel<3, false, 2>), gridw, dim3(256), 0, c->stream, a);
-        else if (a.mode == 0 && tr) hipLaunchKernelGGL((conv_x3_kernel<0, true, 2>), gridw, dim3(256), 0, c->stream, a);
-        else if (a.mode == 0) hipLaunchKernelGGL((conv_x3_kernel<0, false, 2>), gridw, dim3(256), 0, c->stream, a);
-        else if (a.mode == 1 && tr) hipLaunchKernelGGL((conv_x3_kernel<1, true, 2>), gridw, dim3(256), 0, c->stream, a);
-        else if (a.mode == 1) hipLaunchKernelGGL((conv_x3_kernel<1, false, 2>), gridw, dim3(256), 0, c->stream, a);
-        else hipLaunchKernelGGL((conv_x3_kernel<2, false, 2>), gridw, dim3(256), 0, c->stream, a);
+        if (a.mode == 4 && tr) hipLaunchKernelGGL((conv_x3_kernel<4, true, 2>), gridw, dim3(256), 0, L.stream, a);
+        else if (a.mode == 4) hipLaunchKernelGGL((conv_x3_kernel<4, false, 2>), gridw, dim3(256), 0, L.stream, a);
+        else if (a.mode == 3 && tr) hipLaunchKernelGGL((conv_x3_kernel<3, true, 2>), gridw, dim3(256), 0, L.stream, a);
+        else if (a.mode == 3) hipLaunchKernelGGL((conv_x3_kernel<3, false, 2>), gridw, dim3(256), 0, L.stream, a);
+        else if (a.mode == 0 && tr) hipLaunchKernelGGL((conv_x3_kernel<0, true, 2>), gridw, dim3(256), 0, L.stream, a);
+        else if (a.mode == 0) hipLaunchKernelGGL((conv_x3_kernel<0, false, 2>), gridw, dim3(256), 0, L.stream, a);
+        else if (a.mode == 1 && tr) hipLaunchKernelGGL((conv_x3_kernel<1, true, 2>), gridw, dim3(256), 0, L.stream, a);
+        else if (a.mode == 1) hipLaunchKernelGGL((conv_x3_kernel<1, false, 2>), gridw, dim3(256), 0, L.stream, a);
+        else hipLaunchKernelGGL((conv_x3_kernel<2, false, 2>), gridw, dim3(256), 0, L.stream, a);
         break;
     }
     case ConvKernel::Pws2Strided: case ConvKernel::Pws2: case ConvKernel::Pws: case ConvKernel::Pw: {
-        if (ch.kernel == ConvKernel::Pws2Strided) iss_pws2_launch(a, c->stream, true);
-        else if (ch.kernel == ConvKernel::Pws2) iss_pws2_launch(a, c->stream);
-        else if (ch.kernel == ConvKernel::Pws) iss_pws_launch(a, dim3(std::min<unsigned>(a.nblk * a.nblk_n, 512u)), c->stream);
-        else if (ch.f16) hipLaunchKernelGGL(conv_x3_pw_kernel<true>, dim3(std::min<unsigned>(a.nblk * a.nblk_n, 768u)), dim3(256), 0, c->stream, a);
-        else hipLaunchKernelGGL(conv_x3_pw_kernel<false>, dim3(std::min<unsigned>(a.nblk * a.nblk_n, 768u)), dim3(256), 0, c->stream, a);
+        if (ch.kernel == ConvKernel::Pws2Strided) iss_pws2_launch(a, L.stream, true);
+        else if (ch.kernel == ConvKernel::Pws2) iss_pws2_launch(a, L.stream);
+        else if (ch.kernel == ConvKernel::Pws) iss_pws_launch(a, dim3(std::min<unsigned>(a.nblk * a.nblk_n, 512u)), L.stream);
+        else if (ch.f16) hipLaunchKernelGGL(conv_x3_pw_kernel<true>, dim3(std::min<unsigned>(a.nblk * a.nblk_n, 768u)), dim3(256), 0, L.stream, a);
+        else hipLaunchKernelGGL(conv_x3_pw_kernel<false>, dim3(std::min<unsigned>(a.nblk * a.nblk_n, 768u)), dim3(256), 0, L.stream, a);
         break;
     }
     case ConvKernel::Igemm: {
         const dim3 grid1(a.nblk * a.nblk_n);
-        if (a.mode == 0) hipLaunchKernelGGL(conv_igemm_kernel<0>, grid1, dim3(256), 0, c->stream, a);
-        else if (a.mode == 1) hipLaunchKernelGGL(conv_igemm_kernel<1>, grid1, dim3(256), 0, c->stream, a);
-        else hipLaunchKernelGGL(conv_igemm_kernel<2>, grid1, dim3(256), 0, c->stream, a);
+        if (a.mode == 0) hipLaunchKernelGGL(conv_igemm_kernel<0>, grid1, dim3(256), 0, L.stream, a);
+        else if (a.mode == 1) hipLaunchKernelGGL(conv_igemm_kernel<1>, grid1, dim3(256), 0, L.stream, a);
+        else hipLaunchKernelGGL(conv_igemm_kernel<2>, grid1, dim3(256), 0, L.stream, a);
         break;
     }
     case ConvKernel::Declined: return iss_fail(c, ISS_EINVAL, "internal: row %d has no kernel", r);
@@ -1482,40 +1483,40 @@
     return ISS_OK;
 }
 
-int run_conv(iss_ctx* c, IssNet& n, const ConvEnv& env, const PassIo& io, const ConvChoice& ch, int pend) {
+int run_conv(iss_ctx* c, IssLane& L, IssNet& n, const ConvEnv& env, const PassIo& io, const ConvChoice& ch, int pend) {
     const int32_t* R = &n.prog[(size_t)ch.row * ISS_PROG_COLS];
     ConvArgs a;
-    int rc = conv_args(c, n, io, env.bc, ch, a);
+    int rc = conv_args(c, L, n, io, env.bc, ch, a);
     if (rc) return rc;
     double fl = conv_flops(R, (double)a.M);
     if (ch.kernel == ConvKernel::Dhl) fl = 2.0 * R[ISS_C_CIN] * (double)R[ISS_C_COUT] * (double)env.bc;
     if (ch.kernel == ConvKernel::Pwc) fl += 2.0 * a.Cout * (double)a.Cout2 * (double)a.M;
     if (ch.kernel == ConvKernel::Pws2Dual) fl += 2.0 * a.Cin2 * (double)a.Cout * (double)a.M;
     if (ch.first == FirstLayer::Fused || ch.first == FirstLayer::Gather)
-        if ((rc = launch_shared_first_layer(c, n, io, pend, env.bc, env.rmin, env.rmax, a, &fl))) return rc;
-    return launch_conv(c, n, ch, a, fl);
-}
-
-int run_program(iss_ctx* c, IssNet& n, int bc, const int32_t* d_winrow, const float* d_stats,
+        if ((rc = launch_shared_first_layer(c, L, n, io, pend, env.bc, env.rmin, env.rmax, a, &fl))) return rc;
+    return launch_conv(c, L, n, ch, a, fl);
+}
+
+int run_program(iss_ctx* c, IssLane& L, IssNet& n, int bc, const int32_t* d_winrow, const float* d_stats,
                 const uint8_t* d_fin, const float* d_input, float** result, int rmin = 0, int rmax = -1,
                 bool share_first = false) {
     const PassIo io{d_winrow, d_stats, d_fin, d_input};
-    std::vector<ChlState> layout(std::max<size_t>(c->act.size(), (size_t)n.nbuf));
+    std::vector<ChlState> layout(std::max<size_t>(L.act.size(), (size_t)n.nbuf));
     ConvEnv env = make_env(n, bc, rmin, rmax, share_first, effective_precision(c, n), c->diag, d_winrow != nullptr, d_input != nullptr,
                            c->vbx_out.p != nullptr, layout.data());
     int pending = -1;
     for (int r = 0; r < n.nrows; ++r) {
         const int32_t* R = &n.prog[(size_t)r * ISS_PROG_COLS];
-        const float* in = R[ISS_C_IN] == ISS_BUF_INPUT ? d_input : (const float*)c->act[R[ISS_C_IN]].p;
-        float* out = (float*)c->act[R[ISS_C_OUT]].p;
+        const float* in = R[ISS_C_IN] == ISS_BUF_INPUT ? d_input : (const float*)L.act[R[ISS_C_IN]].p;
+        float* out = (float*)L.act[R[ISS_C_OUT]].p;
         const int op = R[ISS_C_OP];
         ChlState out_layout;
         if (op == ISS_OP_CONV) {
             if (pending < 0 && can_defer(env, r)) { pending = r; *result = out; continue; }
             const ConvChoice ch = select_conv(env, r, pending);
             int rc = ISS_OK;
-            if (ch.first == FirstLayer::Alone) rc = run_conv(c, n, env, io, select_row(env, pending, -1, -1, -1), -1);
-            if (!rc) rc = run_conv(c, n, env, io, ch, pending);
+            if (ch.first == FirstLayer::Alone) rc = run_conv(c, L, n, env, io, select_row(env, pending, -1, -1, -1), -1);
+            if (!rc) rc = run_conv(c, L, n, env, io, ch, pending);
             if (pending >= 0) layout[n.prog[(size_t)pending * ISS_PROG_COLS + ISS_C_OUT]] = ChlState{};
             pending = -1;
             if (rc) return rc;
@@ -1524,20 +1525,20 @@
             if (ch.rows == 2) {
                 layout[R[ISS_C_OUT]] = ChlState{};
                 R = &n.prog[(size_t)++r * ISS_PROG_COLS];
-                out = (float*)c->act[R[ISS_C_OUT]].p;
+                out = (float*)L.act[R[ISS_C_OUT]].p;
             }
             if (ch.out != OutLayout::F32) out_layout = ChlState{ch.out_np, ch.out_f16, ch.out == OutLayout::ChlDense};
         } else if (op == ISS_OP_POOL) {
             const long long total = (long long)bc * R[ISS_C_HO] * R[ISS_C_WO] * R[ISS_C_CIN];
-            iss_prof_begin(c, 2, 0);
-            hipLaunchKernelGGL(pool_kernel, dim3((unsigned)((total + 255) / 256)), dim3(256), 0, c->stream, in, out,
+            iss_prof_begin(c, 2, 0, &L);
+            hipLaunchKernelGGL(pool_kernel, dim3((unsigned)((total + 255) / 256)), dim3(256), 0, L.stream, in, out,
                                total, R[ISS_C_H], R[ISS_C_W], R[ISS_C_CIN], R[ISS_C_HO], R[ISS_C_WO], R[ISS_C_KH],
                                R[ISS_C_KW], R[ISS_C_SH], R[ISS_C_SW], R[ISS_C_PT], R[ISS_C_PL], R[ISS_C_POOLKIND]);
             iss_prof_end(c);
         } else if (op == ISS_OP_SOFTMAX) {
             const long long rows = (long long)bc * R[ISS_C_H] * R[ISS_C_W];
-            iss_prof_begin(c, 2, 0);
-            hipLaunchKernelGGL(softmax_kernel, dim3((unsigned)((rows + 255) / 256)), dim3(256), 0, c->stream, in, out,
+            iss_prof_begin(c, 2, 0, &L);
+            hipLaunchKernelGGL(softmax_kernel, dim3((unsigned)((rows + 255) / 256)), dim3(256), 0, L.stream, in, out,
                                rows, R[ISS_C_CIN]);
             iss_prof_end(c);
         } else if (op == ISS_OP_ACT) {
@@ -1546,8 +1547,8 @@
             { const int32_t bits = R[ISS_C_ACTPARAM]; memcpy(&alpha, &bits, sizeof(float)); }
             { const int32_t bits = R[ISS_C_ACTPARAM2]; memcpy(&p2, &bits, sizeof(float)); }
             { const int32_t bits = R[ISS_C_ACTPARAM3]; memcpy(&p3, &bits, sizeof(float)); }
-            iss_prof_begin(c, 2, 0);
-            hipLaunchKernelGGL(act_kernel, dim3((unsigned)std::min<long long>((total + 1023) / 1024, 1 << 20)), dim3(256), 0, c->stream, in, out, total,
+            iss_prof_begin(c, 2, 0, &L);
+            hipLaunchKernelGGL(act_kernel, dim3((unsigned)std::min<long long>((total + 1023) / 1024, 1 << 20)), dim3(256), 0, L.stream, in, out, total,
                                R[ISS_C_ACT], alpha, p2, p3);
             iss_prof_end(c);
         } else if (op == ISS_OP_ELT) {
@@ -1555,22 +1556,22 @@
             const long long hw = (long long)R[ISS_C_H] * R[ISS_C_W];
             const bool chan = k == ISS_ELT_COPY || k == ISS_ELT_ZERO;
             const long long total = (long long)bc * hw * (chan ? R[ISS_C_KH] : R[ISS_C_CIN]);
-            const float* res = R[ISS_C_RES] >= 0 ? (const float*)c->act[R[ISS_C_RES]].p : nullptr;
+            const float* res = R[ISS_C_RES] >= 0 ? (const float*)L.act[R[ISS_C_RES]].p : nullptr;
             if (res && layout[R[ISS_C_RES]].np) return iss_fail(c, ISS_EINVAL, "internal: row %d reads a CHL tensor", r);
             int st[3] = {0, 0, 0};
             if (k == ISS_ELT_PERMUTE) {
                 const int sin[3] = {R[ISS_C_W] * R[ISS_C_CIN], R[ISS_C_CIN], 1};
                 st[0] = sin[R[ISS_C_KH]]; st[1] = sin[R[ISS_C_KW]]; st[2] = sin[R[ISS_C_SH]];
             }
-            iss_prof_begin(c, 2, 0);
-            hipLaunchKernelGGL(elt_kernel, dim3((unsigned)std::min<long long>((total + 255) / 256, 1 << 20)), dim3(256), 0, c->stream, in, res, out,
+            iss_prof_begin(c, 2, 0, &L);
+            hipLaunchKernelGGL(elt_kernel, dim3((unsigned)std::min<long long>((total + 255) / 256, 1 << 20)), dim3(256), 0, L.stream, in, res, out,
                                total, k, R[ISS_C_CIN], R[ISS_C_COUT], R[ISS_C_KH], R[ISS_C_PT], R[ISS_C_PL],
                                R[ISS_C_HO], R[ISS_C_WO], R[ISS_C_COUT], st[0], st[1], st[2], R[ISS_C_ORDER] == 1 ? 1 : 0);
             iss_prof_end(c);
         } else if (op == ISS_OP_STATPOOL) {
             const long long total = (long long)bc * R[ISS_C_H] * R[ISS_C_CIN];
-            iss_prof_begin(c, 2, 0);
-            hipLaunchKernelGGL(statpool_kernel, dim3((unsigned)((total + 255) / 256)), dim3(256), 0, c->stream, in, out,
+            iss_prof_begin(c, 2, 0, &L);
+            hipLaunchKernelGGL(statpool_kernel, dim3((unsigned)((total + 255) / 256)), dim3(256), 0, L.stream, in, out,
                                total, R[ISS_C_H], R[ISS_C_W], R[ISS_C_CIN]);
             iss_prof_end(c);
         }
@@ -1579,6 +1580,15 @@
         layout[R[ISS_C_OUT]] = out_layout;
         if (op != ISS_OP_CONV && R[ISS_C_IN] != ISS_BUF_INPUT && layout[R[ISS_C_IN]].np)
             return iss_fail(c, ISS_EINVAL, "internal: row %d reads a CHL tensor", r);
+    }
+    return ISS_OK;
+}
+
+int reserve_act(iss_ctx* c, IssLane& L, IssNet& n, int bc) {
+    if ((int)L.act.size() < n.nbuf) L.act.resize(n.nbuf);
+    for (int i = 0; i < n.nbuf; ++i) {
+        int rc = iss_reserve(c, L.act[i], (size_t)bc * n.buf_elems[i] * sizeof(float) + issk::ISS_ACT_SLACK);
+        if (rc) return rc;
     }
     return ISS_OK;
 }
@@ -1594,12 +1604,27 @@
     bc = std::min<int64_t>(bc, ((1ll << 31) - 1) / emax);
     if (bc < 1) return iss_fail(c, ISS_EINVAL, "network activation of %lld floats per sample exceeds the 2^31 element limit", (long long)emax);
     if (bc > 8) bc -= bc % 8;
-    if ((int)c->act.size() < n.nbuf) c->act.resize(n.nbuf);
-    for (int i = 0; i < n.nbuf; ++i) {
-        int rc = iss_reserve(c, c->act[i], (size_t)bc * n.buf_elems[i] * sizeof(float) + issk::ISS_ACT_SLACK);
-        if (rc) return rc;
-    }
     *bc_out = (int)bc;
+    return reserve_act(c, c->lane[0], n, (int)bc);
+}
+
+IssLane* lane1(iss_ctx* c, IssNet& n, int bc) {
+    IssLane& L = c->lane[1];
+    if (!L.stream && hipStreamCreateWithFlags(&L.stream, hipStreamNonBlocking) != hipSuccess) L.stream = nullptr;
+    if (L.stream && reserve_act(c, L, n, bc) == ISS_OK) return &L;
+    (void)hipGetLastError();
+    for (auto& b : L.act) { if (b.p) (void)hipFree(b.p); b.p = nullptr; b.cap = 0; }
+    c->err.clear();
+    return nullptr;
+}
+
+int lane_order(iss_ctx* c, hipStream_t from, hipStream_t to) {
+    hipEvent_t ev = iss_event_get(c);
+    if (!ev) return iss_fail(c, ISS_EHIP, "cannot create an event");
+    hipError_t e = hipEventRecord(ev, from);
+    if (e == hipSuccess) e = hipStreamWaitEvent(to, ev, 0);
+    c->ev_pool.push_back(ev);
+    if (e != hipSuccess) return iss_fail(c, ISS_EHIP, "ordering two lanes failed: %s", hipGetErrorString(e));
     return ISS_OK;
 }
 
@@ -1775,26 +1800,35 @@
         for (int i = 1; i < nlive; ++i) { gmin = std::min(gmin, rows[i]); gmax = std::max(gmax, rows[i]); }
         if ((long long)(gmax - gmin + 68) * 4 > (long long)nlive * 68) share = false;
     }
-    for (int s0 = 0; s0 < nlive; s0 += bc) {
-        const int cur = std::min(bc, nlive - s0);
-        float* res = nullptr;
-        int rmin = rows[s0], rmax = rows[s0];
-        for (int i = s0 + 1; i < s0 + cur; ++i) { rmin = std::min(rmin, rows[i]); rmax = std::max(rmax, rows[i]); }
-        rc = run_program(c, n, cur, (const int32_t*)c->d_winrow.p + s0, (const float*)c->d_stats.p + 2 * (size_t)s0,
-                         (const uint8_t*)d_fin + s0, nullptr, &res, rmin, rmax, share);
-        if (rc) return rc;
-        if (compact) {
-            const long long ct = (long long)cur * n.out_dim;
-            iss_prof_begin(c, 2, 0);
-            hipLaunchKernelGGL(scatter_probs_kernel, dim3((unsigned)((ct + 255) / 256)), dim3(256), 0, c->stream, (const float*)res,
-                               (const uint8_t*)d_fin + s0, d_map + s0, (long long)cur, n.out_dim, (float*)c->d_out.p, (uint8_t*)c->d_finite.p);
-            iss_prof_end(c);
-            ISS_HIP(c, hipGetLastError());
-        } else {
-            ISS_HIP(c, hipMemcpyAsync((float*)c->d_out.p + (size_t)s0 * n.out_dim, res, (size_t)cur * n.out_dim * 4,
-                                      hipMemcpyDeviceToDevice, c->stream));
-        }
-    }
+    IssLane* l1 = nlive > bc && !c->prof && c->lanes > 1 ? lane1(c, n, bc) : nullptr;
+    if (l1 && (rc = lane_order(c, c->stream, l1->stream))) return rc;
+    auto run_passes = [&]() -> int {
+        for (int s0 = 0, pass = 0; s0 < nlive; s0 += bc, ++pass) {
+            IssLane& L = l1 && (pass & 1) ? *l1 : c->lane[0];
+            const int cur = std::min(bc, nlive - s0);
+            float* res = nullptr;
+            int rmin = rows[s0], rmax = rows[s0];
+            for (int i = s0 + 1; i < s0 + cur; ++i) { rmin = std::min(rmin, rows[i]); rmax = std::max(rmax, rows[i]); }
+            int prc = run_program(c, L, n, cur, (const int32_t*)c->d_winrow.p + s0, (const float*)c->d_stats.p + 2 * (size_t)s0,
+                                  (const uint8_t*)d_fin + s0, nullptr, &res, rmin, rmax, share);
+            if (prc) return prc;
+            if (compact) {
+                const long long ct = (long long)cur * n.out_dim;
+                iss_prof_begin(c, 2, 0, &L);
+                hipLaunchKernelGGL(scatter_probs_kernel, dim3((unsigned)((ct + 255) / 256)), dim3(256), 0, L.stream, (const float*)res,
+                                   (const uint8_t*)d_fin + s0, d_map + s0, (long long)cur, n.out_dim, (float*)c->d_out.p, (uint8_t*)c->d_finite.p);
+                iss_prof_end(c);
+                ISS_HIP(c, hipGetLastError());
+            } else {
+                ISS_HIP(c, hipMemcpyAsync((float*)c->d_out.p + (size_t)s0 * n.out_dim, res, (size_t)cur * n.out_dim * 4,
+                                          hipMemcpyDeviceToDevice, L.stream));
+            }
+        }
+        return ISS_OK;
+    };
+    rc = run_passes();
+    if (l1) { const int jrc = lane_order(c, l1->stream, c->stream); if (!rc) rc = jrc; }
+    if (rc) return rc;
     if (!compact) {
         hipLaunchKernelGGL(mask_probs_kernel, dim3((unsigned)((tot + 255) / 256)), dim3(256), 0, c->stream,
                            (float*)c->d_out.p, (const uint8_t*)c->d_finite.p, (long long)nslots, n.out_dim);
@@ -1844,7 +1878,7 @@
         const int cur = std::min(bc, nsamp - s0);
         ISS_HIP(c, hipMemcpyAsync(c->d_in.p, x + (size_t)s0 * in_elems, (size_t)cur * in_elems * 4, hipMemcpyHostToDevice, c->stream));
         float* res = nullptr;
-        rc = run_program(c, n, cur, nullptr, nullptr, nullptr, (const float*)c->d_in.p, &res);
+        rc = run_program(c, c->lane[0], n, cur, nullptr, nullptr, nullptr, (const float*)c->d_in.p, &res);
         if (rc) return rc;
         ISS_HIP(c, hipMemcpyAsync((float*)c->d_out.p + (size_t)s0 * n.out_dim, res, (size_t)cur * n.out_dim * 4,
                                   hipMemcpyDeviceToDevice, c->stream));
@@ -1878,7 +1912,7 @@
     for (int s0 = 0; s0 < nwin; s0 += bc) {
         const int cur = std::min(bc, nwin - s0);
         float* res = nullptr;
-        rc = run_program(c, n, cur, (const int32_t*)c->d_winrow.p + s0, nullptr, nullptr, nullptr, &res);
+        rc = run_program(c, c->lane[0], n, cur, (const int32_t*)c->d_winrow.p + s0, nullptr, nullptr, nullptr, &res);
         if (rc) return rc;
         ISS_HIP(c, hipMemcpyAsync((float*)c->d_out.p + (size_t)s0 * n.out_dim, res, (size_t)cur * n.out_dim * 4,
                                   hipMemcpyDeviceToDevice, c->stream));
diff --git a/inaspeechsegmenter_amd/csrc/iss_core.cpp b/inaspeechsegmenter_amd/csrc/iss_core.cpp
--- a/inaspeechsegmenter_amd/csrc/iss_core.cpp
+++ b/inaspeechsegmenter_amd/csrc/iss_core.cpp
@@ -19,7 +19,11 @@
 
 int iss_reserve(iss_ctx* c, DevBuf& b, size_t bytes) {
     if (bytes <= b.cap) return ISS_OK;
-    if (b.p) { ISS_HIP(c, hipStreamSynchronize(c->stream)); ISS_HIP(c, hipFree(b.p)); b.p = nullptr; b.cap = 0; }
+    if (b.p) {
+        ISS_HIP(c, hipStreamSynchronize(c->stream));
+        if (c->lane[1].stream) ISS_HIP(c, hipStreamSynchronize(c->lane[1].stream));
+        ISS_HIP(c, hipFree(b.p)); b.p = nullptr; b.cap = 0;
+    }
     size_t want = bytes + (bytes >> 3) + 256;
     hipError_t e = hipMalloc(&b.p, want);
     if (e != hipSuccess) {
@@ -61,6 +65,7 @@
         delete c;
         return iss_fail(nullptr, ISS_EHIP, "cannot create a stream on device %d", device_id);
     }
+    c->lane[0].stream = c->stream;
     *out = c;
     return ISS_OK;
 }
@@ -71,15 +76,16 @@
     if (!c) return;
     (void)hipSetDevice(c->device);
     if (c->stream) (void)hipStreamSynchronize(c->stream);
+    if (c->lane[1].stream) (void)hipStreamSynchronize(c->lane[1].stream);
     for (int i = 0; i < ISS_MAX_NETS; ++i) iss_cnn_free(c, i);
     void* singles[] = {c->d_window, c->d_melw, c->d_mellim, c->d_tw, c->d_vbx_window, c->d_vbx_melw, c->d_vbx_mellim};
     for (void* p : singles) if (p) (void)hipFree(p);
-    DevBuf* bufs[] = {&c->sig, &c->mspec, &c->loge, &c->d_winrow, &c->d_stats, &c->d_finite, &c->d_out, &c->d_in, &c->raw1, &c->d_rowflag, &c->d_lfinite,
+    DevBuf* bufs[] = {&c->sig, &c->mspec, &c->loge, &c->d_winrow, &c->d_stats, &c->d_finite, &c->d_out, &c->d_in, &c->lane[0].raw1, &c->lane[1].raw1, &c->d_rowflag, &c->d_lfinite,
                       &c->vbx_sig, &c->vbx_dither, &c->vbx_fb, &c->vbx_out, &c->vbx_meta, &c->rs_src, &c->rs_jobs,
                       &c->flac.src, &c->flac.rows, &c->flac.status, &c->flac.stage,
                       &c->adpcm.src, &c->adpcm.rows, &c->adpcm.status, &c->adpcm.stage};
     for (DevBuf* b : bufs) free_buf(*b);
-    for (auto& b : c->act) free_buf(b);
+    for (auto& l : c->lane) for (auto& b : l.act) free_buf(b);
     for (auto& f : c->rs_filters) if (f.d_taps) (void)hipFree(f.d_taps);
     for (auto& p : c->pending) { (void)hipEventDestroy(p.a); (void)hipEventDestroy(p.b); }
     for (auto& e : c->ev_pool) (void)hipEventDestroy(e);
@@ -89,6 +95,7 @@
     if (c->h_rowflag) (void)hipHostFree(c->h_rowflag);
     iss_comm_destroy(c);
     free_buf(c->comm_send); free_buf(c->comm_recv);
+    if (c->lane[1].stream) (void)hipStreamDestroy(c->lane[1].stream);
     if (c->stream) (void)hipStreamDestroy(c->stream);
     delete c;
 }
@@ -100,6 +107,13 @@
     return ISS_OK;
 }
 
+extern "C" int iss_set_lanes(iss_ctx* c, int lanes) {
+    if (!c) return ISS_EINVAL;
+    if (lanes != 1 && lanes != 2) return iss_fail(c, ISS_EINVAL, "iss_set_lanes: %d lanes (1 or 2)", lanes);
+    c->lanes = lanes;
+    return ISS_OK;
+}
+
 extern "C" int iss_synchronize(iss_ctx* c) {
     if (!c) return ISS_EINVAL;
     ISS_HIP(c, hipSetDevice(c->device));
@@ -111,11 +125,12 @@
     if (!c) return ISS_EINVAL;
     ISS_HIP(c, hipSetDevice(c->device));
     ISS_HIP(c, hipStreamSynchronize(c->stream));
-    std::vector<DevBuf*> bufs = {&c->raw1, &c->d_stats, &c->d_finite, &c->d_lfinite, &c->d_out, &c->d_in, &c->d_winrow, &c->d_rowflag,
+    if (c->lane[1].stream) ISS_HIP(c, hipStreamSynchronize(c->lane[1].stream));
+    std::vector<DevBuf*> bufs = {&c->lane[0].raw1, &c->lane[1].raw1, &c->d_stats, &c->d_finite, &c->d_lfinite, &c->d_out, &c->d_in, &c->d_winrow, &c->d_rowflag,
                                  &c->vbx_fb, &c->vbx_meta, &c->vbx_sig, &c->rs_src, &c->rs_jobs,
                                  &c->flac.src, &c->flac.rows, &c->flac.status, &c->flac.stage,
                                  &c->adpcm.src, &c->adpcm.rows, &c->adpcm.status, &c->adpcm.stage};
-    for (auto& b : c->act) bufs.push_back(&b);
+    for (auto& l : c->lane) for (auto& b : l.act) bufs.push_back(&b);
     for (DevBuf* b : bufs) {
         if (!b->p) continue;
         if (b->cap >= 4) ISS_HIP(c, hipMemsetD32Async((hipDeviceptr_t)b->p, (int)word, b->cap / 4, c->stream));
@@ -338,14 +353,17 @@
     return ISS_OK;
 }
 
-static hipEvent_t get_event(iss_ctx* c) {
+hipEvent_t iss_event_get(iss_ctx* c) {
     if (!c->ev_pool.empty()) { hipEvent_t e = c->ev_pool.back(); c->ev_pool.pop_back(); return e; }
-    hipEvent_t e; (void)hipEventCreate(&e); return e;
-}
-void iss_prof_begin(iss_ctx* c, int kind, double flops) {
+    hipEvent_t e = nullptr;
+    if (hipEventCreate(&e) != hipSuccess) { (void)hipGetLastError(); return nullptr; }
+    return e;
+}
+void iss_prof_begin(iss_ctx* c, int kind, double flops, const IssLane* lane) {
     if (!c->prof) return;
-    iss_ctx::Pending p; p.a = get_event(c); p.b = get_event(c); p.kind = kind; p.sub = -1; p.row = -1; p.flops = flops;
-    (void)hipEventRecord(p.a, c->stream);
+    iss_ctx::Pending p; p.a = iss_event_get(c); p.b = iss_event_get(c); p.stream = lane ? lane->stream : c->stream;
+    p.kind = kind; p.sub = -1; p.row = -1; p.flops = flops;
+    (void)hipEventRecord(p.a, p.stream);
     c->pending.push_back(p);
 }
 void iss_prof_tag(iss_ctx* c, int sub) {
@@ -367,7 +385,7 @@
 }
 void iss_prof_end(iss_ctx* c) {
     if (!c->prof || c->pending.empty()) return;
-    (void)hipEventRecord(c->pending.back().b, c->stream);
+    (void)hipEventRecord(c->pending.back().b, c->pending.back().stream);
 }
 void iss_prof_collect(iss_ctx* c) {
     for (auto& p : c->pending) {
@@ -383,7 +401,8 @@
                 e->ms += ms; e->launches += 1; e->flops += p.flops;
             }
         }
-        c->ev_pool.push_back(p.a); c->ev_pool.push_back(p.b);
+        if (p.a) c->ev_pool.push_back(p.a);
+        if (p.b) c->ev_pool.push_back(p.b);
     }
     c->pending.clear();
 }
diff --git a/inaspeechsegmenter_amd/csrc/iss_internal.h b/inaspeechsegmenter_amd/csrc/iss_internal.h
--- a/inaspeechsegmenter_amd/csrc/iss_internal.h
+++ b/inaspeechsegmenter_amd/csrc/iss_internal.h
@@ -65,6 +65,12 @@
     int guard_slots = 0;
 };
 
+struct IssLane {
+    hipStream_t stream = nullptr;
+    std::vector<DevBuf> act;
+    DevBuf raw1;
+};
+
 struct iss_ctx {
     int device = -1;
     hipStream_t stream = nullptr;
@@ -108,9 +114,9 @@
     float guard_threshold = 5e-4f;
     bool in_guard = false;
     uint32_t diag = 0;
-    std::vector<DevBuf> act;
+    IssLane lane[2];
+    int lanes = 2;
     DevBuf d_winrow, d_stats, d_finite, d_out, d_in;
-    DevBuf raw1;
 
     bool vbx_tables = false;
     double* d_vbx_window = nullptr;
@@ -137,7 +143,7 @@
     double prof_flops[ISS_PROF_KINDS] = {};
     double prof_row_ms[ISS_PROF_ROWS] = {};
     int64_t prof_row_launch[ISS_PROF_ROWS] = {};
-    struct Pending { hipEvent_t a, b; int kind; int sub; int row; double flops; std::string inst; };
+    struct Pending { hipEvent_t a, b; hipStream_t stream; int kind; int sub; int row; double flops; std::string inst; };
     std::vector<Pending> pending;
     struct Inst { std::string name; double ms = 0; int64_t launches = 0; double flops = 0; };
     std::vector<Inst> prof_inst;
@@ -146,6 +152,7 @@
 
 int iss_fail(iss_ctx* c, int code, const char* fmt, ...);
 int iss_reserve(iss_ctx* c, DevBuf& b, size_t bytes);
+hipEvent_t iss_event_get(iss_ctx* c);
 void iss_set_signal(iss_ctx* c, const void* ptr, int kind, int64_t n);
 int iss_stage_host(iss_ctx* c, const void* src, size_t bytes, void** pinned_out, int* slot_out);
 void iss_stage_mark(iss_ctx* c, int slot);
@@ -167,7 +174,7 @@
                             hipGetErrorString(e__), __FILE__, __LINE__);                  \
     } while (0)
 
-void iss_prof_begin(iss_ctx* c, int kind, double flops);
+void iss_prof_begin(iss_ctx* c, int kind, double flops, const IssLane* lane = nullptr);
 void iss_prof_tag(iss_ctx* c, int sub);
 void iss_prof_row(iss_ctx* c, int row);
 void iss_prof_inst(iss_ctx* c, const char* fmt, ...);
diff --git a/include/iss.h b/include/iss.h
--- a/include/iss.h
+++ b/include/iss.h
@@ -23,6 +23,7 @@
 const char* iss_last_error(const iss_ctx* ctx);
 const char* iss_version(void);
 int         iss_set_workspace_limit(iss_ctx* ctx, uint64_t bytes);
+int         iss_set_lanes(iss_ctx* ctx, int lanes);
 int         iss_synchronize(iss_ctx* ctx);
 
 
```

New measurement: 7.028 (median of 6 runs). No clear change (+0.7%).
